# IGNF/StrataNet2-Vegetation-Coverage-Maps

Measured on AMD Instinct MI355X. Metric: plots/s fwd+bwd, 32k-pt synthetic plots, batch 16/GPU, higher is better.
Workload: dtype f32; 1 GPU; C2 ref-arch: 16 plots/GPU x 32768 pts, SA npoint 1024/256 + global, r 1/2 m, train step fwd+P2+loss+bwd+Adam, inputs resident in HBM; plots_per_gpu=16, points_per_plot=32768, batches_per_geometry_pass=8, exchange=none (single GPU), parallelism=single GPU, ranks_seen=1, exchange_in_graph=False

## Files before the change

include/strata_hip.h:

```cpp
#ifndef STRATA_HIP_H
#define STRATA_HIP_H

#include <stddef.h>

#ifdef __cplusplus
extern "C" {
#endif

#define SN2_VERSION 102
#define SN2_EINVAL (-1)
#define SN2_ELIMIT (-2)

#define SN2_MAX_NEIGHBORS 2000
#define SN2_STAT_SLOTS 1024

int sn2_version(void);
int sn2_debug_mfma_chain(const float *a, const float *b, float *d, int mode, void *stream);
int sn2_debug_spin(int blocks, long long clocks, int *out, void *stream);

int sn2_debug_fp1_backward_parts(int mask);
int sn2_debug_fp_rows_form(int form);
int sn2_debug_fp_table_form(int form);
#define SN2_PROBE_SINK_WORDS 4096
int sn2_debug_stream_probe(const float *src, float *dst, size_t n_floats, int mode, float *sink, void *stream);
int sn2_debug_mfma_probe(int mode, int iters, float *sink, double *flops, void *stream);

typedef struct sn2_block {
    int cin, cout;
    const float *W, *b;
    const float *gamma, *beta;
    float *running_mean, *running_var;
    float *a, *c;
    float *mean, *invstd;
    float *stat_slots;
    float *dW, *db, *dgamma, *dbeta;
    int grad_replicas, grad_replica_stride;
    int mma_bf16;
    long long *num_batches_tracked;
    int frozen_stats;
} sn2_block;
#define SN2_BN_FROZEN_KEEP 2
int sn2_grad_reduce(float *flat, int n, int replicas, int stride, void *stream);


int sn2_pack_rows(const float *cloud, const float *xyz, int B, int C, int N, float *rows0, void *stream);

#define SN2_FPS_WS_GRID_WORDS 4104
#define SN2_FPS_WS_XCHG_WORDS 4096
#define SN2_FPS_WS_CTL_WORDS 32
#define SN2_FPS_WS_GRID_OFFSET(B, N) (5L * (B) * (N))
#define SN2_FPS_WS_CTL_OFFSET(B, N) (SN2_FPS_WS_GRID_OFFSET(B, N) + (long)(SN2_FPS_WS_GRID_WORDS + SN2_FPS_WS_XCHG_WORDS) * (B))
#define SN2_FPS_WS_RANK_OFFSET(B, N) (SN2_FPS_WS_CTL_OFFSET(B, N) + SN2_FPS_WS_CTL_WORDS)
#define SN2_FPS_WS_WORDS(B, N) (SN2_FPS_WS_RANK_OFFSET(B, N) + 1L * (B) * (N))
size_t sn2_fps_ws_words(int B, int N);
size_t sn2_fps_ws_grid_offset(int B, int N);
size_t sn2_fps_ws_ctl_offset(int B, int N);
size_t sn2_fps_ws_rank_offset(int B, int N);
int sn2_fps(const float *pos_soa, int B, int N, int M, const int *start, int *idx, float *cpos_soa,
            float *cpos_aos, int *order_ws, void *stream);
int sn2_fps_waves(const float *pos_soa, int B, int N, int M, const int *start, int *idx, float *cpos_soa,
                  float *cpos_aos, int *order_ws, int waves, void *stream);
int sn2_fps_status(const float *pos_soa, int B, int N, int M, const int *start, int *idx, float *cpos_soa,
                   float *cpos_aos, int *order_ws, int waves, unsigned *status, void *stream);
int sn2_fps_live(const float *pos_soa, int B, int N, int M, const int *start, const int *n_live, int *idx, float *cpos_soa,
                 float *cpos_aos, int *order_ws, int waves, int *n_live_out, unsigned *status, void *stream);
int sn2_debug_fps_spin_limit(unsigned sweeps);

int sn2_ball_query(const float *src_soa, int B, int N, const float *cpos_soa, int M, float r2, int cap,
                   int *nbr, int *cnt, unsigned long long *total, const int *fps_ws, void *stream);

int sn2_count_sum(const int *cnt, int n, unsigned long long *total, void *stream);
int sn2_count_sum_group(const int *cnt, int G, int n, unsigned long long *total, size_t total_stride, void *stream);

#define SN2_THREE_NN_WS_WORDS(B, S) ((size_t)(B) * (4 * (size_t)(S) + 1032))
size_t sn2_three_nn_ws_words(int B, int S);
int sn2_three_nn(const float *src_soa, int B, int S, const float *dst_soa, int T, int k, int *idx, float *w,
                 void *ws, const int *dst_fps_ws, void *stream);
#define SN2_THREE_NN_XY_WS_WORDS(B, S, T) ((size_t)(B) * (4 * (size_t)(S) + 5 * (size_t)(T) + 1032))
size_t sn2_three_nn_xy_ws_words(int B, int S, int T);
int sn2_three_nn_xy(const float *src_soa, int B, int S, const float *dst_soa, int T, int k, int *idx, float *w,
                    void *ws, void *stream);

int sn2_prepare_plots(const float *raw, long T, const int *offsets, const float *centers, const float *fake_xy, int n_fake,
                      const int *idx, int B, int N, int train, const double *rot, const int *flips, const float *noise,
                      const long *noise_offsets, long noise_T, float z_max, float *cloud, float *xyz, void *stream);

#define SN2_SUBSAMPLE_LDS 1
#define SN2_SUBSAMPLE_GLOBAL 2
#define SN2_SUBSAMPLE_COARSE 4
#define SN2_SUBSAMPLE_LDS_MAX 16384
int sn2_subsample_form(int n_max, int N);
size_t sn2_subsample_ws_words(int B, int n_max, int N, int form);
int sn2_subsample(const int *offsets, int extra, int n_max, int B, int N, unsigned long long seed, const long long *plot_keys,
                  int form, int *ws, size_t ws_words, int *idx, void *stream);

int sn2_train_batch_ws_words(int B, int n_max, int N, size_t *words);
int sn2_train_batch(const float *raw, long T, const int *offsets, const float *centers, const double *coverages, int P,
                    const int *plot_ids, int B, const float *fake_xy, int n_fake, int n_max, int N, int M1, float z_max,
                    unsigned long long seed, long long epoch, const double *cos_sin, int train, int noise, int *ws,
                    size_t ws_words, float *cloud, float *xyz, double *gt, int *fps_start, void *stream);
int sn2_train_batch_live(const float *raw, long T, const int *offsets, const float *centers, const double *coverages, int P,
                         const int *plot_ids, int B, const float *fake_xy, int n_fake, int n_max, int N, int M1, float z_max,
                         unsigned long long seed, long long epoch, const double *cos_sin, int train, int noise, int *ws,
                         size_t ws_words, float *cloud, float *xyz, double *gt, int *fps_start, int *n_live, void *stream);

int sn2_plots_append(const float *src_raw, long src_T, const int *src_offsets, const float *src_centers, const float *src_cov,
                     const int *sel, int K, float *dst_raw, long cap_T, int *dst_offsets, float *dst_centers, double *dst_cov,
                     int cap_P, int P0, long T0, const int *dst_start, long new_T, void *stream);

#define SN2_ZNORM_WS_WORDS(n, cells) ((size_t)5 * (n) + 3 * (size_t)(cells) + 8)
size_t sn2_znorm_ws_words(int n, long cells);
int sn2_znorm(const float *x, const float *y, const float *z, int n, float radius, float x_min, float y_min, float x_max,
              float y_max, int *ws, float *zmin, float *z_out, void *stream);

size_t sn2_parcel_count_ws_words(int P, int rows);
size_t sn2_parcel_znorm_ws_words(long T, float radius, float x_min, float y_min, float x_max, float y_max);
int sn2_parcel_count(const float *cloud, long T, int L, int rows, const float *centers, int P, const int *cell_start,
                     const int *cell_items, int GX, int GY, double gx0, double gy0, double cell_inv, float radius, int *ws,
                     size_t ws_words, int *prefix, long long *total, void *stream);
int sn2_parcel_fill(const float *cloud, long T, int L, int rows, const float *centers, int P, const int *cell_start,
                    const int *cell_items, int GX, int GY, double gx0, double gy0, double cell_inv, float radius, int *prefix,
                    const int *plot_base, long sum_n, float *raw, int *point_index, void *stream);
int sn2_parcel_znorm(const float *cloud, long T, float x_min, float y_min, float x_max, float y_max, float radius,
                     float disc_radius, const int *offsets, const float *centers, int P, const int *point_index, long sum_n,
                     int *ws, size_t ws_words, float *raw, void *stream);

typedef struct sn2_sa {
    int B, Nsrc, M, cap;
    int cf;
    int nl;
    const float *feat; int feat_stride;
    const float *spos; int spos_stride;
    const float *cpos;
    const int *nbr, *cnt;
    const unsigned long long *total;
    const int *order;
    sn2_block blk[2];
    float *ext; int *arg;
    float *out;
    const float *dout;
    float *dfeat;
    float *bwd_ws;
} sn2_sa;
#define SN2_SA_BWD_WS_REPLICAS 32
#define SN2_SA_BWD_WS_WORDS (SN2_SA_BWD_WS_REPLICAS * 2 * 16 * 12)
#define SN2_SA_SOLO_MIN 64
#define SN2_SA_QUAD_MIN 8
#define SN2_SA_OCT_MIN 4
#define SN2_SA_SOLO_FLAG 0x40000000
#define SN2_SA_OCT_FLAG 0x20000000
#define SN2_SA_PACKED_ITEMS(M) ((M) / 8 + 2)
#define SN2_SA_ORDER_WORDS(B, M) ((size_t)4 * (B) * (M) + (size_t)16 * (B) * SN2_SA_PACKED_ITEMS(M) + 8)
size_t sn2_sa_order_words(int B, int M);
int sn2_sa_order(const int *cnt, int B, int M, int *order, void *stream);
int sn2_sa_order_group(const int *cnt, int G, int B, int M, int *order, size_t stride_words, void *stream);
int sn2_sa_forward(const sn2_sa *p, int training, void *stream);
int sn2_sa_backward(const sn2_sa *p, void *stream);

typedef struct sn2_fp {
    int B, R_per_plot, S_per_plot;
    int ca, cb;
    const float *src; int src_stride; const float *src_a, *src_c;
    const int *knn_idx; const float *knn_w;
    const float *skip; int skip_stride;
    sn2_block blk;
    float *h; int h_stride;
    const float *dy;
    float *dsrc; int dsrc_stride;
    float *dskip; int dskip_stride;
    float *du_scratch;
    float *scatter_ws;
    int scatter_ready;
    const int *bn_sums_done;
    float *src_ws;
    int act_bf16;
    const int *row_perm;
} sn2_fp;
#define SN2_INTERP_CHUNKS(R, S) ((3 * (size_t)(R) + 62) / 63 + (size_t)(S))
#define SN2_FP_SRC_WS_WORDS(B, R, S, cout) ((size_t)(B) * SN2_INTERP_CHUNKS(R, S) * ((((cout) + 3) / 4) * 4))
size_t sn2_interp_chunks(int R_per_plot, int S_per_plot);
size_t sn2_fp_src_ws_words(int B, int R_per_plot, int S_per_plot, int cout);
#define SN2_INTERP_WS_WORDS(B, R, S) \
    ((size_t)(B) * (S) * (((R) + 2047) / 2048 + 6) + 6 * (size_t)(B) * (R) + 64 + 4 * (size_t)(B) * SN2_INTERP_CHUNKS(R, S))
size_t sn2_interp_ws_words(int B, int R_per_plot, int S_per_plot);
int sn2_interp_index(const int *knn_idx, const float *knn_w, const float *src_pos, int B, int R_per_plot,
                     int S_per_plot, float *ws, void *stream);
int sn2_interp_index_perm(const int *knn_idx, const float *knn_w, const float *src_pos, const int *row_perm, int B,
                          int R_per_plot, int S_per_plot, float *ws, void *stream);
int sn2_interp_index_group(const int *knn_idx, const float *knn_w, const float *src_pos, const int *row_perm, int G, int B,
                           int R_per_plot, int S_per_plot, float *ws, size_t ws_stride_words, void *stream);
int sn2_fp_forward(const sn2_fp *p, int training, void *stream);
int sn2_fp_backward(const sn2_fp *p, void *stream);

int sn2_plot_max_forward(const float *h, const float *a, const float *c, int B, int R_per_plot, int C, float *out,
                         int *arg, void *stream);
int sn2_plot_max_backward(const float *dout, const int *arg, int B, int R_per_plot, int C, float *dy, void *stream);

int sn2_global_pool_backward(const float *du, int du_stride, const int *arg, const float *h, const float *mean,
                             const float *invstd, int B, int R_per_plot, int C, float *dx, float *dy, float *dgamma,
                             float *dbeta, void *stream);

#define SN2_GLOBAL_MAX_PLOTS 28
#define SN2_GLOBAL_XCHG_WORDS(B) ((size_t)2 * (size_t)(B) * 4 * 128)
#define SN2_GLOBAL_CTL_WORDS 8
size_t sn2_global_xchg_words(int B);
int sn2_global_level_forward(const sn2_fp *sa3, const sn2_fp *fp3, float *x3, int *arg3, unsigned long long *xchg,
                             unsigned *ctl, void *stream);
#define SN2_GLOBAL_BWD_MAX_ROWS 256
#define SN2_GLOBAL_BWD_XCHG_WORDS ((size_t)2 * SN2_GLOBAL_MAX_PLOTS * 128)
#define SN2_GLOBAL_BWD_CTL_WORDS 64
int sn2_global_level_backward(const sn2_fp *sa3, const sn2_fp *fp3, const int *arg3, unsigned long long *xchg, unsigned *ctl,
                              void *stream);
int sn2_debug_global_spin_limit(unsigned sweeps);

#define SN2_HEAD_LOSS_MAX_PLOTS 128
typedef struct sn2_loss_grad {
    const float *pred;
    const double *gt;
    const float *proba;
    const double *pdf;
    const double *grad_total;
    const int *arg, *nocc, *pix;
    int B, N, D;
    double m, e;
} sn2_loss_grad;

typedef struct sn2_head {
    int R, cin, f_stride;
    const float *f, *fa, *fc;
    const float *W1, *b1, *W2, *b2;
    float *coverages, *proba;
    const float *dcoverages, *dproba;
    float *dy;
    float *dW1, *db1, *dW2, *db2;
    int grad_replicas, grad_replica_stride;
    const int *drop_mask;
    float drop_scale;
    int act_bf16;
    float *zero_fill; long zero_fill_words;
    const sn2_loss_grad *loss;
} sn2_head;
int sn2_head_forward(const sn2_head *p, void *stream);
int sn2_fp_head_eval(const sn2_fp *p, const sn2_head *hd, void *stream);
int sn2_head_backward(const sn2_head *p, void *stream);
int sn2_debug_head_backward_occupancy(int bf16, int with_loss);
int sn2_head_bn_sums(const sn2_head *p, const float *gamma, const float *beta, const float *mean, const float *invstd,
                     float *dgamma, float *dbeta, int *ok, void *stream);
int sn2_fp_bn_sums(const sn2_fp *p, const float *gamma, const float *beta, const float *mean, const float *invstd,
                   float *dgamma, float *dbeta, int *ok, void *stream);


int sn2_plot_project_forward(const float *pred_pointwise, const float *cloud_xy, long plot_stride, int B, int N,
                             int D, unsigned long long *keys, int *pix, int *arg, int *nocc, float *pred,
                             void *stream);
#define SN2_P2_KEY_PARTS(N) (((N) + 4095) / 4096 < 1 ? 1 : (((N) + 4095) / 4096 > 64 ? 64 : ((N) + 4095) / 4096))
size_t sn2_p2_key_parts(int N);
int sn2_plot_pixels(const float *cloud_xy, long plot_stride, int B, int N, int D, float *mm, int *pix, void *stream);
int sn2_plot_project_forward_pix(const float *pred_pointwise, const int *pix, int B, int N, int D,
                                 unsigned long long *keys, int *arg, int *nocc, float *pred, void *stream);
int sn2_plot_project_backward(const float *dpred, const int *arg, const int *nocc, const int *pix, int B, int N,
                              int D, float *dpointwise, void *stream);

int sn2_raster_project(const float *coverages, const float *cloud_xy, long plot_stride, int B, int N, int D,
                       int diam_meters, unsigned long long *keys, int *pix, float *rasters, void *stream);

int sn2_mosaic_merge(const float *rasters, const float *weights, const int *offsets, int B, int D, int H, int W,
                     float *mean, float *wsum, int win_y0, int win_x0, int win_h, int win_w, void *stream);

#define SN2_MOSAIC_HIST_WORDS 10004
int sn2_mosaic_finalize(const float *mean, const float *wsum, int H, int W, int *hist_ws, double *sum_ws, float *thr_out,
                        float *out, void *stream);

#define SN2_MOSAIC_CROP_MAX_BANDS 8
#define SN2_MOSAIC_CROP_MAX_EDGES (1 << 20)
#define SN2_MOSAIC_CROP_MAX_BLOCKS 2048
#define SN2_MOSAIC_CROP_BLOCKS(H, W) \
    ((size_t)(H) * (((size_t)(W) + 255) / 256) < SN2_MOSAIC_CROP_MAX_BLOCKS ? (size_t)(H) * (((size_t)(W) + 255) / 256) \
                                                                           : (size_t)SN2_MOSAIC_CROP_MAX_BLOCKS)
#define SN2_MOSAIC_CROP_WS_WORDS(C, H, W) (4 * (size_t)(C) * SN2_MOSAIC_CROP_BLOCKS(H, W))
extern size_t sn2_mosaic_crop_ws_words(int C, int H, int W);
int sn2_mosaic_crop_stats(float *bands, int C, int H, int W, double x_min, double y_max, double pix, const double *edges, int E,
                          void *ws, double *mean, long long *count, void *stream);

int sn2_kde_lookup(const float *cloud, int B, int C, int N, int z_channel, float z_max, const double *X, const double *Y,
                   int K, double *pdf, void *stream);
#define SN2_KDE_FIT_MAX_K 65536
#define SN2_KDE_FIT_ABS_SLOTS 256
#define SN2_KDE_FIT_SLICES 8
#define SN2_KDE_FIT_WS_WORDS(K) \
    (2 * ((4 + 3 * SN2_KDE_FIT_SLICES) * (size_t)(K) + 3 * (((size_t)(K) + 255) / 256)) + SN2_KDE_FIT_ABS_SLOTS)
size_t sn2_kde_fit_ws_words(int K);
int sn2_kde_fit(const float *z, long n, double bw, int K, void *ws, double *X, double *Y, void *stream);
#define SN2_LOSS_BLOCKS 1024
int sn2_loss_forward(const float *pred, const double *gt, int B, const float *proba, const double *pdf, int R, double m,
                     double e, double *partials, double *out, void *stream);
int sn2_loss_backward(const float *pred, const double *gt, int B, const float *proba, const double *pdf, int R, double m,
                      double e, const double *grad_total, float *dpred, float *dproba, void *stream);

#define SN2_PROJECTED_LOSS_WS (2 * 512 + 2)
int sn2_projected_loss_forward(const float *coverages, const int *pix, const float *proba, const double *pdf, const double *gt,
                               int B, int N, int D, double m, double e, unsigned long long *keys, int *arg, int *nocc,
                               float *pred, double *partials, double *out, void *stream);
int sn2_projected_loss_backward(const float *pred, const double *gt, int B, const float *proba, const double *pdf, int N, int D,
                                double m, double e, const double *grad_total, const int *arg, const int *nocc, const int *pix,
                                float *dcoverages, float *dproba, void *stream);

#define SN2_PLOT_LOSSES_SLICE_ROWS 2048
#define SN2_PLOT_LOSSES_SLICES(N) \
    (((N) + SN2_PLOT_LOSSES_SLICE_ROWS - 1) / SN2_PLOT_LOSSES_SLICE_ROWS < 1 ? 1 : \
     (((N) + SN2_PLOT_LOSSES_SLICE_ROWS - 1) / SN2_PLOT_LOSSES_SLICE_ROWS > 64 ? 64 : ((N) + SN2_PLOT_LOSSES_SLICE_ROWS - 1) / SN2_PLOT_LOSSES_SLICE_ROWS))
size_t sn2_plot_losses_ws_words(int B, int N, int D);
int sn2_plot_losses(const float *coverages, const int *pix, const float *proba, const double *pdf, const double *gt, int B, int N,
                    int D, double m, double e, void *ws, float *pred, double *out, void *stream);

int sn2_adam_step(float *param, const float *grad, float *exp_avg, float *exp_avg_sq, int n, float lr, float beta1,
                  float beta2, float eps, float weight_decay, int *step_dev ,
                  float grad_scale, void *stream);

#define SN2_METER_TERMS 4
int sn2_adam_step_dev(float *param, const float *grad, float *exp_avg, float *exp_avg_sq, int n, const float *lr_dev, float beta1,
                      float beta2, float eps, float weight_decay, int *step_dev, float grad_scale, const double *terms, int n_terms,
                      double *meter, void *stream);


typedef struct sn2_net_layer {
    int cin, cout;
    const float *W, *b, *gamma, *beta;
    float *running_mean, *running_var;
    long long *num_batches_tracked;
    int gW, gb, ggamma, gbeta;
    int mma_bf16;
} sn2_net_layer;

typedef struct sn2_net_model {
    sn2_net_layer sa1[2], sa2, sa3, fp3, fp2, fp1;
    const float *lin1_W, *lin1_b, *lin2_W, *lin2_b;
    int g_lin1_W, g_lin1_b, g_lin2_W, g_lin2_b;
    int n_flat;
    float r1_sq, r2_sq;
    int max_neighbors;
    float drop_p;
    int fuse_global_level;
    int fuse_eval_head;
    int source_side;
    int fps_waves_shared, fps_waves_many;
} sn2_net_model;

typedef struct sn2_net_dims {
    int B, N, M1, M2;
    int cap1, cap2;
    int act_bf16;
    int p2_diam_pix;
} sn2_net_dims;

typedef struct sn2_net_geo {
    const float *xyz;
    int *idx1; float *pos1_soa, *pos1_aos; int *ws1;
    int *nbr1, *cnt1; unsigned long long *tot1; int *ord1;
    int *idx2; float *pos2_soa, *pos2_aos; int *ws2;
    int *nbr2, *cnt2; unsigned long long *tot2; int *ord2;
    const float *pos3;
    int *knn3_idx; float *knn3_w;
    int *knn2_idx; float *knn2_w;
    int *knn1_idx; float *knn1_w;
    float *inv3, *inv2, *inv1;
    int *nn_ws2, *nn_ws1;
    const int *rank1;
    float *rows0;
    int *p2_pix; float *p2_mm;
} sn2_net_geo;

typedef struct sn2_net_act {
    float *aux;
    float *stats;
    float *ext1; int *arg1; float *x1;
    float *ext2; int *arg2; float *x2;
    float *h_sa3, *h3;
    float *x3; int *arg3;
    float *h2;
    void *h1;
    float *src_ws1, *src_ws2;
    float *cov, *proba;
    const int *drop_mask;
    float *bwd_arena; long bwd_arena_words;
} sn2_net_act;

#define SN2_NET_GRAD_IMAGES 32
typedef struct sn2_net_bwd {
    const float *dcov, *dproba;
    float *arena; long arena_words;
    int images, image_stride;
    float *dy2, *dy3, *dx1, *dx2, *dx3, *dy_sa3;
    float *sa1_ws;
    void *dy1, *du1;
    float *du2, *du3;
    int *bn_ok;
    float *src_ws1, *src_ws2;
    int defer_grad_reduce;
    int arena_is_zero;
    int frozen_stats;
    unsigned long long *gl_xchg; unsigned *gl_ctl;
    const sn2_loss_grad *loss;
} sn2_net_bwd;

#define SN2_NET_FORK 1
#define SN2_NET_SHARED 2
#define SN2_NET_INVERTED 4
#define SN2_NET_DEFER_JOIN 8
#define SN2_NET_INPUT_ONLY 16
#define SN2_NET_HAS_ROWS0 32
#define SN2_NET_JOIN_PENDING 64
#define SN2_NET_WITH_GEOMETRY 128
#define SN2_NET_HAS_INVERTED 256

typedef struct sn2_net_io {
    const float *cloud;
    const int *fps_start;
    unsigned *fps_status;
    unsigned long long *gl_xchg; unsigned *gl_ctl;
    void *stream_b, *stream_c, *stream_pack;
    void *ctx;
    int flags;
    int training;
    const int *fps_live;
    int *fps_live1;
} sn2_net_io;

int sn2_net_ctx_create(void **ctx);
int sn2_net_ctx_destroy(void *ctx);
int sn2_net_geo_carve(const sn2_net_model *m, const sn2_net_dims *d, void *base, sn2_net_geo *out, size_t *bytes);
int sn2_net_act_carve(const sn2_net_model *m, const sn2_net_dims *d, int training, void *base, sn2_net_act *out, size_t *bytes);
int sn2_net_bwd_carve(const sn2_net_model *m, const sn2_net_dims *d, void *arena_base, void *scratch_base, sn2_net_bwd *out,
                      size_t *arena_bytes, size_t *scratch_bytes);
int sn2_net_geometry(const sn2_net_model *m, const sn2_net_dims *d, const sn2_net_geo *g, const sn2_net_io *io, void *stream);
int sn2_net_forward(const sn2_net_model *m, const sn2_net_dims *d, const sn2_net_geo *g, const sn2_net_act *a,
                    const sn2_net_io *io, void *stream);
int sn2_net_backward(const sn2_net_model *m, const sn2_net_dims *d, const sn2_net_geo *g, const sn2_net_act *a,
                     const sn2_net_bwd *b, void *stream);

int sn2_adam_step_images(float *param, float *grad_images, int replicas, int stride, float *exp_avg, float *exp_avg_sq, int n,
                         float lr, float beta1, float beta2, float eps, float weight_decay, int *step_dev, float grad_scale,
                         void *stream);
int sn2_adam_step_images_dev(float *param, float *grad_images, int replicas, int stride, float *exp_avg, float *exp_avg_sq, int n,
                             const float *lr_dev, float beta1, float beta2, float eps, float weight_decay, int *step_dev,
                             float grad_scale, const double *terms, int n_terms, double *meter, void *stream);

int sn2_fps_fills_ws(int B, int N, int M);
int sn2_three_nn_uses_grid(int S, int T);
int sn2_fp_rows_small(long R);
int sn2_fp_source_side(long R, int cb, int force);
int sn2_global_level_forward_route(int B, int bf16);
int sn2_global_level_backward_route(int B, int M2, int frozen, int bf16);
int sn2_head_loss_route(int B, int N, int D);

#ifdef __cplusplus
}
#endif
#endif
```

stratanet2_vegetation_coverage_maps_amd/_lib.py:

```python
import ctypes
import functools
import os
from ctypes import POINTER, Structure, c_double, c_float, c_int, c_long, c_longlong, c_void_p

HERE = os.path.dirname(os.path.abspath(__file__))
LIB_PATH = os.path.join(HERE, "csrc", "libstrata_hip.so")

CONSTANTS = {
    "SN2_VERSION": 102, "SN2_EINVAL": -1, "SN2_ELIMIT": -2,
    "SN2_MAX_NEIGHBORS": 2000, "SN2_STAT_SLOTS": 1024, "SN2_BN_FROZEN_KEEP": 2,
    "SN2_FPS_WS_GRID_WORDS": 4104, "SN2_FPS_WS_CTL_WORDS": 32,
    "SN2_SUBSAMPLE_LDS": 1, "SN2_SUBSAMPLE_GLOBAL": 2, "SN2_SUBSAMPLE_COARSE": 4, "SN2_SUBSAMPLE_LDS_MAX": 16384,
    "SN2_SA_BWD_WS_WORDS": 32 * 2 * 16 * 12,
    "SN2_GLOBAL_MAX_PLOTS": 28, "SN2_GLOBAL_CTL_WORDS": 8, "SN2_GLOBAL_BWD_MAX_ROWS": 256,
    "SN2_GLOBAL_BWD_XCHG_WORDS": 2 * 28 * 128, "SN2_GLOBAL_BWD_CTL_WORDS": 64,
    "SN2_MOSAIC_HIST_WORDS": 10004, "SN2_MOSAIC_CROP_MAX_BANDS": 8, "SN2_MOSAIC_CROP_MAX_EDGES": 1 << 20,
    "SN2_MOSAIC_CROP_MAX_BLOCKS": 2048, "SN2_KDE_FIT_MAX_K": 65536, "SN2_LOSS_BLOCKS": 1024, "SN2_PROJECTED_LOSS_WS": 2 * 512 + 2,
    "SN2_NET_GRAD_IMAGES": 32, "SN2_METER_TERMS": 4,
    "SN2_NET_FORK": 1, "SN2_NET_SHARED": 2, "SN2_NET_INVERTED": 4, "SN2_NET_DEFER_JOIN": 8, "SN2_NET_INPUT_ONLY": 16,
    "SN2_NET_HAS_ROWS0": 32, "SN2_NET_JOIN_PENDING": 64, "SN2_NET_WITH_GEOMETRY": 128, "SN2_NET_HAS_INVERTED": 256,
}
globals().update(CONSTANTS)
MAX_NEIGHBORS, STAT_SLOTS, BN_FROZEN_KEEP = CONSTANTS["SN2_MAX_NEIGHBORS"], CONSTANTS["SN2_STAT_SLOTS"], CONSTANTS["SN2_BN_FROZEN_KEEP"]
(NET_FORK, NET_SHARED, NET_INVERTED, NET_DEFER_JOIN, NET_INPUT_ONLY, NET_HAS_ROWS0, NET_JOIN_PENDING, NET_WITH_GEOMETRY,
 NET_HAS_INVERTED) = (CONSTANTS["SN2_NET_" + n] for n in ("FORK", "SHARED", "INVERTED", "DEFER_JOIN", "INPUT_ONLY", "HAS_ROWS0",
                                                          "JOIN_PENDING", "WITH_GEOMETRY", "HAS_INVERTED"))


class Block(Structure):
    _fields_ = [("cin", c_int), ("cout", c_int), ("W", c_void_p), ("b", c_void_p), ("gamma", c_void_p),
                ("beta", c_void_p), ("running_mean", c_void_p), ("running_var", c_void_p), ("a", c_void_p),
                ("c", c_void_p), ("mean", c_void_p), ("invstd", c_void_p), ("stat_slots", c_void_p),
                ("dW", c_void_p), ("db", c_void_p), ("dgamma", c_void_p), ("dbeta", c_void_p),
                ("grad_replicas", c_int), ("grad_replica_stride", c_int), ("mma_bf16", c_int),
                ("num_batches_tracked", c_void_p), ("frozen_stats", c_int)]


class SA(Structure):
    _fields_ = [("B", c_int), ("Nsrc", c_int), ("M", c_int), ("cap", c_int), ("cf", c_int), ("nl", c_int),
                ("feat", c_void_p), ("feat_stride", c_int), ("spos", c_void_p), ("spos_stride", c_int),
                ("cpos", c_void_p), ("nbr", c_void_p), ("cnt", c_void_p), ("total", c_void_p), ("order", c_void_p),
                ("blk", Block * 2),
                ("ext", c_void_p), ("arg", c_void_p), ("out", c_void_p), ("dout", c_void_p), ("dfeat", c_void_p),
                ("bwd_ws", c_void_p)]


class FP(Structure):
    _fields_ = [("B", c_int), ("R_per_plot", c_int), ("S_per_plot", c_int), ("ca", c_int), ("cb", c_int),
                ("src", c_void_p), ("src_stride", c_int), ("src_a", c_void_p), ("src_c", c_void_p),
                ("knn_idx", c_void_p), ("knn_w", c_void_p), ("skip", c_void_p), ("skip_stride", c_int),
                ("blk", Block), ("h", c_void_p), ("h_stride", c_int), ("dy", c_void_p), ("dsrc", c_void_p),
                ("dsrc_stride", c_int), ("dskip", c_void_p), ("dskip_stride", c_int), ("du_scratch", c_void_p),
                ("scatter_ws", c_void_p), ("scatter_ready", c_int), ("bn_sums_done", c_void_p), ("src_ws", c_void_p),
                ("act_bf16", c_int), ("row_perm", c_void_p)]


class LossGrad(Structure):
    _fields_ = [(n, c_void_p) for n in ("pred", "gt", "proba", "pdf", "grad_total", "arg", "nocc", "pix")] + [
        ("B", c_int), ("N", c_int), ("D", c_int), ("m", c_double), ("e", c_double)]


class Head(Structure):
    _fields_ = [("R", c_int), ("cin", c_int), ("f_stride", c_int), ("f", c_void_p), ("fa", c_void_p),
                ("fc", c_void_p), ("W1", c_void_p), ("b1", c_void_p), ("W2", c_void_p), ("b2", c_void_p),
                ("coverages", c_void_p), ("proba", c_void_p), ("dcoverages", c_void_p), ("dproba", c_void_p),
                ("dy", c_void_p), ("dW1", c_void_p), ("db1", c_void_p), ("dW2", c_void_p), ("db2", c_void_p),
                ("grad_replicas", c_int), ("grad_replica_stride", c_int), ("drop_mask", c_void_p), ("drop_scale", c_float),
                ("act_bf16", c_int), ("zero_fill", c_void_p), ("zero_fill_words", c_long), ("loss", POINTER(LossGrad))]


class NetLayer(Structure):
    _fields_ = [("cin", c_int), ("cout", c_int), ("W", c_void_p), ("b", c_void_p), ("gamma", c_void_p), ("beta", c_void_p),
                ("running_mean", c_void_p), ("running_var", c_void_p), ("num_batches_tracked", c_void_p),
                ("gW", c_int), ("gb", c_int), ("ggamma", c_int), ("gbeta", c_int), ("mma_bf16", c_int)]


class NetModel(Structure):
    _fields_ = [("sa1", NetLayer * 2), ("sa2", NetLayer), ("sa3", NetLayer), ("fp3", NetLayer), ("fp2", NetLayer), ("fp1", NetLayer),
                ("lin1_W", c_void_p), ("lin1_b", c_void_p), ("lin2_W", c_void_p), ("lin2_b", c_void_p),
                ("g_lin1_W", c_int), ("g_lin1_b", c_int), ("g_lin2_W", c_int), ("g_lin2_b", c_int), ("n_flat", c_int),
                ("r1_sq", c_float), ("r2_sq", c_float), ("max_neighbors", c_int), ("drop_p", c_float),
                ("fuse_global_level", c_int), ("fuse_eval_head", c_int), ("source_side", c_int),
                ("fps_waves_shared", c_int), ("fps_waves_many", c_int)]


class NetDims(Structure):
    _fields_ = [("B", c_int), ("N", c_int), ("M1", c_int), ("M2", c_int), ("cap1", c_int), ("cap2", c_int), ("act_bf16", c_int),
                ("p2_diam_pix", c_int)]


class NetGeo(Structure):
    _fields_ = [(n, c_void_p) for n in (
        "xyz", "idx1", "pos1_soa", "pos1_aos", "ws1", "nbr1", "cnt1", "tot1", "ord1",
        "idx2", "pos2_soa", "pos2_aos", "ws2", "nbr2", "cnt2", "tot2", "ord2", "pos3",
        "knn3_idx", "knn3_w", "knn2_idx", "knn2_w", "knn1_idx", "knn1_w", "inv3", "inv2", "inv1", "nn_ws2", "nn_ws1",
        "rank1", "rows0", "p2_pix", "p2_mm")]


class NetAct(Structure):
    _fields_ = [(n, c_void_p) for n in (
        "aux", "stats", "ext1", "arg1", "x1", "ext2", "arg2", "x2", "h_sa3", "h3", "x3", "arg3", "h2", "h1", "src_ws1", "src_ws2",
        "cov", "proba", "drop_mask", "bwd_arena")] + [("bwd_arena_words", c_long)]


class NetBwd(Structure):
    _fields_ = [("dcov", c_void_p), ("dproba", c_void_p), ("arena", c_void_p), ("arena_words", c_long), ("images", c_int),
                ("image_stride", c_int)] + [(n, c_void_p) for n in (
                    "dy2", "dy3", "dx1", "dx2", "dx3", "dy_sa3", "sa1_ws", "dy1", "du1", "du2", "du3", "bn_ok", "src_ws1", "src_ws2")] + [
                        ("defer_grad_reduce", c_int), ("arena_is_zero", c_int), ("frozen_stats", c_int), ("gl_xchg", c_void_p),
                        ("gl_ctl", c_void_p), ("loss", POINTER(LossGrad))]


class NetIO(Structure):
    _fields_ = [("cloud", c_void_p), ("fps_start", c_void_p), ("fps_status", c_void_p), ("gl_xchg", c_void_p), ("gl_ctl", c_void_p),
                ("stream_b", c_void_p), ("stream_c", c_void_p), ("stream_pack", c_void_p), ("ctx", c_void_p), ("flags", c_int),
                ("training", c_int), ("fps_live", c_void_p), ("fps_live1", c_void_p)]


SIGNATURES = {
    "sn2_version": [],
    "sn2_debug_mfma_chain": [c_void_p, c_void_p, c_void_p, c_int, c_void_p],
    "sn2_debug_spin": [c_int, c_longlong, c_void_p, c_void_p],
    "sn2_debug_fp1_backward_parts": [c_int],
    "sn2_debug_fp_rows_form": [c_int],
    "sn2_debug_fp_table_form": [c_int],
    "sn2_debug_stream_probe": [c_void_p, c_void_p, ctypes.c_size_t, c_int, c_void_p, c_void_p],
    "sn2_debug_mfma_probe": [c_int, c_int, c_void_p, POINTER(c_double), c_void_p],
    "sn2_pack_rows": [c_void_p, c_void_p, c_int, c_int, c_int, c_void_p, c_void_p],
    "sn2_fps": [c_void_p, c_int, c_int, c_int, c_void_p, c_void_p, c_void_p, c_void_p, c_void_p, c_void_p],
    "sn2_fps_waves": [c_void_p, c_int, c_int, c_int, c_void_p, c_void_p, c_void_p, c_void_p, c_void_p, c_int, c_void_p],
    "sn2_fps_status": [c_void_p, c_int, c_int, c_int, c_void_p, c_void_p, c_void_p, c_void_p, c_void_p, c_int, c_void_p, c_void_p],
    "sn2_fps_live": [c_void_p, c_int, c_int, c_int, c_void_p, c_void_p, c_void_p, c_void_p, c_void_p, c_void_p, c_int, c_void_p, c_void_p,
                     c_void_p],
    "sn2_debug_fps_spin_limit": [ctypes.c_uint],
    "sn2_ball_query": [c_void_p, c_int, c_int, c_void_p, c_int, c_float, c_int, c_void_p, c_void_p, c_void_p, c_void_p,
                       c_void_p],
    "sn2_three_nn": [c_void_p, c_int, c_int, c_void_p, c_int, c_int, c_void_p, c_void_p, c_void_p, c_void_p, c_void_p],
    "sn2_count_sum": [c_void_p, c_int, c_void_p, c_void_p],
    "sn2_count_sum_group": [c_void_p, c_int, c_int, c_void_p, ctypes.c_size_t, c_void_p],
    "sn2_three_nn_xy": [c_void_p, c_int, c_int, c_void_p, c_int, c_int, c_void_p, c_void_p, c_void_p, c_void_p],
    "sn2_prepare_plots": [c_void_p, c_long, c_void_p, c_void_p, c_void_p, c_int, c_void_p, c_int, c_int, c_int, c_void_p,
                          c_void_p, c_void_p, c_void_p, c_long, c_float, c_void_p, c_void_p, c_void_p],
    "sn2_znorm": [c_void_p, c_void_p, c_void_p, c_int, c_float, c_float, c_float, c_float, c_float, c_void_p, c_void_p,
                  c_void_p, c_void_p],
    "sn2_parcel_count": [c_void_p, c_long, c_int, c_int, c_void_p, c_int, c_void_p, c_void_p, c_int, c_int, c_double, c_double,
                         c_double, c_float, c_void_p, ctypes.c_size_t, c_void_p, c_void_p, c_void_p],
    "sn2_parcel_fill": [c_void_p, c_long, c_int, c_int, c_void_p, c_int, c_void_p, c_void_p, c_int, c_int, c_double, c_double,
                        c_double, c_float, c_void_p, c_void_p, c_long, c_void_p, c_void_p, c_void_p],
    "sn2_parcel_znorm": [c_void_p, c_long, c_float, c_float, c_float, c_float, c_float, c_float, c_void_p, c_void_p, c_int,
                         c_void_p, c_long, c_void_p, ctypes.c_size_t, c_void_p, c_void_p],
    "sn2_subsample_form": [c_int, c_int],
    "sn2_subsample": [c_void_p, c_int, c_int, c_int, c_int, ctypes.c_ulonglong, c_void_p, c_int, c_void_p, ctypes.c_size_t,
                      c_void_p, c_void_p],
    "sn2_train_batch_ws_words": [c_int, c_int, c_int, POINTER(ctypes.c_size_t)],
    "sn2_train_batch": [c_void_p, c_long, c_void_p, c_void_p, c_void_p, c_int, c_void_p, c_int, c_void_p, c_int, c_int, c_int, c_int,
                        c_float, ctypes.c_ulonglong, c_longlong, c_void_p, c_int, c_int, c_void_p, ctypes.c_size_t, c_void_p, c_void_p,
                        c_void_p, c_void_p, c_void_p],
    "sn2_train_batch_live": [c_void_p, c_long, c_void_p, c_void_p, c_void_p, c_int, c_void_p, c_int, c_void_p, c_int, c_int, c_int, c_int,
                             c_float, ctypes.c_ulonglong, c_longlong, c_void_p, c_int, c_int, c_void_p, ctypes.c_size_t, c_void_p,
                             c_void_p, c_void_p, c_void_p, c_void_p, c_void_p],
    "sn2_plots_append": [c_void_p, c_long, c_void_p, c_void_p, c_void_p, c_void_p, c_int, c_void_p, c_long, c_void_p, c_void_p,
                         c_void_p, c_int, c_int, c_long, c_void_p, c_long, c_void_p],
    "sn2_sa_order": [c_void_p, c_int, c_int, c_void_p, c_void_p],
    "sn2_sa_order_group": [c_void_p, c_int, c_int, c_int, c_void_p, ctypes.c_size_t, c_void_p],
    "sn2_sa_forward": [POINTER(SA), c_int, c_void_p],
    "sn2_sa_backward": [POINTER(SA), c_void_p],
    "sn2_grad_reduce": [c_void_p, c_int, c_int, c_int, c_void_p],
    "sn2_interp_index": [c_void_p, c_void_p, c_void_p, c_int, c_int, c_int, c_void_p, c_void_p],
    "sn2_interp_index_perm": [c_void_p, c_void_p, c_void_p, c_void_p, c_int, c_int, c_int, c_void_p, c_void_p],
    "sn2_interp_index_group": [c_void_p, c_void_p, c_void_p, c_void_p, c_int, c_int, c_int, c_int, c_void_p, ctypes.c_size_t, c_void_p],
    "sn2_fp_forward": [POINTER(FP), c_int, c_void_p],
    "sn2_fp_backward": [POINTER(FP), c_void_p],
    "sn2_plot_max_forward": [c_void_p, c_void_p, c_void_p, c_int, c_int, c_int, c_void_p, c_void_p, c_void_p],
    "sn2_plot_max_backward": [c_void_p, c_void_p, c_int, c_int, c_int, c_void_p, c_void_p],
    "sn2_global_pool_backward": [c_void_p, c_int, c_void_p, c_void_p, c_void_p, c_void_p, c_int, c_int, c_int, c_void_p, c_void_p,
                                 c_void_p, c_void_p, c_void_p],
    "sn2_global_level_forward": [POINTER(FP), POINTER(FP), c_void_p, c_void_p, c_void_p, c_void_p, c_void_p],
    "sn2_global_level_backward": [POINTER(FP), POINTER(FP), c_void_p, c_void_p, c_void_p, c_void_p],
    "sn2_debug_global_spin_limit": [ctypes.c_uint],
    "sn2_head_forward": [POINTER(Head), c_void_p],
    "sn2_fp_head_eval": [POINTER(FP), POINTER(Head), c_void_p],
    "sn2_fp_bn_sums": [POINTER(FP), c_void_p, c_void_p, c_void_p, c_void_p, c_void_p, c_void_p, c_void_p, c_void_p],
    "sn2_head_bn_sums": [POINTER(Head), c_void_p, c_void_p, c_void_p, c_void_p, c_void_p, c_void_p, c_void_p, c_void_p],
    "sn2_head_backward": [POINTER(Head), c_void_p],
    "sn2_debug_head_backward_occupancy": [c_int, c_int],
    "sn2_plot_project_forward": [c_void_p, c_void_p, c_long, c_int, c_int, c_int, c_void_p, c_void_p, c_void_p,
                                 c_void_p, c_void_p, c_void_p],
    "sn2_plot_pixels": [c_void_p, c_long, c_int, c_int, c_int, c_void_p, c_void_p, c_void_p],
    "sn2_plot_project_forward_pix": [c_void_p, c_void_p, c_int, c_int, c_int, c_void_p, c_void_p, c_void_p, c_void_p, c_void_p],
    "sn2_plot_project_backward": [c_void_p, c_void_p, c_void_p, c_void_p, c_int, c_int, c_int, c_void_p, c_void_p],
    "sn2_raster_project": [c_void_p, c_void_p, c_long, c_int, c_int, c_int, c_int, c_void_p, c_void_p, c_void_p,
                           c_void_p],
    "sn2_mosaic_merge": [c_void_p, c_void_p, c_void_p, c_int, c_int, c_int, c_int, c_void_p, c_void_p,
                         c_int, c_int, c_int, c_int, c_void_p],
    "sn2_mosaic_finalize": [c_void_p, c_void_p, c_int, c_int, c_void_p, c_void_p, c_void_p, c_void_p, c_void_p],
    "sn2_mosaic_crop_stats": [c_void_p, c_int, c_int, c_int, c_double, c_double, c_double, c_void_p, c_int, c_void_p, c_void_p,
                              c_void_p, c_void_p],
    "sn2_kde_lookup": [c_void_p, c_int, c_int, c_int, c_int, c_float, c_void_p, c_void_p, c_int, c_void_p, c_void_p],
    "sn2_kde_fit": [c_void_p, c_long, c_double, c_int, c_void_p, c_void_p, c_void_p, c_void_p],
    "sn2_loss_forward": [c_void_p, c_void_p, c_int, c_void_p, c_void_p, c_int, c_double, c_double, c_void_p, c_void_p,
                         c_void_p],
    "sn2_loss_backward": [c_void_p, c_void_p, c_int, c_void_p, c_void_p, c_int, c_double, c_double, c_void_p, c_void_p,
                          c_void_p, c_void_p],
    "sn2_adam_step": [c_void_p, c_void_p, c_void_p, c_void_p, c_int, c_float, c_float, c_float, c_float, c_float,
                      c_void_p, c_float, c_void_p],
    "sn2_adam_step_dev": [c_void_p, c_void_p, c_void_p, c_void_p, c_int, c_void_p, c_float, c_float, c_float, c_float,
                          c_void_p, c_float, c_void_p, c_int, c_void_p, c_void_p],
    "sn2_projected_loss_forward": [c_void_p, c_void_p, c_void_p, c_void_p, c_void_p, c_int, c_int, c_int, c_double, c_double, c_void_p,
                                   c_void_p, c_void_p, c_void_p, c_void_p, c_void_p, c_void_p],
    "sn2_projected_loss_backward": [c_void_p, c_void_p, c_int, c_void_p, c_void_p, c_int, c_int, c_double, c_double, c_void_p, c_void_p,
                                    c_void_p, c_void_p, c_void_p, c_void_p, c_void_p],
    "sn2_plot_losses": [c_void_p, c_void_p, c_void_p, c_void_p, c_void_p, c_int, c_int, c_int, c_double, c_double, c_void_p, c_void_p,
                        c_void_p, c_void_p],
    "sn2_adam_step_images": [c_void_p, c_void_p, c_int, c_int, c_void_p, c_void_p, c_int, c_float, c_float, c_float, c_float, c_float,
                             c_void_p, c_float, c_void_p],
    "sn2_adam_step_images_dev": [c_void_p, c_void_p, c_int, c_int, c_void_p, c_void_p, c_int, c_void_p, c_float, c_float, c_float,
                                 c_float, c_void_p, c_float, c_void_p, c_int, c_void_p, c_void_p],
    "sn2_net_ctx_create": [POINTER(c_void_p)],
    "sn2_net_ctx_destroy": [c_void_p],
    "sn2_net_geo_carve": [POINTER(NetModel), POINTER(NetDims), c_void_p, POINTER(NetGeo), POINTER(ctypes.c_size_t)],
    "sn2_net_act_carve": [POINTER(NetModel), POINTER(NetDims), c_int, c_void_p, POINTER(NetAct), POINTER(ctypes.c_size_t)],
    "sn2_net_bwd_carve": [POINTER(NetModel), POINTER(NetDims), c_void_p, c_void_p, POINTER(NetBwd), POINTER(ctypes.c_size_t),
                          POINTER(ctypes.c_size_t)],
    "sn2_net_geometry": [POINTER(NetModel), POINTER(NetDims), POINTER(NetGeo), POINTER(NetIO), c_void_p],
    "sn2_net_forward": [POINTER(NetModel), POINTER(NetDims), POINTER(NetGeo), POINTER(NetAct), POINTER(NetIO), c_void_p],
    "sn2_net_backward": [POINTER(NetModel), POINTER(NetDims), POINTER(NetGeo), POINTER(NetAct), POINTER(NetBwd), c_void_p],
    "sn2_fps_fills_ws": [c_int, c_int, c_int],
    "sn2_three_nn_uses_grid": [c_int, c_int],
    "sn2_fp_rows_small": [c_long],
    "sn2_fp_source_side": [c_long, c_int, c_int],
    "sn2_global_level_forward_route": [c_int, c_int],
    "sn2_global_level_backward_route": [c_int, c_int, c_int, c_int],
    "sn2_head_loss_route": [c_int, c_int, c_int],
}

SIZE_HELPERS = {
    "sn2_fps_ws_words": [c_int, c_int],
    "sn2_fps_ws_grid_offset": [c_int, c_int],
    "sn2_fps_ws_ctl_offset": [c_int, c_int],
    "sn2_fps_ws_rank_offset": [c_int, c_int],
    "sn2_three_nn_ws_words": [c_int, c_int],
    "sn2_three_nn_xy_ws_words": [c_int, c_int, c_int],
    "sn2_znorm_ws_words": [c_int, c_long],
    "sn2_sa_order_words": [c_int, c_int],
    "sn2_interp_chunks": [c_int, c_int],
    "sn2_interp_ws_words": [c_int, c_int, c_int],
    "sn2_fp_src_ws_words": [c_int, c_int, c_int, c_int],
    "sn2_global_xchg_words": [c_int],
    "sn2_p2_key_parts": [c_int],
    "sn2_kde_fit_ws_words": [c_int],
    "sn2_parcel_count_ws_words": [c_int, c_int],
    "sn2_parcel_znorm_ws_words": [c_long, c_float, c_float, c_float, c_float, c_float],
    "sn2_subsample_ws_words": [c_int, c_int, c_int, c_int],
    "sn2_plot_losses_ws_words": [c_int, c_int, c_int],
}

EXTERN_SIZE_HELPERS = {
    "sn2_mosaic_crop_ws_words": [c_int, c_int, c_int],
}

_lib = None


class StrataHipError(RuntimeError):
    pass


def load():
    global _lib
    if _lib is not None:
        return _lib
    if not os.path.exists(LIB_PATH):
        raise StrataHipError(
            f"{LIB_PATH} not found: build it with `python -m stratanet2_vegetation_coverage_maps_amd._build` "
            "(or __graft_entry__.build()); the HIP library is mandatory, there is no fallback path")
    lib = ctypes.CDLL(LIB_PATH)
    for name, argtypes in SIGNATURES.items():
        fn = getattr(lib, name)
        fn.argtypes = argtypes
        fn.restype = c_int
    for name, argtypes in list(SIZE_HELPERS.items()) + list(EXTERN_SIZE_HELPERS.items()):
        fn = getattr(lib, name)
        fn.argtypes = argtypes
        fn.restype = ctypes.c_size_t
    if lib.sn2_version() != SN2_VERSION:
        raise StrataHipError(f"libstrata_hip.so version {lib.sn2_version()} != binding {SN2_VERSION}: rebuild")
    _lib = lib
    return lib


@functools.lru_cache(maxsize=4096)
def host_value(name: str, *args) -> int:
    return getattr(load(), name)(*args)


def check(rc: int, what: str):
    if rc != 0:
        kind = "hipError_t" if rc > 0 else {-1: "SN2_EINVAL", -2: "SN2_ELIMIT"}.get(rc, "error")
        raise StrataHipError(f"{what} failed: {kind} {rc}")
```

stratanet2_vegetation_coverage_maps_amd/csrc/global_level.hip:

```cpp
#include "global_level.h"

namespace {

#ifdef SN2_GL_STAMPS
__device__ unsigned long long g_gl_dbg[16];
extern "C" int sn2_debug_gl_stamps(unsigned long long* out) {
    return (int)hipMemcpyFromSymbol(out, HIP_SYMBOL(g_gl_dbg), sizeof(g_gl_dbg));
}
#define GSTAMP(i)                                                                                   \
    if (blockIdx.x == 0 && threadIdx.x == 0) {                                                      \
        unsigned long long t_;                                                                      \
        asm volatile("s_memtime %0\n\ts_waitcnt lgkmcnt(0)" : "=s"(t_)::"memory");                   \
        g_gl_dbg[i] = t_;                                                                           \
    }
#else
#define GSTAMP(i)
#endif
constexpr int GL_QS = OuterAcc<16, 36>::QS;
constexpr int GL_W3 = 64 * 35 + 64, GL_WF = 64 * 96 + 64;
constexpr int GL_FIXED_FLOATS = GL_GROUPS * 64 * GL_QS + GL_GROUPS * 128 + 128 + 64 + 2 * 1024 + 2 * 8 * 128 + GL_W3 + GL_WF;
static_assert((GL_FIXED_FLOATS + GL_MAX_PLOTS * GL_GROUPS * 128) * 4 <= 160 * 1024, "LDS");

template <int KB>
__device__ __forceinline__ void gl_block_tiles(const float* s_q, int QS, int lane, int g, long row0, long R_lim,
                                               const float (&Wb)[KB], float init, float* __restrict__ h, int h_stride,
                                               float& ssum, float& ssq, f32x4 (&V)[4]) {
    const int qq = lane >> 4, cc = lane & 15, o = 16 * g + cc;
#pragma unroll
    for (int t = 0; t < 4; ++t) V[t] = f32x4{init, init, init, init};
#pragma unroll
    for (int kb = 0; kb < KB; ++kb) {
#pragma unroll
        for (int t = 0; t < 4; ++t)
            V[t] = __builtin_amdgcn_mfma_f32_16x16x4f32(s_q[(16 * t + cc) * QS + 4 * kb + qq], Wb[kb], V[t], 0, 0, 0);
    }
#pragma unroll
    for (int t = 0; t < 4; ++t)
#pragma unroll
        for (int j = 0; j < 4; ++j) {
            const long row = row0 + 16 * t + 4 * qq + j;
            const float v = row < R_lim ? fmaxf(V[t][j], 0.f) : 0.f;
            V[t][j] = v;
            ssum += v;
            ssq = fmaf(v, v, ssq);
            if (row < R_lim) h[(size_t)row * h_stride + o] = v;
        }
}

struct GlLayer {
    const float *W, *bias, *gamma, *beta;
    float *running_mean, *running_var, *a, *c, *mean, *invstd;
    long long* nbt;
    float* h;
};
struct GlArgs {
    int B, M2;
    const float* x2;
    const float* pos2;
    const int* knn_idx;
    const float* knn_w;
    float* x3;
    int* arg3;
    GlLayer sa3, fp3;
    gl_u64* xchg;
    unsigned* ctl;
    unsigned spin_limit;
};

template <bool REPAIR>
__device__ __forceinline__ void gl_level_body(const GlArgs& A, float* gl_smem) {
    const int tid = threadIdx.x, lane = tid & 63;
    const int grp = __builtin_amdgcn_readfirstlane(tid >> 8), g = __builtin_amdgcn_readfirstlane((tid >> 6) & 3);
    float* s_q = gl_smem + grp * 64 * GL_QS;

    float* s_red = gl_smem + GL_GROUPS * 64 * GL_QS;
    float* s_ac = s_red + GL_GROUPS * 128;
    float* s_x3 = s_ac + 128;
    float* s_mv = s_x3 + 64;
    int* s_mi = reinterpret_cast<int*>(s_mv + 1024);
    double* s_d = reinterpret_cast<double*>(s_mi + 1024);
    float* s_w3 = reinterpret_cast<float*>(s_d + 8 * 128);
    float* s_wf = s_w3 + GL_W3;
    float* s_x = s_wf + GL_WF;
    __shared__ unsigned s_epoch;
    __shared__ int s_fail;
    const int B = A.B, M2 = A.M2;
    const int b_lo = REPAIR ? 0 : (int)blockIdx.x, b_hi = REPAIR ? B : b_lo + 1;
    const bool lead = REPAIR || blockIdx.x == 0;
    float w3r[3], b3r, bfr;
    f32x4 wfr[2];
#pragma unroll
    for (int j = 0; j < 3; ++j) w3r[j] = A.sa3.W[min(tid + 1024 * j, 64 * 35 - 1)];
#pragma unroll
    for (int j = 0; j < 2; ++j) wfr[j] = reinterpret_cast<const f32x4*>(A.fp3.W)[min(tid + 1024 * j, 64 * 96 / 4 - 1)];
    b3r = A.sa3.bias[tid & 63], bfr = A.fp3.bias[tid & 63];
    unsigned epoch_now = 0;
    if (tid == 0) epoch_now = __hip_atomic_load(&A.ctl[0], __ATOMIC_RELAXED, __HIP_MEMORY_SCOPE_AGENT);
#pragma unroll
    for (int j = 0; j < 3; ++j)
        if (tid + 1024 * j < 64 * 35) s_w3[tid + 1024 * j] = w3r[j];
#pragma unroll
    for (int j = 0; j < 2; ++j)
        if (tid + 1024 * j < 64 * 96 / 4) reinterpret_cast<f32x4*>(s_wf)[tid + 1024 * j] = wfr[j];
    if (tid < 64) s_w3[64 * 35 + tid] = b3r, s_wf[64 * 96 + tid] = bfr;
    if (tid == 0) {
        s_epoch = epoch_now + 1u;
        s_fail = 0;
    }
    const int nblk = (M2 + 63) >> 6, trips = (nblk + GL_GROUPS - 1) / GL_GROUPS;
    const int qq = lane >> 4, cc = lane & 15, o = 16 * g + cc;
    const int n_gran = B * GL_GROUPS * 128;
    const double n_rows = (double)B * (double)M2;
    __syncthreads();
    const unsigned epoch = s_epoch;
    unsigned applied = 0;
    if constexpr (REPAIR) applied = __hip_atomic_load(&A.ctl[3], __ATOMIC_RELAXED, __HIP_MEMORY_SCOPE_AGENT);
    f32x4 V3[4];
#pragma unroll
    for (int t = 0; t < 4; ++t) V3[t] = f32x4{0.f, 0.f, 0.f, 0.f};
    GSTAMP(0)
    for (int b = b_lo; b < b_hi; ++b) {
        constexpr int CA = 32, CB = 3, CI = CA + CB, CK = CI + 1, KB = (CK + 3) / 4, QS = OuterAcc<16, CK>::QS;
        const long row_lo = (long)b * M2, R_lim = row_lo + M2;
        float Wb[KB];
        float ssum = 0.f, ssq = 0.f;
        for (int it = 0; it < trips; ++it) {
            const int blk = it * GL_GROUPS + grp;
            const long r0 = row_lo + (long)blk * 64;
            if (blk < nblk) {
                stage_inputs<CA, CB, false>(s_q, QS, g, lane, r0, (int)R_lim, M2, M2, A.x2, 32, nullptr, nullptr, nullptr, nullptr,
                                            A.pos2, 4);
                if (g == 2) {
#pragma unroll
                    for (int k = CK; k < 4 * KB; ++k) s_q[lane * QS + k] = 0.f;
                }
            }
            __syncthreads();
            if (it == 0) {
#pragma unroll
                for (int kb = 0; kb < KB; ++kb) {
                    const int k = 4 * kb + qq;
                    Wb[kb] = k < CI ? s_w3[o * CI + k] : (k == CI ? s_w3[64 * CI + o] : 0.f);
                }
            }
            if (blk < nblk) gl_block_tiles<KB>(s_q, QS, lane, g, r0, R_lim, Wb, 0.f, A.sa3.h, 64, ssum, ssq, V3);
            __syncthreads();
        }
        ssum += __shfl_xor(ssum, 16);
        ssq += __shfl_xor(ssq, 16);
        ssum += __shfl_xor(ssum, 32);
        ssq += __shfl_xor(ssq, 32);
        if (qq == 0) {
            s_red[grp * 128 + o] = ssum;
            s_red[grp * 128 + 64 + o] = ssq;
        }
        __syncthreads();
        if (b == b_lo) { GSTAMP(1) }
        if (tid < GL_GROUPS * 128)
            __hip_atomic_store(A.xchg + (size_t)b * GL_GROUPS * 128 + tid,
                               ((gl_u64)(epoch * 2u + 0u) << 32) | (gl_u64)__float_as_uint(s_red[tid]), __ATOMIC_RELAXED,
                               __HIP_MEMORY_SCOPE_AGENT);
        if constexpr (REPAIR) __syncthreads();
    }
    {
        const unsigned tag = epoch * 2u + 0u;
        if (!gl_collect(A.xchg, n_gran, tag, s_x, A.spin_limit)) s_fail = 1;
        __syncthreads();
        GSTAMP(2)
        if (s_fail) {
            if constexpr (!REPAIR) {
                if (tid < GL_GROUPS * 128)
                    __hip_atomic_store(A.xchg + n_gran + (size_t)b_lo * GL_GROUPS * 128 + tid, (gl_u64)((epoch * 2u + 1u) ^ GL_POISON) << 32,
                                       __ATOMIC_RELAXED, __HIP_MEMORY_SCOPE_AGENT);
                if (tid == 0) {
                    atomicAdd(&A.ctl[1], 1u);
                    if (lead) {
                        __hip_atomic_store(&A.ctl[3], 0u, __ATOMIC_RELAXED, __HIP_MEMORY_SCOPE_AGENT);
                        __hip_atomic_store(&A.ctl[0], epoch, __ATOMIC_RELAXED, __HIP_MEMORY_SCOPE_AGENT);
                    }
                }
                return;
            }
        }
        {
            const int col = tid & 127, part = tid >> 7;
            double acc = 0.0;
            for (int w = part; w < B * GL_GROUPS; w += 8) acc += (double)s_x[w * 128 + col];
            s_d[part * 128 + col] = acc;
        }
        __syncthreads();
        if (tid < 64) {
            double s1 = 0.0, s2 = 0.0;
#pragma unroll
            for (int part = 0; part < 8; ++part) s1 += s_d[part * 128 + tid], s2 += s_d[part * 128 + 64 + tid];
            float aa, cc2, mean, invstd;
            const bool upd = lead && !(applied & 1u);
            sn2_bn_from_sums(s1, s2, n_rows, A.sa3.gamma[tid], A.sa3.beta[tid], upd ? &A.sa3.running_mean[tid] : nullptr,
                             upd ? &A.sa3.running_var[tid] : nullptr, aa, cc2, mean, invstd);
            s_ac[tid] = aa;
            s_ac[64 + tid] = cc2;
            if (lead) {
                A.sa3.a[tid] = aa, A.sa3.c[tid] = cc2, A.sa3.mean[tid] = mean, A.sa3.invstd[tid] = invstd;
                if (tid == 0 && upd && A.sa3.nbt) *A.sa3.nbt += 1;
            }
        }
        __syncthreads();
    }
    GSTAMP(3)
    for (int b = b_lo; b < b_hi; ++b) {
    const long row_lo = (long)b * M2, R_lim = row_lo + M2;
    if (!REPAIR && trips == 1) {
        const float aa = s_ac[o], cc2 = s_ac[64 + o];
        float best = -INFINITY;
        int bi = 0x7FFFFFFF;
#pragma unroll
        for (int t = 0; t < 4; ++t)
#pragma unroll
            for (int j = 0; j < 4; ++j) {
                const int r = grp * 64 + 16 * t + 4 * qq + j;
                const float y = fmaf(aa, V3[t][j], cc2);
                if (r < M2 && y > best) best = y, bi = r;
            }
#pragma unroll
        for (int m = 16; m <= 32; m <<= 1) {
            const float v = __shfl_xor(best, m);
            const int i = __shfl_xor(bi, m);
            if (v > best || (v == best && i < bi)) best = v, bi = i;
        }
        if (qq == 0) s_mv[grp * 64 + o] = best, s_mi[grp * 64 + o] = bi;
        __syncthreads();
        if (tid < 64) {
            best = s_mv[tid], bi = s_mi[tid];
            for (int k2 = 1; k2 < GL_GROUPS; ++k2) {
                const float v = s_mv[k2 * 64 + tid];
                const int i = s_mi[k2 * 64 + tid];
                if (v > best || (v == best && i < bi)) best = v, bi = i;
            }
            A.x3[(size_t)b * 64 + tid] = best;
            A.arg3[(size_t)b * 64 + tid] = bi;
            s_x3[tid] = best;
        }
        __syncthreads();
    } else {
        const int ch = tid & 63, rg = tid >> 6;
        const float aa = s_ac[ch], cc2 = s_ac[64 + ch];
        float best = -INFINITY;
        int bi = 0x7FFFFFFF;
        const float* hb = A.sa3.h + (size_t)row_lo * 64 + ch;
        int r = rg;
        for (; r + 7 * 16 < M2; r += 8 * 16) {
            float v[8];
#pragma unroll
            for (int u = 0; u < 8; ++u) v[u] = hb[(size_t)(r + u * 16) * 64];
#pragma unroll
            for (int u = 0; u < 8; ++u) {
                const float y = fmaf(aa, v[u], cc2);
                if (y > best) best = y, bi = r + u * 16;
            }
        }
        for (; r < M2; r += 16) {
            const float y = fmaf(aa, hb[(size_t)r * 64], cc2);
            if (y > best) best = y, bi = r;
        }
        s_mv[tid] = best;
        s_mi[tid] = bi;
        __syncthreads();
        if (tid < 64) {
            for (int k2 = 1; k2 < 16; ++k2) {
                const float v = s_mv[k2 * 64 + ch];
                const int i = s_mi[k2 * 64 + ch];
                if (v > best || (v == best && i < bi)) best = v, bi = i;
            }
            A.x3[(size_t)b * 64 + ch] = best;
            A.arg3[(size_t)b * 64 + ch] = bi;
            s_x3[ch] = best;
        }
        __syncthreads();
    }
    if (b == b_lo) { GSTAMP(4) }
    {
        constexpr int CA = 64, CB = 32, CI = CA + CB, KB = CB / 4, QS = OuterAcc<16, 36>::QS;
        float* s_pv = s_mv;
        {
            const int oo = tid >> 4, part = tid & 15;
            const float4 w4 = *reinterpret_cast<const float4*>(s_wf + oo * CI + 4 * part);
            const float4 u4 = *reinterpret_cast<const float4*>(s_x3 + 4 * part);
            float acc = ((w4.x * u4.x + w4.y * u4.y) + w4.z * u4.z) + w4.w * u4.w;
#pragma unroll
            for (int m = 8; m > 0; m >>= 1) acc += __shfl_xor(acc, m);
            if (part == 0) s_pv[oo] = acc + s_wf[64 * CI + oo];
        }
        float Wb[KB];
#pragma unroll
        for (int kb = 0; kb < KB; ++kb) Wb[kb] = s_wf[o * CI + CA + 4 * kb + qq];
        float ssum = 0.f, ssq = 0.f;
        f32x4 Vf[4];
        for (int it = 0; it < trips; ++it) {
            const int blk = it * GL_GROUPS + grp;
            const long r0 = row_lo + (long)blk * 64;
            if (blk < nblk && (REPAIR || trips > 1)) {
                const int t256 = tid & 255;
#pragma unroll
                for (int pass = 0; pass < 2; ++pass) {
                    const int row = pass * 32 + (t256 >> 3), q8 = t256 & 7;
                    const long r = r0 + row;
                    const size_t rr = r < R_lim ? (size_t)r : (size_t)(R_lim - 1);
                    *reinterpret_cast<float4*>(&s_q[row * QS + 4 * q8]) = reinterpret_cast<const float4*>(A.x2 + rr * 32)[q8];
                }
            }
            __syncthreads();
            if (blk < nblk) gl_block_tiles<KB>(s_q, QS, lane, g, r0, R_lim, Wb, s_pv[o], A.fp3.h, 64, ssum, ssq, Vf);
            __syncthreads();
        }
        ssum += __shfl_xor(ssum, 16);
        ssq += __shfl_xor(ssq, 16);
        ssum += __shfl_xor(ssum, 32);
        ssq += __shfl_xor(ssq, 32);
        if (qq == 0) {
            s_red[grp * 128 + o] = ssum;
            s_red[grp * 128 + 64 + o] = ssq;
        }
    }
    __syncthreads();
    if (b == b_lo) { GSTAMP(5) }
    if (tid < GL_GROUPS * 128)
        __hip_atomic_store(A.xchg + n_gran + (size_t)b * GL_GROUPS * 128 + tid,
                           ((gl_u64)(epoch * 2u + 1u) << 32) | (gl_u64)__float_as_uint(s_red[tid]), __ATOMIC_RELAXED,
                           __HIP_MEMORY_SCOPE_AGENT);
    if constexpr (REPAIR) __syncthreads();
    }
    {
        gl_u64* gx = A.xchg + n_gran;
        const unsigned tag = epoch * 2u + 1u;
        if (!lead) return;
        if (!gl_collect(gx, n_gran, tag, s_x, A.spin_limit)) s_fail = 1;
        __syncthreads();
        GSTAMP(6)
        if (s_fail) {
            if (tid == 0) {
                atomicAdd(&A.ctl[1], 1u);
                __hip_atomic_store(&A.ctl[3], 1u, __ATOMIC_RELAXED, __HIP_MEMORY_SCOPE_AGENT);
                __hip_atomic_store(&A.ctl[0], epoch, __ATOMIC_RELAXED, __HIP_MEMORY_SCOPE_AGENT);
            }
            return;
        }
        {
            const int col = tid & 127, part = tid >> 7;
            double acc = 0.0;
            for (int w = part; w < B * GL_GROUPS; w += 8) acc += (double)s_x[w * 128 + col];
            s_d[part * 128 + col] = acc;
        }
        __syncthreads();
        if (tid < 64) {
            double s1 = 0.0, s2 = 0.0;
#pragma unroll
            for (int part = 0; part < 8; ++part) s1 += s_d[part * 128 + tid], s2 += s_d[part * 128 + 64 + tid];
            float aa, cc2, mean, invstd;
            const bool upd = !(applied & 2u);
            sn2_bn_from_sums(s1, s2, n_rows, A.fp3.gamma[tid], A.fp3.beta[tid], upd ? &A.fp3.running_mean[tid] : nullptr,
                             upd ? &A.fp3.running_var[tid] : nullptr, aa, cc2, mean, invstd);
            A.fp3.a[tid] = aa, A.fp3.c[tid] = cc2, A.fp3.mean[tid] = mean, A.fp3.invstd[tid] = invstd;
            if (tid == 0 && upd && A.fp3.nbt) *A.fp3.nbt += 1;
        }
        __syncthreads();
        GSTAMP(7)
        if (tid == 0) {
            if constexpr (REPAIR) {
                __hip_atomic_store(&A.ctl[2], __hip_atomic_load(&A.ctl[1], __ATOMIC_RELAXED, __HIP_MEMORY_SCOPE_AGENT), __ATOMIC_RELAXED,
                                   __HIP_MEMORY_SCOPE_AGENT);
                __hip_atomic_store(&A.ctl[0], epoch + 2u, __ATOMIC_RELAXED, __HIP_MEMORY_SCOPE_AGENT);
            } else {
                __hip_atomic_store(&A.ctl[3], 3u, __ATOMIC_RELAXED, __HIP_MEMORY_SCOPE_AGENT);
                __hip_atomic_store(&A.ctl[0], epoch, __ATOMIC_RELAXED, __HIP_MEMORY_SCOPE_AGENT);
            }
        }
    }
}

__global__ __launch_bounds__(1024) void global_level_fwd_kernel(GlArgs A) {
    extern __shared__ __attribute__((aligned(16))) float gl_smem[];
    __shared__ int s_repair;
    gl_level_body<false>(A, gl_smem);
    __syncthreads();
    if (threadIdx.x == 0) {
        const unsigned t = atomicAdd(&A.ctl[4], 1u);
        int repair = 0;
        if (t == gridDim.x - 1) {
            __hip_atomic_store(&A.ctl[4], 0u, __ATOMIC_RELAXED, __HIP_MEMORY_SCOPE_AGENT);
            repair = __hip_atomic_load(&A.ctl[1], __ATOMIC_RELAXED, __HIP_MEMORY_SCOPE_AGENT) !=
                     __hip_atomic_load(&A.ctl[2], __ATOMIC_RELAXED, __HIP_MEMORY_SCOPE_AGENT);
        }
        s_repair = repair;
    }
    __syncthreads();
    if (!s_repair) return;
    gl_level_body<true>(A, gl_smem);
}

}

unsigned g_gl_spin_limit = 1u << 18;
extern "C" int sn2_debug_global_spin_limit(unsigned sweeps) {
    g_gl_spin_limit = sweeps ? sweeps : (1u << 18);
    return 0;
}

extern "C" int sn2_global_level_forward_route(int B, int bf16) { return B <= GL_MAX_PLOTS && !bf16; }
extern "C" size_t sn2_global_xchg_words(int B) { return SN2_GLOBAL_XCHG_WORDS(B); }

extern "C" int sn2_global_level_forward(const sn2_fp* sa3, const sn2_fp* fp3, float* x3, int* arg3, unsigned long long* xchg,
                                        unsigned* ctl, void* stream) {
    if (!sa3 || !fp3 || !x3 || !arg3 || !xchg || !ctl) return SN2_EINVAL;
    const int B = sa3->B, M2 = sa3->R_per_plot;
    if (!(B > 0 && M2 > 0 && fp3->B == B && fp3->R_per_plot == M2 && sa3->S_per_plot == M2 && fp3->S_per_plot == 1)) return SN2_EINVAL;
    if (!(sa3->ca == 32 && sa3->cb == 3 && sa3->blk.cin == 35 && sa3->blk.cout == 64 && fp3->ca == 64 && fp3->cb == 32 &&
          fp3->blk.cin == 96 && fp3->blk.cout == 64))
        return SN2_ELIMIT;
    if (!sn2_global_level_forward_route(B, sa3->blk.mma_bf16 || fp3->blk.mma_bf16) || sa3->act_bf16 || fp3->act_bf16) return SN2_ELIMIT;
    if (sa3->knn_idx || sa3->src_a || !fp3->knn_idx || !fp3->knn_w || fp3->src_a) return SN2_EINVAL;
    if (!sa3->src || sa3->src_stride != 32 || !sa3->skip || sa3->skip_stride != 4 || !sa3->h || sa3->h_stride != 64) return SN2_EINVAL;
    if (fp3->src != x3 || fp3->src_stride != 64 || fp3->skip != sa3->src || fp3->skip_stride != 32 || !fp3->h || fp3->h_stride != 64)
        return SN2_EINVAL;
    if ((long)B * M2 >= (1L << 31) / 64) return SN2_ELIMIT;
    for (const sn2_block* k : {&sa3->blk, &fp3->blk})
        if (!k->W || !k->b || !k->gamma || !k->beta || !k->running_mean || !k->running_var || !k->a || !k->c || !k->mean || !k->invstd)
            return SN2_EINVAL;
    GlArgs A;
    A.B = B, A.M2 = M2;
    A.x2 = sa3->src, A.pos2 = sa3->skip, A.knn_idx = fp3->knn_idx, A.knn_w = fp3->knn_w, A.x3 = x3, A.arg3 = arg3;
    auto layer = [](const sn2_fp* p) {
        GlLayer l;
        l.W = p->blk.W, l.bias = p->blk.b, l.gamma = p->blk.gamma, l.beta = p->blk.beta;
        l.running_mean = p->blk.running_mean, l.running_var = p->blk.running_var;
        l.a = p->blk.a, l.c = p->blk.c, l.mean = p->blk.mean, l.invstd = p->blk.invstd;
        l.nbt = p->blk.num_batches_tracked, l.h = p->h;
        return l;
    };
    A.sa3 = layer(sa3), A.fp3 = layer(fp3);
    A.xchg = xchg, A.ctl = ctl;
    A.spin_limit = g_gl_spin_limit;
    const size_t lds = ((size_t)GL_FIXED_FLOATS + (size_t)B * GL_GROUPS * 128) * 4;
    (void)hipFuncSetAttribute(reinterpret_cast<const void*>(&global_level_fwd_kernel), hipFuncAttributeMaxDynamicSharedMemorySize, (int)lds);
    hipLaunchKernelGGL(global_level_fwd_kernel, dim3(B), dim3(1024), lds, (hipStream_t)stream, A);
    SN2_RETURN_LAUNCH();
}
```

stratanet2_vegetation_coverage_maps_amd/csrc/net.hip:

```cpp
#include "common.h"

#include <cstring>
#include <new>

namespace {

constexpr int WIDTHS[7] = {16, 16, 32, 64, 64, 34, 34};
constexpr int WIDTH_SUM = 260;
constexpr int GRAD_IMAGES = SN2_NET_GRAD_IMAGES;

struct NetCtx {
    hipEvent_t fork, b_tables, b_nn, b_done, c_nn, c_done, pack_fork, packed;
};

inline bool fp_src_ws_wanted(const sn2_net_model* m, long R, int cb, bool force) {
    return m->source_side && sn2_fp_source_side(R, cb, force);
}
inline bool fused_eval_head(const sn2_net_model* m, const sn2_net_dims* d, int training) {
    return !training && m->fuse_eval_head && !d->act_bf16 && m->source_side;
}
inline int gl_bf16(const sn2_net_model* m) { return m->sa3.mma_bf16 || m->fp3.mma_bf16; }

struct Carver {
    uintptr_t base;
// ... 298 lines not shown
    if (!g || !bytes) return SN2_EINVAL;
    const size_t B = d->B, N = d->N, M1 = d->M1, M2 = d->M2;
    memset(g, 0, sizeof(*g));
    Carver c(base);
    g->idx1 = c.take<int>(B * M1), g->pos1_soa = c.take<float>(B * 3 * M1), g->pos1_aos = c.take<float>(B * M1 * 4);
    g->ws1 = sn2_fps_fills_ws(d->B, d->N, d->M1) ? c.take<int>((size_t)SN2_FPS_WS_WORDS(B, N)) : nullptr;
    g->nbr1 = c.take<int>(B * M1 * (size_t)d->cap1), g->cnt1 = c.take<int>(B * M1);
    g->tot1 = c.take<unsigned long long>(1), g->ord1 = c.take<int>(SN2_SA_ORDER_WORDS(B, M1));
    g->idx2 = c.take<int>(B * M2), g->pos2_soa = c.take<float>(B * 3 * M2), g->pos2_aos = c.take<float>(B * M2 * 4);
    g->ws2 = sn2_fps_fills_ws(d->B, d->M1, d->M2) ? c.take<int>((size_t)SN2_FPS_WS_WORDS(B, M1)) : nullptr;
    g->nbr2 = c.take<int>(B * M2 * (size_t)d->cap2), g->cnt2 = c.take<int>(B * M2);
    g->tot2 = c.take<unsigned long long>(1), g->ord2 = c.take<int>(SN2_SA_ORDER_WORDS(B, M2));
    g->knn3_idx = c.take<int>(B * M2 * 3), g->knn3_w = c.take<float>(B * M2 * 3);
    g->knn2_idx = c.take<int>(B * M1 * 3), g->knn2_w = c.take<float>(B * M1 * 3);
    g->knn1_idx = c.take<int>(B * N * 3), g->knn1_w = c.take<float>(B * N * 3);
    g->inv3 = c.take<float>(SN2_INTERP_WS_WORDS(B, M2, 1));
    g->inv2 = c.take<float>(SN2_INTERP_WS_WORDS(B, M1, M2));
    g->inv1 = c.take<float>(SN2_INTERP_WS_WORDS(B, N, M1));
    g->nn_ws2 = sn2_three_nn_uses_grid(d->M2, d->M1) ? c.take<int>(SN2_THREE_NN_XY_WS_WORDS(B, M2, M1)) : nullptr;
    g->nn_ws1 = sn2_three_nn_uses_grid(d->M1, d->N) ? c.take<int>(SN2_THREE_NN_XY_WS_WORDS(B, M1, N)) : nullptr;
    g->rows0 = c.take<float>(B * N * 12);
    if (d->p2_diam_pix > 0) g->p2_pix = c.take<int>(B * N), g->p2_mm = c.take<float>(B * 4);
    *bytes = c.bytes();
    return 0;
}

extern "C" int sn2_net_act_carve(const sn2_net_model* m, const sn2_net_dims* d, int training, void* base, sn2_net_act* a,
                                 size_t* bytes) {
    SN2_TRY(check_dims(m, d));
    if (!a || !bytes) return SN2_EINVAL;
    const size_t B = d->B, N = d->N, M1 = d->M1, M2 = d->M2;
    memset(a, 0, sizeof(*a));
    Carver c(base);
    a->aux = c.take<float>(4 * WIDTH_SUM), a->stats = c.take<float>((size_t)SN2_STAT_SLOTS * 2 * WIDTH_SUM);
    a->ext1 = c.take<float>(B * M1 * 16), a->arg1 = c.take<int>(B * M1 * 16), a->x1 = c.take<float>(B * M1 * 16);
    a->ext2 = c.take<float>(B * M2 * 32), a->arg2 = c.take<int>(B * M2 * 32), a->x2 = c.take<float>(B * M2 * 32);
    a->h_sa3 = c.take<float>(B * M2 * 64), a->h3 = c.take<float>(B * M2 * 64);
    a->x3 = c.take<float>(B * 64), a->arg3 = c.take<int>(B * 64);
    a->h2 = c.take<float>(B * M1 * 36);
    const bool fused_eval = fused_eval_head(m, d, training);
    if (!fused_eval) a->h1 = d->act_bf16 ? (void*)c.take<unsigned short>(B * N * 36) : (void*)c.take<float>(B * N * 36);
    if (fp_src_ws_wanted(m, (long)B * N, 8, fused_eval)) a->src_ws1 = c.take<float>(SN2_FP_SRC_WS_WORDS(B, N, M1, 34));
    if (fp_src_ws_wanted(m, (long)B * M1, 16, false)) a->src_ws2 = c.take<float>(SN2_FP_SRC_WS_WORDS(B, M1, M2, 34));
    *bytes = c.bytes();
    return 0;
}

extern "C" int sn2_net_bwd_carve(const sn2_net_model* m, const sn2_net_dims* d, void* arena_base, void* scratch_base,
                                 sn2_net_bwd* b, size_t* arena_bytes, size_t* scratch_bytes) {
    SN2_TRY(check_dims(m, d));
    if (!b || !arena_bytes || !scratch_bytes || m->n_flat <= 0) return SN2_EINVAL;
    const size_t B = d->B, N = d->N, M1 = d->M1, M2 = d->M2;
    memset(b, 0, sizeof(*b));
    const size_t stride = ((size_t)m->n_flat + 63) / 64 * 64;
    float* ar = static_cast<float*>(arena_base);
    size_t o = GRAD_IMAGES * stride;
    auto take = [&](size_t n) {
        float* p = ar + o;
        o += (n + 3) / 4 * 4;
        return p;
    };
    b->arena = ar, b->images = GRAD_IMAGES, b->image_stride = (int)stride;
    b->dy2 = take(B * M1 * 36), b->dy3 = take(B * M2 * 64), b->dx1 = take(B * M1 * 16), b->dx2 = take(B * M2 * 32);
    b->dx3 = take(B * 64), b->dy_sa3 = take(B * M2 * 64);
    b->sa1_ws = take(SN2_SA_BWD_WS_WORDS);
    b->arena_words = (long)o;
    *arena_bytes = o * sizeof(float);
    Carver c(scratch_base);
    if (d->act_bf16) {
        b->dy1 = c.take<unsigned short>(B * N * 36), b->du1 = c.take<unsigned short>(B * N * 36);
    } else {
        b->dy1 = c.take<float>(B * N * 36), b->du1 = c.take<float>(B * N * 36);
    }
    b->du2 = c.take<float>(B * M1 * 64), b->du3 = c.take<float>(B * M2 * 64);
    b->bn_ok = c.take<int>(4);
    if (fp_src_ws_wanted(m, (long)B * N, 8, false)) b->src_ws1 = c.take<float>(SN2_FP_SRC_WS_WORDS(B, N, M1, 34));
    if (fp_src_ws_wanted(m, (long)B * M1, 16, false)) b->src_ws2 = c.take<float>(SN2_FP_SRC_WS_WORDS(B, M1, M2, 34));
    *scratch_bytes = c.bytes();
    return 0;
}

extern "C" int sn2_net_geometry(const sn2_net_model* m, const sn2_net_dims* d, const sn2_net_geo* g, const sn2_net_io* io,
                                void* stream) {
    SN2_TRY(check_dims(m, d));
    if (!io) return SN2_EINVAL;
    SN2_TRY(check_geo(d, g));
    SN2_TRY(check_geo_workspaces(d, g));
    if ((io->flags & SN2_NET_INVERTED) && (!g->inv1 || !g->inv2 || !g->inv3)) return SN2_EINVAL;
    return geometry_impl(m, d, g, io, io->flags, (hipStream_t)stream);
}

extern "C" int sn2_net_forward(const sn2_net_model* m, const sn2_net_dims* d, const sn2_net_geo* g, const sn2_net_act* a,
                               const sn2_net_io* io, void* stream) {
    SN2_TRY(check_dims(m, d));
    SN2_TRY(check_model_ptrs(m));
    if (!io || !a) return SN2_EINVAL;
    SN2_TRY(check_geo(d, g));
    if (!a->aux || !a->stats || !a->ext1 || !a->arg1 || !a->x1 || !a->ext2 || !a->arg2 || !a->x2 || !a->h_sa3 || !a->h3 || !a->x3 ||
        !a->arg3 || !a->h2 || !a->cov || !a->proba)
        return SN2_EINVAL;
    if (io->training < 0 || io->training > SN2_BN_FROZEN_KEEP) return SN2_EINVAL;
    const int mode = io->training, training = mode != 0 ? 1 : 0, batch_stats = mode == 1 ? 1 : 0, flags = io->flags;
    const int B = d->B, N = d->N, M2 = d->M2;
    hipStream_t cur = (hipStream_t)stream;
    NetCtx* ctx = static_cast<NetCtx*>(io->ctx);
    const bool fused_eval = fused_eval_head(m, d, training);
    if (!fused_eval && !a->h1) return SN2_EINVAL;
    if (training && !(g->inv1 && g->inv2 && g->inv3)) return SN2_EINVAL;
    const GradDst nograd{nullptr, 0, 0};
    bool join_b = false, join_c = false, wait_pack = false;
    bool have_rows0 = flags & SN2_NET_HAS_ROWS0;
    if (flags & SN2_NET_WITH_GEOMETRY) {
        if (!io->cloud) return SN2_EINVAL;
        SN2_TRY(check_geo_workspaces(d, g));
        int gflags = (flags & (SN2_NET_FORK | SN2_NET_SHARED)) | (training ? SN2_NET_INVERTED : 0);
        const bool fork = (flags & SN2_NET_FORK) && ctx && io->stream_b && io->stream_c;
        if (fork) {
            gflags |= SN2_NET_DEFER_JOIN;
            if (io->stream_pack && !have_rows0) {
                hipStream_t sp = (hipStream_t)io->stream_pack;
                NET_HIP(hipEventRecord(ctx->pack_fork, cur));
                NET_HIP(hipStreamWaitEvent(sp, ctx->pack_fork, 0));
                SN2_TRY(sn2_pack_rows(io->cloud, g->xyz, B, 10, N, g->rows0, sp));
                NET_HIP(hipEventRecord(ctx->packed, sp));
                wait_pack = have_rows0 = true;
            }
        } else {
            gflags &= ~SN2_NET_FORK;
        }
        SN2_TRY(geometry_impl(m, d, g, io, gflags, cur));
        join_b = join_c = fork;
    } else {
        if (flags & SN2_NET_JOIN_PENDING) {
            if (!ctx) return SN2_EINVAL;
            join_b = join_c = true;
        }
        if (training && !(flags & SN2_NET_HAS_INVERTED)) {
            if (join_b) NET_HIP(hipStreamWaitEvent(cur, ctx->b_done, 0));
            if (join_c) NET_HIP(hipStreamWaitEvent(cur, ctx->c_done, 0));
            join_b = join_c = false;
            SN2_TRY(inverted_tables(d, g, 3, cur));
        }
    }
    if (wait_pack) NET_HIP(hipStreamWaitEvent(cur, ctx->packed, 0));
    if (!have_rows0) {
        if (!io->cloud) return SN2_EINVAL;
        SN2_TRY(sn2_pack_rows(io->cloud, g->xyz, B, 10, N, g->rows0, cur));
    }
    sn2_sa sa;
    sa1_desc(&sa, m, d, g, a, nograd, nullptr);
    SN2_TRY(sn2_sa_forward(&sa, mode, cur));
    if (join_b) NET_HIP(hipStreamWaitEvent(cur, ctx->b_tables, 0));
    sa2_desc(&sa, m, d, g, a, nograd, nullptr, nullptr);
    SN2_TRY(sn2_sa_forward(&sa, mode, cur));
    if (join_b) NET_HIP(hipStreamWaitEvent(cur, ctx->b_nn, 0));
    sn2_fp p3, pf3;
    fp_desc(&p3, d, a, sa3_in(m, d, g, a), nograd);
    fp_desc(&pf3, d, a, fp3_in(m, d, g, a), nograd);
    if (batch_stats && m->fuse_global_level && io->gl_xchg && io->gl_ctl && sn2_global_level_forward_route(B, gl_bf16(m))) {
        SN2_TRY(sn2_global_level_forward(&p3, &pf3, a->x3, a->arg3, io->gl_xchg, io->gl_ctl, cur));
    } else {
        SN2_TRY(sn2_fp_forward(&p3, mode, cur));
        SN2_TRY(sn2_plot_max_forward(a->h_sa3, p3.blk.a, p3.blk.c, B, M2, 64, a->x3, a->arg3, cur));
        SN2_TRY(sn2_fp_forward(&pf3, mode, cur));
    }
    sn2_fp p2;
    fp_desc(&p2, d, a, fp2_in(m, d, g, a, a->src_ws2), nograd);
    SN2_TRY(sn2_fp_forward(&p2, mode, cur));
    if (join_c) NET_HIP(hipStreamWaitEvent(cur, ctx->c_nn, 0));
    sn2_fp p1;
    sn2_head hd;
    if (fused_eval) {
        if (!a->src_ws1) return SN2_EINVAL;
        sn2_net_act a2 = *a;
        a2.h1 = nullptr;
        fp_desc(&p1, d, &a2, fp1_in(m, d, g, &a2, a->src_ws1), nograd);
        head_desc(&hd, m, d, &a2, 0);
        SN2_TRY(sn2_fp_head_eval(&p1, &hd, cur));
    } else {
        fp_desc(&p1, d, a, fp1_in(m, d, g, a, a->src_ws1), nograd);
        SN2_TRY(sn2_fp_forward(&p1, mode, cur));
        head_desc(&hd, m, d, a, batch_stats);
        if (training && a->bwd_arena && a->bwd_arena_words > 0) hd.zero_fill = a->bwd_arena, hd.zero_fill_words = a->bwd_arena_words;
        SN2_TRY(sn2_head_forward(&hd, cur));
    }
    if (join_b) NET_HIP(hipStreamWaitEvent(cur, ctx->b_done, 0));
    if (join_c) NET_HIP(hipStreamWaitEvent(cur, ctx->c_done, 0));
    return 0;
}

extern "C" int sn2_net_backward(const sn2_net_model* m, const sn2_net_dims* d, const sn2_net_geo* g, const sn2_net_act* a,
                                const sn2_net_bwd* b, void* stream) {
    SN2_TRY(check_dims(m, d));
    SN2_TRY(check_model_ptrs(m));
    if (!a || !b) return SN2_EINVAL;
    SN2_TRY(check_geo(d, g));
    if (!g->inv1 || !g->inv2 || !g->inv3) return SN2_EINVAL;
    if (!a->aux || !a->stats || !a->h1 || !a->h2 || !a->h3 || !a->h_sa3 || !a->x3 || !a->arg3) return SN2_EINVAL;
    if (!b->arena || b->images != GRAD_IMAGES || b->image_stride < m->n_flat || !b->dy1 || !b->du1 || !b->du2 || !b->du3 || !b->bn_ok ||
        !b->dy2 || !b->dy3 || !b->dx1 || !b->dx2 || !b->dx3 || !b->dy_sa3 || b->arena_words <= 0)
        return SN2_EINVAL;
    const int B = d->B, M2 = d->M2;
    if (b->loss && (b->dcov || b->dproba || b->loss->B != d->B || b->loss->N != d->N ||
                    !sn2_head_loss_route(b->loss->B, b->loss->N, b->loss->D)))
        return SN2_EINVAL;
    hipStream_t cur = (hipStream_t)stream;
    if (!b->arena_is_zero) {
        sn2_fill_words(b->arena, 0u, (size_t)b->arena_words, cur);
        NET_HIP(hipGetLastError());
    }
    const GradDst gd{b->arena, b->image_stride, b->frozen_stats ? 1 : 0};
    sn2_head hd;
    head_desc(&hd, m, d, a, b->frozen_stats ? 0 : 1);
    hd.coverages = hd.proba = nullptr;
    hd.dcoverages = b->dcov, hd.dproba = b->dproba, hd.dy = static_cast<float*>(b->dy1);
    hd.loss = b->loss;
    hd.dW1 = b->arena + m->g_lin1_W, hd.db1 = b->arena + m->g_lin1_b, hd.dW2 = b->arena + m->g_lin2_W, hd.db2 = b->arena + m->g_lin2_b;
    hd.grad_replicas = GRAD_IMAGES, hd.grad_replica_stride = b->image_stride;
    SN2_TRY(sn2_head_backward(&hd, cur));
    SN2_TRY(sn2_head_bn_sums(&hd, m->fp1.gamma, m->fp1.beta, aux_row(a, 6, 2), aux_row(a, 6, 3), b->arena + m->fp1.ggamma,
                             b->arena + m->fp1.gbeta, b->bn_ok + 0, cur));
    sn2_fp p1;
    fp_desc(&p1, d, a, fp1_in(m, d, g, a, b->src_ws1), gd);
    p1.dy = static_cast<const float*>(b->dy1), p1.dsrc = b->dy2, p1.dsrc_stride = 36, p1.dskip = nullptr, p1.dskip_stride = 0;
    p1.du_scratch = static_cast<float*>(b->du1), p1.scatter_ws = g->inv1, p1.scatter_ready = 1, p1.bn_sums_done = b->bn_ok + 0;
    p1.row_perm = (g->rank1 && p1.src_ws) ? g->rank1 : nullptr;
    SN2_TRY(sn2_fp_backward(&p1, cur));
    SN2_TRY(sn2_fp_bn_sums(&p1, m->fp2.gamma, m->fp2.beta, aux_row(a, 5, 2), aux_row(a, 5, 3), b->arena + m->fp2.ggamma,
                           b->arena + m->fp2.gbeta, b->bn_ok + 1, cur));
    sn2_fp p2;
    fp_desc(&p2, d, a, fp2_in(m, d, g, a, b->src_ws2), gd);
    p2.dy = b->dy2, p2.dsrc = b->dy3, p2.dsrc_stride = 64, p2.dskip = b->dx1, p2.dskip_stride = 16;
    p2.du_scratch = b->du2, p2.scatter_ws = g->inv2, p2.scatter_ready = 1, p2.bn_sums_done = b->bn_ok + 1;
    SN2_TRY(sn2_fp_backward(&p2, cur));
    sn2_fp pf3, p3;
    fp_desc(&pf3, d, a, fp3_in(m, d, g, a), gd);
    pf3.dy = b->dy3, pf3.dsrc = b->dx3, pf3.dsrc_stride = 64, pf3.dskip = b->dx2, pf3.dskip_stride = 32;
    fp_desc(&p3, d, a, sa3_in(m, d, g, a), gd);
    p3.dsrc = b->dx2, p3.dsrc_stride = 32;
    if (m->fuse_global_level && b->gl_xchg && b->gl_ctl && sn2_global_level_backward_route(B, M2, b->frozen_stats, gl_bf16(m))) {
        SN2_TRY(sn2_global_level_backward(&p3, &pf3, a->arg3, b->gl_xchg, b->gl_ctl, cur));
    } else {
        SN2_TRY(sn2_fp_bn_sums(&p2, m->fp3.gamma, m->fp3.beta, aux_row(a, 4, 2), aux_row(a, 4, 3), b->arena + m->fp3.ggamma,
                               b->arena + m->fp3.gbeta, b->bn_ok + 2, cur));
        pf3.du_scratch = b->du3, pf3.scatter_ws = g->inv3, pf3.scatter_ready = -1, pf3.bn_sums_done = b->bn_ok + 2;
        SN2_TRY(sn2_fp_backward(&pf3, cur));
        SN2_TRY(sn2_global_pool_backward(b->du3, 64, a->arg3, a->h_sa3, aux_row(a, 3, 2), aux_row(a, 3, 3), B, M2, 64, b->dx3,
                                         b->dy_sa3, b->arena + m->sa3.ggamma, b->arena + m->sa3.gbeta, cur));
        p3.dy = b->dy_sa3, p3.bn_sums_done = b->bn_ok + 3;
        SN2_TRY(sn2_fp_backward(&p3, cur));
    }
    sn2_sa sa;
    sa2_desc(&sa, m, d, g, a, gd, b->dx2, b->dx1);
    SN2_TRY(sn2_sa_backward(&sa, cur));
    sa1_desc(&sa, m, d, g, a, gd, b->dx1, b->sa1_ws);
    SN2_TRY(sn2_sa_backward(&sa, cur));
    if (b->defer_grad_reduce) return 0;
    return sn2_grad_reduce(b->arena, m->n_flat, GRAD_IMAGES, b->image_stride, cur);
}
```

stratanet2_vegetation_coverage_maps_amd/csrc/sa.hip:

```cpp
#include "mlp.h"

template <int CF, int NL, int C1, int C2, int PASS>
int sa_mfma_launch_fwd(const sn2_sa* p, int training, hipStream_t st, int* nblocks_out);
template <int CF, int NL, int C1, int C2, int PASS>
int sa_mfma_launch_bwd(const sn2_sa* p, float* ws, hipStream_t st);

namespace {


__global__ __launch_bounds__(256) void sa_bwd_prep_kernel(const float* __restrict__ dout, const float* __restrict__ ext,
                                                          const int* __restrict__ arg, const float* __restrict__ mean,
                                                          const float* __restrict__ invstd, int rows, int C,
                                                          float* __restrict__ dgamma, float* __restrict__ dbeta) {
    const int o = threadIdx.x % C, g = threadIdx.x / C, G = 256 / C;
    float sb = 0.f, sg = 0.f;
    const float mu = mean[o], is = invstd[o];
    const int step = gridDim.x * G;
    for (int r0 = blockIdx.x * G + g; g < G && r0 < rows; r0 += 8 * step) {
        int ar[8];
        float dv[8], ev[8];
#pragma unroll
        for (int u = 0; u < 8; ++u) {
            const int r = r0 + u * step;
            const size_t i = (size_t)(r < rows ? r : r0) * C + o;
            ar[u] = r < rows ? arg[i] : -1;
            dv[u] = dout[i];
            ev[u] = ext[i];
        }
#pragma unroll
        for (int u = 0; u < 8; ++u)
            if (ar[u] >= 0) {
                sb += dv[u];
                sg = fmaf(dv[u], (ev[u] - mu) * is, sg);
            }
    }
    __shared__ float s_red[128];
    for (int i = threadIdx.x; i < 2 * C; i += 256) s_red[i] = 0.f;
    __syncthreads();
    if (g < G) {
        atomicAdd(&s_red[o], sb);
        atomicAdd(&s_red[C + o], sg);
    }
    __syncthreads();
    if (threadIdx.x < 2 * C) {
        const float v = s_red[threadIdx.x];
        if (v != 0.f) atomicAdd(threadIdx.x < C ? &dbeta[threadIdx.x] : &dgamma[threadIdx.x - C], v);
    }
}

__global__ __launch_bounds__(256) void sa_bwd_combine_kernel(const float* __restrict__ ws, const float* __restrict__ dgamma,
                                                             const float* __restrict__ dbeta,
                                                             const unsigned long long* __restrict__ total, int C, int CIN,
                                                             float* __restrict__ dW, float* __restrict__ db) {
    const int n = C * (CIN + 1), i = threadIdx.x;
    if (i >= n) return;
    float part[2][SN2_SA_BWD_WS_REPLICAS];
#pragma unroll
    for (int r = 0; r < SN2_SA_BWD_WS_REPLICAS; ++r) {
        part[0][r] = ws[(size_t)r * 2 * n + i];
        part[1][r] = ws[(size_t)r * 2 * n + n + i];
    }
    const unsigned long long etot = *total;
    const float invE = etot > 0 ? (float)(1.0 / (double)etot) : 0.f;
    const int o = i / (CIN + 1), k = i - o * (CIN + 1);
    const float dg = dgamma[o] * invE, de = dbeta[o] * invE;
    float sx = 0.f, sm = 0.f;
#pragma unroll
    for (int r = 0; r < SN2_SA_BWD_WS_REPLICAS; ++r) sx += part[0][r], sm += part[1][r];
    const float v = -fmaf(dg, sx, de * sm);
    float* dst = k < CIN ? &dW[o * CIN + k] : &db[o];
    *dst += v;
}

int check(const sn2_sa* p) {
    if (!p || p->B <= 0 || p->Nsrc <= 0 || p->M <= 0 || p->cap <= 0) return SN2_EINVAL;
    if (!p->feat || !p->spos || !p->cpos || !p->nbr || !p->cnt || !p->total || !p->ext || !p->arg || !p->out)
        return SN2_EINVAL;
    if (p->feat_stride < p->cf || (p->feat_stride & 3) || p->spos_stride < 4 || (p->spos_stride & 3)) return SN2_EINVAL;
    const bool sa1 = p->cf == 8 && p->nl == 2 && p->blk[0].cin == 11 && p->blk[0].cout == 16 && p->blk[1].cin == 16 &&
                     p->blk[1].cout == 16;
    const bool sa2 = p->cf == 16 && p->nl == 1 && p->blk[0].cin == 19 && p->blk[0].cout == 32;
    const bool sa3 = p->cf == 32 && p->nl == 1 && p->blk[0].cin == 35 && p->blk[0].cout == 64;
    return (sa1 || sa2 || sa3) ? 0 : SN2_ELIMIT;
}

template <int CF, int NL, int C1, int C2>
int forward_t(const sn2_sa* p, int training, hipStream_t st) {
    const sn2_block* last = &p->blk[NL - 1];
    int nb = 0;
    const int batch_stats = training == 1;
    if constexpr (NL == 2) {
        if (batch_stats) SN2_TRY((sa_mfma_launch_fwd<CF, NL, C1, C2, 0>(p, training, st, &nb)));
        SN2_TRY(sn2_bn_finalize(&p->blk[0], nb, p->total, 0, batch_stats, st));
    }
    if (!training) {
        SN2_TRY(sn2_bn_finalize(last, 0, p->total, 0, 0, st));
        return sa_mfma_launch_fwd<CF, NL, C1, C2, 1>(p, 0, st, &nb);
    }
    SN2_TRY((sa_mfma_launch_fwd<CF, NL, C1, C2, 1>(p, training, st, &nb)));
    return sn2_bn_finalize_apply(last, batch_stats ? nb : 0, p->total, 0, batch_stats, p->ext, p->arg, p->out, (long)p->B * p->M, st);
}

template <int CF, int NL, int C1, int C2>
int backward_t(const sn2_sa* p, hipStream_t st) {
    const sn2_block* last = &p->blk[NL - 1];
    const int rows = p->B * p->M, C = last->cout;
    int pb = sn2_cdiv(rows, 256 / C);
    if (pb > 256) pb = 256;
    hipLaunchKernelGGL(sa_bwd_prep_kernel, dim3(pb), dim3(256), 0, st, p->dout, p->ext, p->arg, last->mean, last->invstd,
                       rows, C, last->dgamma, last->dbeta);
    if constexpr (NL == 2) {
        const sn2_block* k0 = &p->blk[0];
        if (!p->dfeat && p->bwd_ws && !k0->mma_bf16) {
            SN2_TRY((sa_mfma_launch_bwd<CF, NL, C1, C2, 2>(p, p->bwd_ws, st)));
            if (k0->frozen_stats || last->frozen_stats) return 0;
            static_assert(C1 * (CF + 4) <= 256, "one thread per element of [dW0 | db0]");
            hipLaunchKernelGGL(sa_bwd_combine_kernel, dim3(1), dim3((C1 * (CF + 4) + 63) / 64 * 64), 0, st, p->bwd_ws, k0->dgamma,
                               k0->dbeta, p->total, C1, CF + 3, k0->dW, k0->db);
            SN2_RETURN_LAUNCH();
        }
        SN2_TRY((sa_mfma_launch_bwd<CF, NL, C1, C2, 2>(p, nullptr, st)));
    }
    SN2_TRY((sa_mfma_launch_bwd<CF, NL, C1, C2, 3>(p, nullptr, st)));
    return 0;
}

}

namespace {
__global__ __launch_bounds__(1024) void sa_order_sort_kernel(const int* __restrict__ cnt, int B, int M, int P2,
                                                             int* __restrict__ order_all, size_t stride) {
    extern __shared__ __attribute__((aligned(16))) unsigned s_key[];
    __shared__ int s_n[3];
    const int bg = blockIdx.x, tid = threadIdx.x, NT = (int)blockDim.x;
    const int hb = bg / B, b = bg - hb * B;
    int* __restrict__ order = order_all + (size_t)hb * stride;
    const int* cb = cnt + (size_t)bg * M;
    if (tid < 3) s_n[tid] = 0;
    __syncthreads();
    int n_here[3] = {0, 0, 0};
    for (int i = tid; i < P2; i += NT) {
        unsigned key = 0xFFFFFFFFu;
        if (i < M) {
            const int c = cb[i];
            key = ((unsigned)(0x3FFFF - c) << 14) | (unsigned)i;
            n_here[0] += c > SN2_SA_SOLO_MIN ? 1 : 0;
            n_here[1] += (c > SN2_SA_QUAD_MIN && c <= SN2_SA_SOLO_MIN) ? 1 : 0;
            n_here[2] += (c > SN2_SA_OCT_MIN && c <= SN2_SA_QUAD_MIN) ? 1 : 0;
        }
        s_key[i] = key;
    }
#pragma unroll
    for (int k = 0; k < 3; ++k)
        if (n_here[k]) atomicAdd(&s_n[k], n_here[k]);
    __syncthreads();
    for (int k = 2; k <= P2; k <<= 1) {
        for (int j = k >> 1; j > 0; j >>= 1) {
            for (int t = tid; t < (P2 >> 1); t += NT) {
                const int lo = ((t & ~(j - 1)) << 1) | (t & (j - 1)), hi = lo | j;
                const unsigned a = s_key[lo], c = s_key[hi];
                const bool up = (lo & k) == 0;
                if ((a > c) == up) {
                    s_key[lo] = c;
                    s_key[hi] = a;
                }
            }
            __syncthreads();
        }
    }
    const int nsolo = s_n[0], r_oct = nsolo + s_n[1], r_hex = r_oct + s_n[2];
    const int items_a = nsolo + ((s_n[1] + 3) >> 2), n_oct_items = (s_n[2] + 7) >> 3, n_hex_items = (M - r_hex + 15) >> 4;
    int* packed = order + (size_t)4 * B * M;
    for (int r = tid; r < M; r += NT) {
        const int id = b * M + (int)(s_key[r] & 0x3FFFu);
        if (r < nsolo) {
            int* dst = order + 4 * ((size_t)r * B + b);
            dst[0] = dst[1] = dst[2] = dst[3] = id | SN2_SA_SOLO_FLAG;
        } else if (r < r_oct) {
            const int rl = r - nsolo;
            order[4 * ((size_t)(nsolo + (rl >> 2)) * B + b) + (rl & 3)] = id;
        } else if (r < r_hex) {
            const int rl = r - r_oct;
            int* dst = packed + 16 * ((size_t)(rl >> 3) * B + b) + 2 * (rl & 7);
            dst[0] = dst[1] = id | SN2_SA_OCT_FLAG;
        } else {
            const int rl = r - r_hex;
            packed[16 * ((size_t)(n_oct_items + (rl >> 4)) * B + b) + (rl & 15)] = id;
        }
    }
    if (tid == 0) {
        int* trailer = packed + (size_t)16 * B * SN2_SA_PACKED_ITEMS(M);
        atomicMax(&trailer[0], items_a);
        atomicMax(&trailer[1], n_oct_items + n_hex_items);
    }
}
}

static int sa_order_impl(const int* cnt, int G, int B, int M, int* order, size_t stride, hipStream_t st);
extern "C" size_t sn2_sa_order_words(int B, int M) { return SN2_SA_ORDER_WORDS(B, M); }

extern "C" int sn2_sa_order(const int* cnt, int B, int M, int* order, void* stream) {
    if (!cnt || !order || B <= 0 || M <= 0) return SN2_EINVAL;
    return sa_order_impl(cnt, 1, B, M, order, SN2_SA_ORDER_WORDS(B, M), (hipStream_t)stream);
}
extern "C" int sn2_sa_order_group(const int* cnt, int G, int B, int M, int* order, size_t stride_words, void* stream) {
    if (!cnt || !order || G <= 0 || B <= 0 || M <= 0 || stride_words < SN2_SA_ORDER_WORDS(B, M)) return SN2_EINVAL;
    return sa_order_impl(cnt, G, B, M, order, stride_words, (hipStream_t)stream);
}
static int sa_order_impl(const int* cnt, int G, int B, int M, int* order, size_t stride, hipStream_t st) {
    if (M > 16384) return SN2_ELIMIT;
    sn2_fill_words(order, 0xFFFFFFFFu, (size_t)(G - 1) * stride + (size_t)SN2_SA_ORDER_WORDS(B, M), st);
    int P2 = 2;
    while (P2 < M) P2 <<= 1;
    if ((size_t)P2 * 4 > 48 * 1024)
        (void)hipFuncSetAttribute(reinterpret_cast<const void*>(&sa_order_sort_kernel),
                                  hipFuncAttributeMaxDynamicSharedMemorySize, P2 * 4);
    hipLaunchKernelGGL(sa_order_sort_kernel, dim3(G * B), dim3(sn2_small_sort_wg(B) ? 256 : 1024), (size_t)P2 * 4, st, cnt, B, M, P2,
                       order, stride);
    SN2_RETURN_LAUNCH();
}

extern "C" int sn2_sa_forward(const sn2_sa* p, int training, void* stream) {
    SN2_TRY(check(p));
    if (training < 0 || training > SN2_BN_FROZEN_KEEP) return SN2_EINVAL;
    if (p->nl == 2) return forward_t<8, 2, 16, 16>(p, training, (hipStream_t)stream);
    if (p->cf == 32) return forward_t<32, 1, 64, 64>(p, training, (hipStream_t)stream);
    return forward_t<16, 1, 32, 32>(p, training, (hipStream_t)stream);
}

extern "C" int sn2_sa_backward(const sn2_sa* p, void* stream) {
    SN2_TRY(check(p));
    if (!p->dout) return SN2_EINVAL;
    if (p->nl == 2) return backward_t<8, 2, 16, 16>(p, (hipStream_t)stream);
    if (p->cf == 32) return backward_t<32, 1, 64, 64>(p, (hipStream_t)stream);
    return backward_t<16, 1, 32, 32>(p, (hipStream_t)stream);
}
```

stratanet2_vegetation_coverage_maps_amd/executor.py:

```python
import ctypes
import weakref
from ctypes import byref

import torch

from . import _lib
from . import hip_ops as ops
from ._lib import NetAct, NetBwd, NetDims, NetGeo, NetIO, NetModel, StrataHipError

F32, I32, I64, BF16, U8 = torch.float32, torch.int32, torch.int64, torch.bfloat16, torch.uint8
_FAKE_BASE = 1 << 40
_ITEM = {F32: 4, I32: 4, I64: 8, BF16: 2, U8: 1}


def _geo_shapes(B, N, M1, M2, cap1, cap2):
    return {
        "idx1": (I32, (B, M1)), "pos1_soa": (F32, (B, 3, M1)), "pos1_aos": (F32, (B * M1, 4)), "ws1": (I32, (ops.fps_ws_words(B, N),)),
        "nbr1": (I32, (B * M1, cap1)), "cnt1": (I32, (B * M1,)), "tot1": (I64, (1,)), "ord1": (I32, (ops.sa_order_len(B, M1),)),
        "idx2": (I32, (B, M2)), "pos2_soa": (F32, (B, 3, M2)), "pos2_aos": (F32, (B * M2, 4)), "ws2": (I32, (ops.fps_ws_words(B, M1),)),
        "nbr2": (I32, (B * M2, cap2)), "cnt2": (I32, (B * M2,)), "tot2": (I64, (1,)), "ord2": (I32, (ops.sa_order_len(B, M2),)),
        "knn3_idx": (I32, (B * M2, 3)), "knn3_w": (F32, (B * M2, 3)), "knn2_idx": (I32, (B * M1, 3)), "knn2_w": (F32, (B * M1, 3)),
        "knn1_idx": (I32, (B * N, 3)), "knn1_w": (F32, (B * N, 3)),
        "inv3": (F32, (ops.interp_ws_words(B, M2, 1),)), "inv2": (F32, (ops.interp_ws_words(B, M1, M2),)),
        "inv1": (F32, (ops.interp_ws_words(B, N, M1),)),
# ... 70 lines not shown
        if len(_ZEROS) > 16:
            _ZEROS.clear()
        z = _ZEROS[key] = torch.zeros(B, 3, 1, dtype=F32, device=dev)
    return z


class ArenaGeometry:

    def __init__(self, plan, dev, model):
        self.plan = plan
        self.B, self.N, self.M1, self.M2 = plan.B, plan.N, plan.M1, plan.M2
        self.arena = torch.empty(plan.geo_bytes, dtype=U8, device=dev)
        self.pos3 = _pos3(dev, plan.B)
        self.fps_live1 = torch.empty(plan.B, dtype=I32, device=dev)
        self.xyz = None
        self.has_rows0, self.has_inverted = False, False
        self.ready, self._join = None, None
        self.p2_diam_pix = None
        g = NetGeo()
        base = self.arena.data_ptr()
        for name, (off, _, _) in plan.geo_offsets.items():
            setattr(g, name, base + off)
        g.pos3 = self.pos3.data_ptr()
        self._want_rank1 = bool(model.fp1_morton_rows and "ws1" in plan.geo_offsets and model._fp1_source_side(plan.B * plan.N))
        if self._want_rank1:
            g.rank1 = self.rank1.data_ptr()
        self.cgeo = g

    _PAIRS = {"knn3": ("knn3_idx", "knn3_w"), "knn2": ("knn2_idx", "knn2_w"), "knn1": ("knn1_idx", "knn1_w")}

    def __getattr__(self, name):
        d = self.__dict__
        plan = d.get("plan")
        if plan is None:
            raise AttributeError(name)
        spec = plan.geo_offsets.get(name)
        if spec is not None:
            v = _view(d["arena"], *spec)
        elif name in self._PAIRS:
            v = tuple(getattr(self, n) for n in self._PAIRS[name])
        elif name == "nn_ws":
            v = tuple(getattr(self, n) if n in plan.geo_offsets else None for n in ("nn_ws2", "nn_ws1"))
        elif name == "rank1":
            v = ops.fps_ws_rank(self.ws1, self.B, self.N) if d.get("_want_rank1") else None
        elif name in ("ws1", "ws2", "nn_ws1", "nn_ws2", "p2_pix", "p2_mm"):
            v = None
        else:
            raise AttributeError(name)
        d[name] = v
        return v


def geo_struct(g):
    cg = getattr(g, "cgeo", None)
    if cg is not None:
        return cg
    cg = NetGeo()
    p = lambda t: None if t is None else t.data_ptr()
    for n in ("idx1", "pos1_soa", "pos1_aos", "nbr1", "cnt1", "tot1", "ord1", "idx2", "pos2_soa", "pos2_aos", "nbr2", "cnt2", "tot2",
              "ord2", "inv3", "inv2", "inv1", "rows0"):
        setattr(cg, n, p(getattr(g, n)))
    for n in ("ws1", "ws2", "rank1", "p2_pix", "p2_mm"):
        setattr(cg, n, p(getattr(g, n, None)))
    nn_ws = getattr(g, "nn_ws", None) or (None, None)
    cg.nn_ws2, cg.nn_ws1 = p(nn_ws[0]), p(nn_ws[1])
    for k in ("knn3", "knn2", "knn1"):
        idx, w = getattr(g, k)
        setattr(cg, k + "_idx", idx.data_ptr())
        setattr(cg, k + "_w", w.data_ptr())
    pos3 = getattr(g, "pos3", None)
    if pos3 is None:
        pos3 = g.pos3 = _pos3(g.idx1.device, g.B)
    cg.pos3 = pos3.data_ptr()
    g.cgeo = cg
    return cg


def _check_handle(g, plan, what):
    d = plan.dims
    ok = (g.B, g.N, g.M1, g.M2) == (d.B, d.N, d.M1, d.M2)
    if ok:
        gp = getattr(g, "plan", None)
        if gp is not None:
            ok = gp is plan or (gp.dims.cap1, gp.dims.cap2, gp.geo_bytes) == (d.cap1, d.cap2, plan.geo_bytes) or \
                (gp.dims.cap1, gp.dims.cap2) == (d.cap1, d.cap2) and gp.dims.p2_diam_pix >= d.p2_diam_pix
        else:
            ok = g.nbr1.shape[1] == d.cap1 and g.nbr2.shape[1] == d.cap2
    if not ok:
        raise ValueError(f"{what} do not match this batch")


class NetSaved:

    def __init__(self, plan, geo, arena, cact, training):
        self.plan, self.geo, self.arena, self.cact, self.training = plan, geo, arena, cact, training
        self.B, self.N, self.M1, self.M2 = plan.B, plan.N, plan.M1, plan.M2

    def __getattr__(self, name):
        d = self.__dict__
        plan = d.get("plan")
        if plan is None:
            raise AttributeError(name)
        spec = plan.act_offsets[1 if d["training"] else 0].get(name)
        if spec is not None:
            v = d[name] = _view(d["arena"], *spec)
            return v
        return getattr(d["geo"], name)


_BLOCKS = ("sa1_module.conv.local_nn.0", "sa1_module.conv.local_nn.1", "sa2_module.conv.local_nn.0", "sa3_module.nn.0",
           "fp3_module.nn.0", "fp2_module.nn.0", "fp1_module.nn.0")


class ModelStruct:

    def __init__(self, model, params, max_neighbors):
        offs, n_flat = ops.flat_layout(params)
        off_of = {id(p): o for p, o in zip(params, offs)}
        self.param_offsets, self.n_flat = offs, n_flat
        self.param_shapes = [tuple(p.shape) for p in params]
        self.param_numels = [p.numel() for p in params]
        m = NetModel()
        mods = dict(model.named_modules())
        layers = [m.sa1[0], m.sa1[1], m.sa2, m.sa3, m.fp3, m.fp2, m.fp1]
        self.tensors = []
        for L, name in zip(layers, _BLOCKS):
            blk = mods[name]
            lin, bn = blk[0], blk[2]
            prefix = name.rsplit(".", 1)[0]
            for t in (lin.weight, lin.bias, bn.weight, bn.bias, bn.running_mean, bn.running_var):
                ops._chk(t, F32, None, name)
            L.cin, L.cout = lin.in_features, lin.out_features
            L.W, L.b, L.gamma, L.beta = lin.weight.data_ptr(), lin.bias.data_ptr(), bn.weight.data_ptr(), bn.bias.data_ptr()
            L.running_mean, L.running_var = bn.running_mean.data_ptr(), bn.running_var.data_ptr()
            nbt = bn.num_batches_tracked
            if nbt is not None:
                ops._chk(nbt, I64, None, "num_batches_tracked")
            L.num_batches_tracked = None if nbt is None else nbt.data_ptr()
            L.gW, L.gb, L.ggamma, L.gbeta = (off_of[id(t)] for t in (lin.weight, lin.bias, bn.weight, bn.bias))
            L.mma_bf16 = int(model.mma_dtype == "bf16" and prefix in model.BF16_BLOCKS)
            self.tensors += [lin.weight, lin.bias, bn.weight, bn.bias, bn.running_mean, bn.running_var] + ([nbt] if nbt is not None else [])
        for t, shape in ((model.lin1.weight, (16, 34)), (model.lin1.bias, (16,)), (model.lin2.weight, (5, 16)), (model.lin2.bias, (5,))):
            ops._chk(t, F32, shape, "head parameter")
        m.lin1_W, m.lin1_b, m.lin2_W, m.lin2_b = (t.data_ptr() for t in (model.lin1.weight, model.lin1.bias, model.lin2.weight, model.lin2.bias))
        m.g_lin1_W, m.g_lin1_b, m.g_lin2_W, m.g_lin2_b = (off_of[id(t)] for t in (model.lin1.weight, model.lin1.bias, model.lin2.weight,
                                                                                model.lin2.bias))
        self.tensors += [model.lin1.weight, model.lin1.bias, model.lin2.weight, model.lin2.bias]
        m.n_flat = n_flat
        m.r1_sq, m.r2_sq = ops.r2_threshold(model.sa1_module.r), ops.r2_threshold(model.sa2_module.r)
        m.max_neighbors = int(max_neighbors)
        m.drop_p = float(model.drop)
        m.fuse_global_level, m.fuse_eval_head, m.source_side = int(bool(model.fuse_global_level)), int(bool(model.fuse_eval_head)), int(bool(ops.SOURCE_SIDE))
        m.fps_waves_shared, m.fps_waves_many = int(model.fps_waves_shared), int(model.fps_waves_many)
        self.c = m
        self.settings = settings_of(model, max_neighbors)
        self.key = tuple(t.data_ptr() for t in self.tensors)
        self.plans = {}
        dev = model.lin1.weight.device
        if any(t.device != dev for t in self.tensors):
            raise StrataHipError("PointNet2: parameters and buffers must live on one HIP device")

    def current(self, model, max_neighbors):
        return self.settings == settings_of(model, max_neighbors) and self.key == tuple(t.data_ptr() for t in self.tensors)

    def plan(self, model, B, N):
        k = (B, N)
        p = self.plans.get(k)
        if p is None:
            if len(self.plans) > 32:
                self.plans.clear()
            p = self.plans[k] = Plan(model, self.c, B, N, self.c.max_neighbors)
        return p


def settings_of(model, max_neighbors):
    return (model.mma_dtype, float(model.drop), bool(model.fuse_global_level), bool(model.fuse_eval_head), bool(ops.SOURCE_SIDE),
            int(model.fps_waves_shared), int(model.fps_waves_many), float(model.sa1_module.r), float(model.sa2_module.r),
            float(model.sa1_module.ratio), float(model.sa2_module.ratio), int(max_neighbors), model.p2_diam_pix,
            bool(model.fp1_morton_rows))


class NetCtx:

    def __init__(self):
        h = ctypes.c_void_p()
        _lib.check(_lib.load().sn2_net_ctx_create(byref(h)), "sn2_net_ctx_create")
        self.handle = h.value
        self._fin = weakref.finalize(self, _destroy_ctx, self.handle)


def _destroy_ctx(handle):
    try:
        _lib.load().sn2_net_ctx_destroy(handle)
    except Exception:
        pass


def _io(model, dev, training, flags, cloud=None, fps_start=None, fork=False, n_live=None, geo=None):
    io = NetIO()
    if n_live is not None:
        io.fps_live, io.fps_live1 = n_live.data_ptr(), geo.fps_live1.data_ptr()
    io.cloud = None if cloud is None else cloud.data_ptr()
    io.fps_start = None if fps_start is None else fps_start.data_ptr()
    io.fps_status = ops.fps_status_word(dev).data_ptr()
    io.training = int(training) if training in (0, 1, 2) else int(bool(training))
    if fork:
        io.stream_b = ops.shared_stream(dev, "fork_b").cuda_stream
        io.stream_c = ops.shared_stream(dev, "fork_c").cuda_stream
        io.stream_pack = ops.shared_stream(dev, "pack").cuda_stream
        io.ctx = model._net_ctx().handle
    io.flags = flags
    return io


def geometry(model, ms, xyz, fps_start, out=None, fork=None, shared=False, defer_join=False, inverted=True, cloud=None, n_live=None):
    dev = xyz.device
    B, _, N = xyz.shape
    ops._chk(xyz, F32, (B, 3, N), "xyz")
    ops._chk(fps_start, I32, (2, B), "fps_start")
    if n_live is not None:
        ops._chk(n_live, I32, (B,), "n_live")
    plan = ms.plan(model, B, N)
    g = out if out is not None else ArenaGeometry(plan, dev, model)
    _check_handle(g, plan, "geometry buffers")
    cg = geo_struct(g)
    g.xyz = xyz
    cg.xyz = xyz.data_ptr()
    fork = model.geometry_fork if fork is None else fork
    flags = (_lib.NET_FORK if fork else 0) | (_lib.NET_SHARED if shared else 0) | (_lib.NET_INVERTED if inverted else 0)
    if fork and defer_join:
        flags |= _lib.NET_DEFER_JOIN
    if cloud is not None:
        ops._chk(cloud, F32, (B, 10, N), "cloud")
        flags |= _lib.NET_INPUT_ONLY
    io = _io(model, dev, model.training, flags, cloud=cloud, fps_start=fps_start, fork=fork, n_live=n_live, geo=g)
    _lib.check(_lib.load().sn2_net_geometry(byref(ms.c), byref(plan.dims), byref(cg), byref(io), ops._stream()), "sn2_net_geometry")
    g.has_inverted = bool(inverted)
    g.has_rows0 = cloud is not None
    if cloud is not None and plan.dims.p2_diam_pix > 0 and getattr(g, "p2_pix", None) is not None:
        g.p2_diam_pix = int(plan.dims.p2_diam_pix)
    g._join = "ctx" if (fork and defer_join) else None
    return g


def forward(model, ms, xyz, cloud, fps_start, training, geo=None, drop_keep=None, need_grad=True, n_live=None):
    dev = xyz.device
    B, _, N = xyz.shape
    ops._chk(xyz, F32, (B, 3, N), "xyz")
    ops._chk(cloud, F32, (B, 10, N), "cloud")
    plan = ms.plan(model, B, N)
    lib = _lib.load()
    fork = False
    frozen = (not training) and bool(need_grad)
    keep = bool(training) or frozen
    mode = 1 if training else (_lib.BN_FROZEN_KEEP if frozen else 0)
    if geo is None:
        ops._chk(fps_start, I32, (2, B), "fps_start")
        geo = ArenaGeometry(plan, dev, model)
        fork = bool(model.geometry_fork)
        flags = _lib.NET_WITH_GEOMETRY | (_lib.NET_FORK if fork else 0)
        geo.has_inverted = keep
        fs = fps_start
        if n_live is not None:
            ops._chk(n_live, I32, (B,), "n_live")
    else:
        _check_handle(geo, plan, "prefetched geometry tables")
        flags, fs, n_live = 0, None, None
        if getattr(geo, "has_rows0", False):
            flags |= _lib.NET_HAS_ROWS0
        if getattr(geo, "_join", None) is not None:
            flags |= _lib.NET_JOIN_PENDING
            geo._join = None
            fork = True
        if getattr(geo, "has_inverted", True):
            flags |= _lib.NET_HAS_INVERTED
    cg = geo_struct(geo)
    geo.xyz = xyz
    cg.xyz = xyz.data_ptr()
    t = 1 if keep else 0
    arena = torch.empty(plan.act_bytes[t], dtype=U8, device=dev)
    ca = NetAct()
    base = arena.data_ptr()
    for name, (off, _, _) in plan.act_offsets[t].items():
        setattr(ca, name, base + off)
    cov = torch.empty(B * N, 4, dtype=F32, device=dev)
    proba = torch.empty(B * N, 4, dtype=F32, device=dev)
    ca.cov, ca.proba = cov.data_ptr(), proba.data_ptr()
    if drop_keep is not None:
        ops._chk(drop_keep, I32, (B * N,), "drop_mask")
        ca.drop_mask = drop_keep.data_ptr()
    bwd_arena = None
    if keep and need_grad:
        bwd_arena = torch.empty(plan.bwd_arena_words, dtype=F32, device=dev)
        ca.bwd_arena, ca.bwd_arena_words = bwd_arena.data_ptr(), plan.bwd_arena_words
    io = _io(model, dev, mode, flags, cloud=cloud, fps_start=fs, fork=fork, n_live=n_live, geo=geo)
    if training and model.fuse_global_level and plan.gl_forward:
        ws = ops.global_level_ws(dev, owner=model)
        io.gl_xchg, io.gl_ctl = ws[0].data_ptr(), ws[1].data_ptr()
    _lib.check(lib.sn2_net_forward(byref(ms.c), byref(plan.dims), byref(cg), byref(ca), byref(io), ops._stream()), "sn2_net_forward")
    geo.has_rows0 = True
    if keep:
        geo.has_inverted = True
    s = NetSaved(plan, geo, arena, ca, keep)
    s.frozen = frozen
    s.drop_keep = drop_keep
    s.xyz = xyz
    s.ms = ms
    s.bwd_arena = bwd_arena
    return cov, proba, s


def backward(model, s, dcov, dproba, loss=None):
    plan, ms = s.plan, s.ms
    dev = s.xyz.device
    R = plan.B * plan.N
    arena = s.__dict__.get("bwd_arena")
    s.bwd_arena = None
    pre_zeroed = arena is not None
    if arena is None:
        arena = torch.empty(plan.bwd_arena_words, dtype=F32, device=dev)
    scratch = torch.empty(plan.bwd_scratch_bytes, dtype=U8, device=dev)
    cb = NetBwd()
    sz, sz2 = ctypes.c_size_t(), ctypes.c_size_t()
    lib = _lib.load()
    _lib.check(lib.sn2_net_bwd_carve(byref(ms.c), byref(plan.dims), arena.data_ptr(), scratch.data_ptr(), byref(cb), byref(sz), byref(sz2)),
               "sn2_net_bwd_carve")
    if dcov is not None:
        dcov = ops._chk(dcov.contiguous(), F32, (R, 4), "dcoverages")
        cb.dcov = dcov.data_ptr()
    if dproba is not None:
        dproba = ops._chk(dproba.contiguous(), F32, (R, 4), "dproba")
        cb.dproba = dproba.data_ptr()
# ... 19 lines not shown
```

stratanet2_vegetation_coverage_maps_amd/hip_ops.py:

```python
import ctypes
import math
from typing import Optional

import numpy as np
import torch

from . import _lib
from ._lib import FP, SA, Block, Head, LossGrad, StrataHipError, check

I32, F32, F64, I64, BF16 = torch.int32, torch.float32, torch.float64, torch.int64, torch.bfloat16


_timing = None


class timing:

    def __init__(self, names=None):
        self.names = None if names is None else set(names)
        self.events = []

    def __enter__(self):
        global _timing
        self._prev, _timing = _timing, self
# ... 575 lines not shown
    _call("sn2_plots_append", _ptr(src_raw), src_T, _ptr(src_offsets), _ptr(src_centers), _ptr(src_cov), _ptr(sel), K, _ptr(dst_raw),
          cap_T, _ptr(dst_offsets), _ptr(dst_centers), _ptr(dst_cov), cap_P, P0, T0, _ptr(dst_start), new_T, _stream())


def znorm(xyz: torch.Tensor, radius: float):
    _, n = xyz.shape
    _chk(xyz, F32, (3, n), "xyz")
    if not radius > 0:
        raise ValueError("znorm: radius must be positive")
    lo = xyz[:2].min(1).values.tolist()
    hi = xyz[:2].max(1).values.tolist()
    cells = (int((hi[0] - lo[0]) / radius) + 2) * (int((hi[1] - lo[1]) / radius) + 2)
    ws = torch.empty(_host("sn2_znorm_ws_words", n, cells), dtype=I32, device=xyz.device)
    zmin = torch.empty(n, dtype=F32, device=xyz.device)
    zout = torch.empty(n, dtype=F32, device=xyz.device)
    _call("sn2_znorm", _ptr(xyz[0]), _ptr(xyz[1]), _ptr(xyz[2]), n, float(radius), lo[0], lo[1], hi[0], hi[1], _ptr(ws),
          _ptr(zmin), _ptr(zout), _stream())
    return zmin, zout


def parcel_count_ws_words(P: int, rows: int) -> int:
    return int(_lib.load().sn2_parcel_count_ws_words(int(P), int(rows)))


def parcel_znorm_ws_words(T: int, radius: float, x_min: float, y_min: float, x_max: float, y_max: float) -> int:
    return int(_lib.load().sn2_parcel_znorm_ws_words(int(T), float(radius), float(x_min), float(y_min), float(x_max),
                                                     float(y_max)))


def _chk_center_grid(grid, P: int):
    start, items, GX, GY, gx0, gy0, inv = grid
    _chk(start, I32, (GX * GY + 1,), "cell_start")
    _chk(items, I32, None, "cell_items")
    if items.dim() != 1 or items.numel() < 1 or items.numel() > P:
        raise ValueError("cell_items: expected 1..P centre ids")
    return start, items, int(GX), int(GY), float(gx0), float(gy0), float(inv)


def parcel_count(cloud: torch.Tensor, centers: torch.Tensor, grid, radius: float, L: int, rows: int):
    _, T = cloud.shape
    _chk(cloud, F32, (10, T), "cloud")
    P = centers.shape[0]
    _chk(centers, F32, (P, 2), "centers")
    start, items, GX, GY, gx0, gy0, inv = _chk_center_grid(grid, P)
    dev = cloud.device
    nw = parcel_count_ws_words(P, rows)
    ws = torch.empty(nw + 4, dtype=I32, device=dev)
    prefix = torch.empty(P * rows + 1, dtype=I32, device=dev)
    total = torch.empty(1, dtype=I64, device=dev)
    _call("sn2_parcel_count", _ptr(cloud), T, int(L), int(rows), _ptr(centers), P, _ptr(start), _ptr(items), GX, GY, gx0, gy0,
          inv, float(radius), _ptr(ws), nw, _ptr(prefix), _ptr(total), _stream())
    return prefix, total


def parcel_fill(cloud: torch.Tensor, centers: torch.Tensor, grid, radius: float, L: int, rows: int, prefix: torch.Tensor,
                plot_base: torch.Tensor, sum_n: int):
    _, T = cloud.shape
    _chk(cloud, F32, (10, T), "cloud")
    P = centers.shape[0]
    _chk(centers, F32, (P, 2), "centers")
    start, items, GX, GY, gx0, gy0, inv = _chk_center_grid(grid, P)
    _chk(prefix, I32, (P * rows + 1,), "prefix")
    _chk(plot_base, I32, (P,), "plot_base")
    dev = cloud.device
    raw = torch.empty(10, sum_n, dtype=F32, device=dev)
    pidx = torch.empty(sum_n, dtype=I32, device=dev)
    _call("sn2_parcel_fill", _ptr(cloud), T, int(L), int(rows), _ptr(centers), P, _ptr(start), _ptr(items), GX, GY, gx0, gy0,
          inv, float(radius), _ptr(prefix), _ptr(plot_base), int(sum_n), _ptr(raw), _ptr(pidx), _stream())
    return raw, pidx


def parcel_znorm(cloud: torch.Tensor, bbox, radius: float, disc_radius: float, offsets: torch.Tensor, centers: torch.Tensor,
                 point_index: torch.Tensor, raw: torch.Tensor):
    _, T = cloud.shape
    _chk(cloud, F32, (10, T), "cloud")
    P = centers.shape[0]
    _chk(centers, F32, (P, 2), "centers")
    _chk(offsets, I32, (P + 1,), "offsets")
    sum_n = point_index.shape[0]
    _chk(point_index, I32, (sum_n,), "point_index")
    _chk(raw, F32, (10, sum_n), "raw")
    nw = parcel_znorm_ws_words(T, radius, *bbox)
    if nw == 0:
        raise ValueError("parcel_znorm: the parcel's extent needs more than 2^26 cells of the z-norm radius")
    ws = torch.empty(nw + 4, dtype=I32, device=cloud.device)
    _call("sn2_parcel_znorm", _ptr(cloud), T, *[float(v) for v in bbox], float(radius), float(disc_radius), _ptr(offsets),
          _ptr(centers), P, _ptr(point_index), sum_n, _ptr(ws), nw, _ptr(raw), _stream())
    return raw


def sa_order_len(B: int, M: int) -> int:
    return _host("sn2_sa_order_words", int(B), int(M))


def sa_order(cnt: torch.Tensor, B: int, M: int, out: Optional[torch.Tensor] = None) -> torch.Tensor:
    _chk(cnt, I32, (B * M,), "cnt")
    n = sa_order_len(B, M)
    if out is None:
        out = torch.empty(n, dtype=I32, device=cnt.device)
    else:
        _chk(out, I32, (n,), "out order")
    _call("sn2_sa_order", _ptr(cnt), B, M, _ptr(out), _stream())
    return out


def sa_order_group(cnt: torch.Tensor, G: int, B: int, M: int, out_all: torch.Tensor, stride: int):
    _chk(cnt, I32, (G * B * M,), "cnt")
    if stride < sa_order_len(B, M):
        raise ValueError("sa_order_group: stride smaller than a table")
    _chk(out_all, I32, (G * stride,), "out order tables")
    _call("sn2_sa_order_group", _ptr(cnt), G, B, M, _ptr(out_all), stride, _stream(), key="sn2_sa_order")


SA_BWD_WS_WORDS = _lib.SN2_SA_BWD_WS_WORDS


def sa_desc(blocks, feat, cf, spos, cpos_aos, nbr, cnt, total, B, Nsrc, M, ext, arg, out, dout=None, dfeat=None,
            with_grads=False, order=None, bwd_ws=None) -> SA:
    cap = nbr.shape[1]
    cl = blocks[-1].cout
    feat_stride = _chk_rows(feat, F32, B * Nsrc, cf, "feat")
    spos_stride = _chk_rows(spos, F32, B * Nsrc, 4, "spos")
    _chk(cpos_aos, F32, (B * M, 4), "cpos_aos")
    _chk(nbr, I32, (B * M, cap), "nbr")
    _chk(cnt, I32, (B * M,), "cnt")
    _chk(total, I64, (1,), "total")
    _chk(ext, F32, (B * M, cl), "ext")
    _chk(arg, I32, (B * M, cl), "arg")
    _chk(out, F32, (B * M, cl), "out")
    d = SA()
    d.B, d.Nsrc, d.M, d.cap, d.cf, d.nl = B, Nsrc, M, cap, cf, len(blocks)
    d.feat, d.feat_stride, d.spos, d.spos_stride = _ptr(feat), feat_stride, _ptr(spos), spos_stride
    d.cpos, d.nbr, d.cnt, d.total = _ptr(cpos_aos), _ptr(nbr), _ptr(cnt), _ptr(total)
    if order is not None:
        _chk(order, I32, (sa_order_len(B, M),), "order")
    d.order = _ptr(order)
    for i, bb in enumerate(blocks):
        bb.fill(d.blk[i], with_grads)
    d.ext, d.arg, d.out = _ptr(ext), _ptr(arg), _ptr(out)
    if dout is not None:
        _chk(dout, F32, (B * M, cl), "dout")
    if dfeat is not None:
        _chk(dfeat, F32, (B * Nsrc, cf), "dfeat")
    if bwd_ws is not None:
        _chk(bwd_ws, F32, (SA_BWD_WS_WORDS,), "bwd_ws")
    d.dout, d.dfeat, d.bwd_ws = _ptr(dout), _ptr(dfeat), _ptr(bwd_ws)
    return d


def sa_forward(d: SA, training: bool):
    _call("sn2_sa_forward", d, int(training), _stream(), tag=f"cf={d.cf}")


def sa_backward(d: SA):
    _call("sn2_sa_backward", d, _stream(), tag=f"cf={d.cf}")


def interp_ws_words(B: int, R_per_plot: int, S_per_plot: int) -> int:
    return _host("sn2_interp_ws_words", int(B), int(R_per_plot), int(S_per_plot))


def interp_chunks(R_per_plot: int, S_per_plot: int) -> int:
    return _host("sn2_interp_chunks", int(R_per_plot), int(S_per_plot))


def fp_src_ws_words(B: int, R_per_plot: int, S_per_plot: int, cout: int) -> int:
    return _host("sn2_fp_src_ws_words", int(B), int(R_per_plot), int(S_per_plot), int(cout))


def fp_rows_small(R: int) -> bool:
    return bool(_host("sn2_fp_rows_small", int(R)))


def fp_source_side(R: int, cb: int, force: bool = False) -> bool:
    return bool(_host("sn2_fp_source_side", int(R), int(cb), int(bool(force))))


def interp_index(knn, B: int, R_per_plot: int, S_per_plot: int, out: Optional[torch.Tensor] = None,
                 src_pos: Optional[torch.Tensor] = None, row_perm: Optional[torch.Tensor] = None) -> torch.Tensor:
    if src_pos is not None:
        _chk(src_pos, F32, (B * S_per_plot, 4), "src_pos")
    if row_perm is not None:
        _chk(row_perm, I32, (B * R_per_plot,), "row_perm")
    R = B * R_per_plot
    _chk(knn[0], I32, (R, 3), "knn_idx")
    _chk(knn[1], F32, (R, 3), "knn_w")
    n = interp_ws_words(B, R_per_plot, S_per_plot)
    if out is None:
        out = torch.empty(n, dtype=F32, device=knn[0].device)
    else:
        _chk(out, F32, (n,), "out index")
    _call("sn2_interp_index_perm", _ptr(knn[0]), _ptr(knn[1]), _ptr(src_pos), _ptr(row_perm), B, R_per_plot, S_per_plot, _ptr(out),
          _stream(), key="sn2_interp_index")
    return out


def interp_index_group(knn, G: int, B: int, R_per_plot: int, S_per_plot: int, out_all: torch.Tensor, stride: int,
                       src_pos: Optional[torch.Tensor] = None, row_perm: Optional[torch.Tensor] = None):
    R = G * B * R_per_plot
    _chk(knn[0], I32, (R, 3), "knn_idx")
    _chk(knn[1], F32, (R, 3), "knn_w")
    if src_pos is not None:
        _chk(src_pos, F32, (G * B * S_per_plot, 4), "src_pos")
    if row_perm is not None:
        _chk(row_perm, I32, (R,), "row_perm")
    if stride % 4 or stride < interp_ws_words(B, R_per_plot, S_per_plot):
        raise ValueError("interp_index_group: stride must be a multiple of 4 words and hold one index")
    _chk(out_all, F32, (G * stride,), "out indices")
    _call("sn2_interp_index_group", _ptr(knn[0]), _ptr(knn[1]), _ptr(src_pos), _ptr(row_perm), G, B, R_per_plot, S_per_plot, _ptr(out_all),
          stride, _stream(), key="sn2_interp_index")


SOURCE_SIDE = True


def fp_desc(block: BlockBuffers, B, R_per_plot, S_per_plot, ca, cb, src, h, src_affine=None, knn=None, skip=None,
            dy=None, dsrc=None, dskip=None, du_scratch=None, with_grads=False, interp_index=None,
            bn_sums_done=None, row_perm=None, force_src_ws=False, gather=True) -> FP:
    R = B * R_per_plot
    hs = (block.cout + 3) // 4 * 4
    AT = BF16 if (h is not None and h.dtype == BF16) else F32
    n_src_rows = R if knn is None else B * S_per_plot
    src_stride = _chk_rows(src, F32, n_src_rows, ca, "src")
    if src.shape[1] < (ca + 3) // 4 * 4 and src_stride < (ca + 3) // 4 * 4:
        raise ValueError("fp: src rows must be padded to a multiple of 4 floats")
    if h is not None or not force_src_ws:
        _chk(h, AT, (R, hs), "h")
    d = FP()
    d.B, d.R_per_plot, d.S_per_plot, d.ca, d.cb = B, R_per_plot, S_per_plot, ca, cb
    d.src, d.src_stride = _ptr(src), src_stride
    if src_affine is not None:
        _chk(src_affine[0], F32, (ca,), "src_a")
        _chk(src_affine[1], F32, (ca,), "src_c")
        d.src_a, d.src_c = _ptr(src_affine[0]), _ptr(src_affine[1])
    else:
        d.src_a = d.src_c = None
    if knn is not None:
        _chk(knn[0], I32, (R, 3), "knn_idx")
        _chk(knn[1], F32, (R, 3), "knn_w")
        d.knn_idx, d.knn_w = _ptr(knn[0]), _ptr(knn[1])
    else:
        d.knn_idx = d.knn_w = None
    if cb > 0:
        d.skip_stride = _chk_rows(skip, F32, R, cb, "skip", align=4 if cb % 4 == 0 else 1)
        d.skip = _ptr(skip)
    else:
        d.skip, d.skip_stride = None, 0
    block.fill(d.blk, with_grads)
    if not fp_rows_small(R):
        d.blk.mma_bf16 = 0
    d.h, d.h_stride = _ptr(h), hs
    if dy is not None:
        _chk(dy, AT, (R, hs), "dy")
    d.dsrc_stride = d.dskip_stride = 0
    if dsrc is not None:
        d.dsrc_stride = _chk_rows(dsrc, F32, n_src_rows, ca, "dsrc", align=1)
    if dskip is not None:
        d.dskip_stride = _chk_rows(dskip, F32, R, cb, "dskip", align=1)
    d.scatter_ws, d.scatter_ready = None, 0
    if bn_sums_done is not None:
        _chk(bn_sums_done, I32, (1,), "bn_sums_done")
    d.bn_sums_done = _ptr(bn_sums_done)
    d._src_ws = None
    if SOURCE_SIDE and knn is not None and fp_source_side(R, cb, force_src_ws):
        d._src_ws = torch.empty(fp_src_ws_words(B, R_per_plot, S_per_plot, block.cout), dtype=F32, device=src.device)
    d.src_ws = _ptr(d._src_ws)
    d.row_perm = None
    if row_perm is not None and d._src_ws is not None and du_scratch is not None:
        _chk(row_perm, I32, (R,), "row_perm")
        d.row_perm = _ptr(row_perm)
    d.act_bf16 = int(AT == BF16)
    if d.act_bf16 and d._src_ws is None:
        raise ValueError("fp: bfloat16 activation rows need the source-side form (hip_ops.fp_source_side)")
    if du_scratch is not None:
        _chk(du_scratch, AT, (R, max(ca, hs)), "du_scratch")
        if knn is not None and dsrc is not None:
            words = interp_ws_words(B, R_per_plot, S_per_plot)
            if interp_index is not None:
                _chk(interp_index, F32, (words,), "interp_index")
                d._scatter_ws, d.scatter_ready = interp_index, 1
            else:
                d._scatter_ws = torch.empty(words, dtype=F32, device=src.device)
            d.scatter_ws = _ptr(d._scatter_ws)
            if not gather:
                d.scatter_ready = -1
    d.dy, d.dsrc, d.dskip, d.du_scratch = _ptr(dy), _ptr(dsrc), _ptr(dskip), _ptr(du_scratch)
    return d


def fp_bn_sums(d: FP, gamma, beta, mean, invstd, dgamma, dbeta, ok):
    for t, n in ((gamma, "gamma"), (beta, "beta"), (mean, "mean"), (invstd, "invstd"), (dgamma, "dgamma"), (dbeta, "dbeta")):
        _chk(t, F32, (d.ca,), n)
    _chk(ok, I32, (1,), "ok")
    _call("sn2_fp_bn_sums", d, _ptr(gamma), _ptr(beta), _ptr(mean), _ptr(invstd), _ptr(dgamma), _ptr(dbeta), _ptr(ok), _stream())


def fp_forward(d: FP, training: bool):
    _call("sn2_fp_forward", d, int(training), _stream(), tag=f"{d.ca}+{d.cb}->{d.blk.cout}")


def fp_backward(d: FP):
    _call("sn2_fp_backward", d, _stream(), tag=f"{d.ca}+{d.cb}->{d.blk.cout}")


def plot_max_forward(h, a, c, B, R_per_plot, C):
    hs = (C + 3) // 4 * 4
    _chk(h, F32, (B * R_per_plot, hs), "h")
    _chk(a, F32, (C,), "a")
    _chk(c, F32, (C,), "c")
    out = torch.empty(B, C, dtype=F32, device=h.device)
    arg = torch.empty(B, C, dtype=I32, device=h.device)
    _call("sn2_plot_max_forward", _ptr(h), _ptr(a), _ptr(c), B, R_per_plot, C, _ptr(out), _ptr(arg), _stream())
    return out, arg


GL_MAX_PLOTS = _lib.SN2_GLOBAL_MAX_PLOTS
_GLOBAL_WS = {}
_GLOBAL_WS_ALL = []


class _GlobalWs(list):
    __slots__ = ("__weakref__",)


def global_level_ws(dev, B: int = GL_MAX_PLOTS, owner=None):
    dev = torch.device(dev)
    if B > GL_MAX_PLOTS:
        raise ValueError(f"global_level_forward takes at most {GL_MAX_PLOTS} plots")
    key = dev.index if dev.index is not None else torch.cuda.current_device()
    store = _GLOBAL_WS if owner is None else owner.__dict__.setdefault("_gl_ws", {})
    ws = store.get(key)
    if ws is None:
        if torch.cuda.is_current_stream_capturing():
            raise StrataHipError("global_level_forward: its exchange area must exist before a stream capture starts -- run one "
                                 "eager training forward first (TrainPipeline.capture does) or call hip_ops.global_level_ws(dev, owner=model)")
        ws = _GlobalWs([torch.zeros(_host("sn2_global_xchg_words", GL_MAX_PLOTS), dtype=I64, device=dev),
                        torch.zeros(_lib.SN2_GLOBAL_CTL_WORDS, dtype=I32, device=dev), 0,
                        torch.zeros(_lib.SN2_GLOBAL_BWD_XCHG_WORDS, dtype=I64, device=dev),
                        torch.zeros(_lib.SN2_GLOBAL_BWD_CTL_WORDS, dtype=I32, device=dev)])
        store[key] = ws
        import weakref
        _GLOBAL_WS_ALL[:] = [r for r in _GLOBAL_WS_ALL if r() is not None]
        _GLOBAL_WS_ALL.append(weakref.ref(ws))
    return ws


def global_level_forward_fused(B: int, *blocks) -> bool:
    return bool(_host("sn2_global_level_forward_route", int(B), int(any(b.mma_bf16 for b in blocks))))


def global_level_forward(d_sa3: FP, d_fp3: FP, x3: torch.Tensor, arg3: torch.Tensor, owner=None):
    B = d_sa3.B
    _chk(x3, F32, (B, 64), "x3")
    _chk(arg3, I32, (B, 64), "arg3")
    ws = global_level_ws(x3.device, B, owner=owner)
    _call("sn2_global_level_forward", d_sa3, d_fp3, _ptr(x3), _ptr(arg3), _ptr(ws[0]), _ptr(ws[1]), _stream())


GL_BWD_MAX_ROWS = _lib.SN2_GLOBAL_BWD_MAX_ROWS


def global_level_backward_fused(B: int, M2: int, frozen: bool, *blocks) -> bool:
    return bool(_host("sn2_global_level_backward_route", int(B), int(M2), int(bool(frozen)), int(any(b.mma_bf16 for b in blocks))))


def global_level_backward(d_sa3: FP, d_fp3: FP, arg3: torch.Tensor, owner=None):
    B = d_sa3.B
    _chk(arg3, I32, (B, 64), "arg3")
    ws = global_level_ws(arg3.device, B, owner=owner)
    _call("sn2_global_level_backward", d_sa3, d_fp3, _ptr(arg3), _ptr(ws[3]), _ptr(ws[4]), _stream())


def global_level_gave_up(dev, warn: bool = True) -> int:
    dev = torch.device(dev)
    key = dev.index if dev.index is not None else torch.cuda.current_device()
    total = 0
    for r in list(_GLOBAL_WS_ALL):
        ws = r()
        if ws is None or ws[1].device.index != key:
            continue
        n = int(ws[1][1].item()) + int(ws[4][1].item())
        total += n
        if n > ws[2]:
            seen, ws[2] = ws[2], n
            if warn:
                import warnings
                warnings.warn(f"global_level_forward / backward: {n - seen} exchange wait(s) gave up on {dev}; those launches were finished "
                              "by their last workgroup alone (results unaffected, the passes took longer); set "
                              "PointNet2.fuse_global_level = False where other kernels or processes share the device",
                              StrataHipWarning, stacklevel=2)
    return total


def plot_max_backward(dout, arg, B, R_per_plot, C, dy):
    hs = (C + 3) // 4 * 4
    _chk(dout, F32, (B, C), "dout")
    _chk(arg, I32, (B, C), "arg")
    _chk(dy, F32, (B * R_per_plot, hs), "dy")
    _call("sn2_plot_max_backward", _ptr(dout), _ptr(arg), B, R_per_plot, C, _ptr(dy), _stream())


def global_pool_backward(du, arg, h, mean, invstd, B, R_per_plot, dx, dy, dgamma, dbeta):
    _chk(du, F32, (B * R_per_plot, 64), "du")
    _chk(arg, I32, (B, 64), "arg")
    _chk(h, F32, (B * R_per_plot, 64), "h")
    for t, n in ((mean, "mean"), (invstd, "invstd"), (dgamma, "dgamma"), (dbeta, "dbeta")):
        _chk(t, F32, (64,), n)
    _chk(dx, F32, (B, 64), "dx")
    _chk(dy, F32, (B * R_per_plot, 64), "dy")
    _call("sn2_global_pool_backward", _ptr(du), 64, _ptr(arg), _ptr(h), _ptr(mean), _ptr(invstd), B, R_per_plot, 64, _ptr(dx), _ptr(dy),
          _ptr(dgamma), _ptr(dbeta), _stream())


def dropout_mask_words(keep: torch.Tensor) -> torch.Tensor:
    if keep.dim() != 2 or keep.shape[1] != 16:
        raise ValueError("dropout mask must be (rows, 16)")
    pow2 = (2 ** torch.arange(16, device=keep.device, dtype=torch.int32))
    return ((keep != 0).to(torch.int32) * pow2).sum(1, dtype=torch.int32).contiguous()


def head_loss_route(B: int, N: int, diam_pix: int) -> bool:
    return bool(_host("sn2_head_loss_route", int(B), int(N), int(diam_pix)))


def loss_grad_desc(pred, gt, proba, pdf, grad_total, arg, nocc, pix, B: int, N: int, diam_pix: int, m: float, e: float) -> LossGrad:
    R, D = B * N, int(diam_pix)
    _chk(pred, F32, (B, 4), "pred")
    _chk(gt, F64, (B, 4), "gt")
    _chk(proba, F32, (R, 4), "proba")
    if pdf is not None:
        _chk(pdf, F64, (R, 3), "pdf")
    _chk(grad_total, F64, None, "grad_total")
    _chk(arg, I32, (B * D * D * 3,), "arg")
    _chk(nocc, I32, (B,), "nocc")
    _chk(pix, I32, (R,), "pix")
    if grad_total.numel() != 1:
        raise ValueError("loss_grad_desc: grad_total is ONE fp64 scalar on the device")
    g = LossGrad()
    g.pred, g.gt, g.proba, g.pdf, g.grad_total = _ptr(pred), _ptr(gt), _ptr(proba), _ptr(pdf), _ptr(grad_total)
    g.arg, g.nocc, g.pix = _ptr(arg), _ptr(nocc), _ptr(pix)
    g.B, g.N, g.D, g.m, g.e = int(B), int(N), D, float(m), float(e)
    g.tensors = (pred, gt, proba, pdf, grad_total, arg, nocc, pix)
    return g


def head_desc(f, fa, fc, lin1, lin2, coverages=None, proba=None, dcov=None, dproba=None, dy=None, grads=None,
              grad_images=(1, 0), drop_mask=None, drop_p: float = 0.0, rows: Optional[int] = None, loss: Optional[LossGrad] = None) -> Head:
    if f is None:
        if rows is None or coverages is None:
            raise ValueError("head_desc: without f the row count and the outputs must be given")
        R, AT = int(rows), F32
    else:
        R = f.shape[0]
        AT = BF16 if f.dtype == BF16 else F32
        _chk(f, AT, (R, 36), "f")
    _chk(fa, F32, (34,), "fa")
    _chk(fc, F32, (34,), "fc")
    _chk(lin1.weight, F32, (16, 34), "lin1.weight")
    _chk(lin1.bias, F32, (16,), "lin1.bias")
    _chk(lin2.weight, F32, (5, 16), "lin2.weight")
    _chk(lin2.bias, F32, (5,), "lin2.bias")
    d = Head()
    d.R, d.cin, d.f_stride = R, 34, 36
    d.f, d.fa, d.fc = _ptr(f), _ptr(fa), _ptr(fc)
    d.W1, d.b1, d.W2, d.b2 = _ptr(lin1.weight), _ptr(lin1.bias), _ptr(lin2.weight), _ptr(lin2.bias)
    for t, n in ((coverages, "coverages"), (proba, "proba"), (dcov, "dcoverages"), (dproba, "dproba")):
        if t is not None:
            _chk(t, F32, (R, 4), n)
    d.coverages, d.proba, d.dcoverages, d.dproba = _ptr(coverages), _ptr(proba), _ptr(dcov), _ptr(dproba)
    if dy is not None:
        _chk(dy, AT, (R, 36), "dy")
    d.dy = _ptr(dy)
    d.act_bf16 = int(AT == BF16)
    if grads is not None:
        for t, ref in zip(grads, (lin1.weight, lin1.bias, lin2.weight, lin2.bias)):
            _chk(t, F32, ref.shape, "head grad view")
        d.dW1, d.db1, d.dW2, d.db2 = (_ptr(t) for t in grads)
        d.grad_replicas, d.grad_replica_stride = grad_images
    else:
        d.dW1 = d.db1 = d.dW2 = d.db2 = None
        d.grad_replicas, d.grad_replica_stride = 1, 0
    if drop_mask is not None:
        _chk(drop_mask, I32, (R,), "drop_mask")
        d.drop_mask, d.drop_scale = _ptr(drop_mask), (1.0 / (1.0 - drop_p) if drop_p < 1.0 else 0.0)
    else:
        d.drop_mask, d.drop_scale = None, 1.0
    if loss is not None:
        if dcov is not None or dproba is not None:
            raise ValueError("head_desc: a loss-gradient descriptor takes the place of dcov and dproba")
        d.loss = ctypes.pointer(loss)
        d._loss = loss
    return d


GRAD_IMAGES = _lib.SN2_NET_GRAD_IMAGES


def flat_layout(params):
    offs, o = [], 0
    for p in params:
        offs.append(o)
        o += p.numel()
    return offs, o


def grad_images_alloc(n_flat: int, device, extra_words: int = 0):
    stride = (n_flat + 63) // 64 * 64
    arena = torch.zeros(GRAD_IMAGES * stride + extra_words, dtype=F32, device=device)
# ... 388 lines not shown
```

stratanet2_vegetation_coverage_maps_amd/point_net2.py:

```python
import os
from collections import OrderedDict

import torch
import torch.nn as nn
from torch.nn import BatchNorm1d as BN
from torch.nn import Linear as Lin
from torch.nn import ReLU
from torch.nn import Sequential as Seq

from . import executor as X
from . import hip_ops as ops
from ._lib import BN_FROZEN_KEEP, MAX_NEIGHBORS as _MAXN, STAT_SLOTS, StrataHipError

MAX_NEIGHBORS = _MAXN

F32, I32, I64, F64 = torch.float32, torch.int32, torch.int64, torch.float64


def MLP(channels):
    return Seq(*[Seq(Lin(channels[i - 1], channels[i]), ReLU(), BN(channels[i])) for i in range(1, len(channels))])


class PointConv(nn.Module):

    def __init__(self, local_nn):
        super().__init__()
        self.local_nn = local_nn


class SAModule(nn.Module):
    def __init__(self, ratio, r, nn_):
        super().__init__()
        self.ratio, self.r = ratio, r
        self.conv = PointConv(nn_)


class GlobalSAModule(nn.Module):
    def __init__(self, nn_):
        super().__init__()
        self.nn = nn_


class FPModule(nn.Module):
    def __init__(self, k, nn_):
        super().__init__()
        self.k = k
        self.nn = nn_


def _at(o, stem, l, tail=""):
    return getattr(o, f"{stem}{l}{tail}")


def _put(o, stem, l, value, tail=""):
    setattr(o, f"{stem}{l}{tail}", value)


def _pad4(c):
    return (c + 3) // 4 * 4


class _Saved:
    pass


def _blocks_of(seq, aux_arena, stats_arena, cursor, mma_bf16=False):
    out = []
    for blk in seq:
        lin, bn = blk[0], blk[2]
        c = lin.out_features
        aux = aux_arena[cursor[0]:cursor[0] + 4 * c].view(4, c)
        ns = STAT_SLOTS * 2 * c
        st = stats_arena[cursor[1]:cursor[1] + ns]
        cursor[0] += 4 * c
        cursor[1] += ns
        out.append(ops.BlockBuffers(lin, bn, aux, st))
        out[-1].mma_bf16 = mma_bf16
    return out


class _PointNet2Fn(torch.autograd.Function):

    @staticmethod
    def forward(ctx, model, xyz, cloud, fps_start, geo, drop_keep, *params):
        training = model.training
        need_grad = bool(getattr(model, "_grad_mode_at_call", True)) and any(ctx.needs_input_grad[6:])
        n_live = model.__dict__.pop("_n_live_at_call", None)
        cov, proba, saved = model._forward_impl(xyz, cloud, fps_start, training, geo, drop_keep, need_grad=need_grad,
                                                **({} if n_live is None else {"n_live": n_live}))
        ctx.model = model
        if not isinstance(saved, X.NetSaved):
            saved.training = training
        ctx.saved = saved if need_grad else None
        ctx.n_params = len(params)
        return cov, proba

    @staticmethod
    def backward(ctx, dcov, dproba):
        if ctx.saved is None:
            raise RuntimeError("PointNet2: backward through a forward that recorded no graph")
        pending = ctx.__dict__.pop("loss_grad", None)
        loss = None
        if pending is not None:
            if pending.is_placeholder(dcov) and pending.is_placeholder(dproba):
                loss, dcov, dproba = pending.desc(), None, None
            else:
                gc, gp = pending.materialize()
                dcov = gc if (dcov is None or pending.is_placeholder(dcov)) else dcov + gc
                dproba = gp if (dproba is None or pending.is_placeholder(dproba)) else dproba + gp
        grads = ctx.model._backward_impl(ctx.saved, dcov, dproba) if loss is None else ctx.model._backward_impl(ctx.saved, None, None, loss=loss)
        ctx.saved = None
        return (None, None, None, None, None, None) + tuple(grads)


class PointNet2(nn.Module):
    def __init__(self, args):
        super().__init__()
        self._init_fields(args)
        ndim = 3
        mlp1 = [self.n_input_feats + ndim, 16, 16]
        mlp2 = [mlp1[-1] + ndim, 32]
        mlp3 = [mlp2[-1] + ndim, 64]
        self.sa1_module = SAModule(args.ratio1, args.r1, MLP(mlp1))
        self.sa2_module = SAModule(args.ratio2, args.r2, MLP(mlp2))
        self.sa3_module = GlobalSAModule(MLP(mlp3))
        mlp3_fp = [mlp3[-1] + mlp2[-1], 64]
        mlp2_fp = [mlp3_fp[-1] + mlp1[-1], 34]
        mlp1_fp = [mlp2_fp[-1] + self.n_input_feats, 34]
        self.fp3_module = FPModule(1, MLP(mlp3_fp))
        self.fp2_module = FPModule(3, MLP(mlp2_fp))
        self.fp1_module = FPModule(3, MLP(mlp1_fp))
        self.lin1 = nn.Linear(mlp1_fp[-1], 16)
        self.lin2 = nn.Linear(16, self.n_class + 1)
        self.lin2.bias = nn.Parameter(torch.tensor([0.733, 0.266, 0.235, 0.358, 0.500]))
        self.softmax = nn.Softmax(dim=1)
        self.sigmoid = nn.Sigmoid()
        if self.cuda_device is not None:
            self.cuda(self.cuda_device)

    def _init_fields(self, args):
        self.cuda_device = args.cuda
        self.subsample_size = args.subsample_size
        self.n_class = args.n_class
        self.drop = args.drop
        self.n_input_feats = args.n_input_feats - 2
        self.set_patience_attributes(args)
        self.log_embeddings = args.log_embeddings
        self.last_G_tensor = None
        self._last_flat_grad = None
        self._last_cloud_dev = None
        self.set_mma_dtype(getattr(args, "mma_dtype", "fp32"))
        if self.n_class != 4 or self.n_input_feats != 8:
            raise ValueError("the HIP kernels cover the reference architecture: n_class=4, 10 input features")

    BF16_BLOCKS = ("sa1_module.conv.local_nn", "sa2_module.conv.local_nn", "sa3_module.nn", "fp3_module.nn", "fp2_module.nn")
    mma_dtype = "fp32"
    fps_waves_shared = int(os.environ.get("SN2_FPS_WAVES_SHARED", "8"))
    fps_waves_many = int(os.environ.get("SN2_FPS_WAVES_MANY", "4"))
    geometry_fork = True
    executor = os.environ.get("SN2_EXECUTOR", "1") == "1"
    defer_grad_reduce = False
    _grad_images_pending = None
    geometry_pair_takes_group_cloud = True
    fuse_eval_head = os.environ.get("SN2_FUSE_EVAL_HEAD", "1") == "1"
    fuse_global_level = os.environ.get("SN2_FUSE_GLOBAL_LEVEL", "1") == "1"
    fuse_loss_backward = os.environ.get("SN2_FUSE_LOSS_BACKWARD", "1") == "1"
    p2_diam_pix = None

    def set_mma_dtype(self, dtype: str):
        if dtype not in ("fp32", "bf16"):
            raise ValueError("mma_dtype must be 'fp32' or 'bf16'")
        self.mma_dtype = dtype
        return self

    def forward(self, cloud_data):
        cloud, xyz = cloud_data["cloud"], cloud_data["xyz"]
        dev = self.lin1.weight.device
        if dev.type != "cuda":
            raise StrataHipError("PointNet2.forward needs a HIP device (args.cuda): the product path has no CPU "
                                 "fallback; the CPU restatement lives in oracle/ and is test infrastructure")
        if cloud.dim() != 3 or cloud.shape[1] != self.n_input_feats + 2 or xyz.shape != (cloud.shape[0], 3, cloud.shape[2]):
            raise ValueError(f"expected cloud (B,{self.n_input_feats + 2},N) and xyz (B,3,N), got "
                             f"{tuple(cloud.shape)} and {tuple(xyz.shape)}")
        with torch.cuda.device(dev):
            geo = cloud_data.get("geometry", None) if isinstance(cloud_data, dict) else None
            if geo is None and not cloud.is_cuda and not xyz.is_cuda and self.host_upload_overlap:
                return self._forward_from_host(cloud_data, cloud, dev)
            cloud_d = cloud.to(device=dev, dtype=F32, non_blocking=True).contiguous()
            if geo is not None:
                if getattr(geo, "ready", None) is not None:
                    cs = torch.cuda.current_stream()
                    cs.wait_event(geo.ready)
                    for v in geo.__dict__.values():
                        for t in (v if isinstance(v, tuple) else (v,)):
                            if isinstance(t, torch.Tensor):
                                t.record_stream(cs)
                xyz_d, fs = geo.xyz, None
            else:
                xyz_d, fs = self._stage_positions(cloud_data, dev)
                self._n_live_at_call = self._stage_live(cloud_data, dev, xyz_d.shape[0])
            self._last_cloud_dev = (cloud, cloud_d)
            params = self._params()
            self._grad_mode_at_call = torch.is_grad_enabled()
            cov, proba = _PointNet2Fn.apply(self, xyz_d, cloud_d, fs, geo, self._dropout_keep(cloud_data, cloud_d), *params)
        return cov, proba

    host_upload_overlap = os.environ.get("SN2_HOST_UPLOAD_OVERLAP", "1") == "1"

    def _forward_from_host(self, cloud_data, cloud, dev):
        ring = ops.pinned_ring(dev)
        cur = torch.cuda.current_stream(dev)
        cloud_d = torch.empty(cloud.shape, dtype=F32, device=dev)
        start = torch.cuda.Event()
        start.record(cur)
        xyz_d, fs = self._stage_positions(cloud_data, dev, ring=ring)
        g = self._geometry(xyz_d, fs, defer_join=True, inverted=self.training or torch.is_grad_enabled(),
                           **self._live_kw(self._stage_live(cloud_data, dev, xyz_d.shape[0])))
        up = ops.shared_stream(dev, "upload")
        up.wait_event(start)
        ring.upload(cloud, stream=up, dtype=F32, out=cloud_d, consumer=cur)
        self._last_cloud_dev = (cloud, cloud_d)
        from .project_to_2d import remember_upload
        remember_upload(cloud, cloud_d)
        params = self._params()
        self._grad_mode_at_call = torch.is_grad_enabled()
        return _PointNet2Fn.apply(self, xyz_d, cloud_d, None, g, self._dropout_keep(cloud_data, cloud_d), *params)

    def _params(self):
        c = self.__dict__.get("_leafs")
        if c is not None:
            mods = self._modules
            ok = all(mods.get(k) is v for k, v in c[0]) and all(m._parameters.get(n) is p for m, n, p in c[1]) and \
                all(m._buffers.get(n) is b for m, n, b in c[2])
            if ok:
                return self.__dict__["_param_list"]
        self.invalidate_caches()
        ps = list(self.parameters())
        leaf_p, leaf_b = [], []
        for mod in self.modules():
            leaf_p += [(mod, n, p) for n, p in mod._parameters.items() if p is not None]
            leaf_b += [(mod, n, b) for n, b in mod._buffers.items() if b is not None]
        self.__dict__["_param_list"] = ps
        self.__dict__["_leafs"] = (tuple(self._modules.items()), leaf_p, leaf_b)
        return ps

    def invalidate_caches(self):
        for k in ("_param_list", "_leafs", "_net_ms"):
            self.__dict__.pop(k, None)

    def _apply(self, fn, *a, **kw):
        self.invalidate_caches()
        return super()._apply(fn, *a, **kw)

    def load_state_dict(self, *a, **kw):
        self.invalidate_caches()
        return super().load_state_dict(*a, **kw)

    def _use_executor(self):
        return bool(self.executor) and ops._timing is None

    def _net_model(self):
        params = self._params()
        ms = self.__dict__.get("_net_ms")
        if ms is None or not ms.current(self, MAX_NEIGHBORS):
            ms = self.__dict__["_net_ms"] = X.ModelStruct(self, params, MAX_NEIGHBORS)
        return ms

    def _net_ctx(self):
        c = self.__dict__.get("_net_ctx_obj")
        if c is None:
            c = self.__dict__["_net_ctx_obj"] = X.NetCtx()
        return c

    def _dropout_keep(self, cloud_data, cloud_d):
        if not (self.training and self.drop > 0):
            return None
        R = cloud_d.shape[0] * cloud_d.shape[2]
        keep = cloud_data.get("dropout_mask", None) if isinstance(cloud_data, dict) else None
        if keep is None:
            keep = torch.empty(R, 16, dtype=F32, device=cloud_d.device).bernoulli_(max(0.0, 1.0 - float(self.drop)))
        else:
            keep = torch.as_tensor(keep).to(device=cloud_d.device)
            if tuple(keep.shape) != (R, 16):
                raise ValueError(f"dropout_mask must have shape ({R},16)")
        return ops.dropout_mask_words(keep)

    fp1_morton_rows = os.environ.get("SN2_FP1_MORTON_ROWS", "0") == "1"

    @staticmethod
    def _fp1_source_side(rows):
        return bool(ops.SOURCE_SIDE) and ops.fp_source_side(rows, 8)

    def _act_dtype(self, rows):
        return torch.bfloat16 if (self.mma_dtype == "bf16" and self._fp1_source_side(rows)) else F32

    @property
    def sa_levels(self):
        return tuple(m for m in self._modules.values() if isinstance(m, SAModule))

    @property
    def global_sa(self):
        return next(m for m in self._modules.values() if isinstance(m, GlobalSAModule))

    @property
    def fp_levels(self):
        return tuple(m for m in self._modules.values() if isinstance(m, FPModule))

    def _fp_by_level(self):
        fps = self.fp_levels
        return dict(zip(range(len(fps), 0, -1), fps))

    def _block_seqs(self):
        sa = [(f"sa{l}_module.conv.local_nn", m.conv.local_nn) for l, m in enumerate(self.sa_levels, 1)]
        fp = self._fp_by_level()
        return sa + [(f"sa{len(sa) + 1}_module.nn", self.global_sa.nn)] + [(f"fp{j}_module.nn", m.nn) for j, m in fp.items()]

    def _sizes(self, N):
        out = []
        for m in self.sa_levels:
# ... 196 lines not shown
        pos, sa, fp = self._positions(gp, xyz2, L), self.sa_levels, self._fp_by_level()
        live = n_live2
        for l in range(1, L + 1):
            live = self._fps_level(gp, pos, l, Ms[l], fps_start2[l - 1], live, waves=self.fps_waves_shared if l == 1 else 0)
            self._ball_level(gp, pos, l, sa[l - 1].r, False)
        for j in range(L + 1, 0, -1):
            self._nn_table(gp, pos, j, fp[j].k)
        grp = gp._grp
        tot_flat = grp.totals.view(-1)
        for l in range(1, L + 1):
            ops.count_sum_group(_at(gp, "cnt", l), G, B * Ms[l], tot_flat[l - 1:], L)
        for l in range(1, L + 1):
            ops.sa_order_group(_at(gp, "cnt", l), G, B, Ms[l], grp.ord[l], grp.so[l])
        rank = gp.rank1 if halves[0].rank1 is not None else None
        for j in range(L + 1, 0, -1):
            kw = {"src_pos": gp.pos1_aos, "row_perm": rank} if j == 1 else {}
            ops.interp_index_group(_at(gp, "knn", j), G, B, Ms[j - 1], Ms[j] if j <= L else 1, grp.inv[j], grp.si[j], **kw)
        if cloud2 is not None:
            self._input_only(gp, cloud2, xyz2)
        for h, g in enumerate(halves):
            g.xyz = xyz2[h * B:(h + 1) * B]
            g.has_rows0 = cloud2 is not None
            g.p2_diam_pix = gp.p2_diam_pix if cloud2 is not None else None
            g.has_inverted = True
            if clouds is not None and cloud2 is None:
                self._input_only(g, clouds[h], g.xyz)
        return halves

    def prefetch_geometry(self, cloud_data, lane: int = 0):
        dev = self.lin1.weight.device
        if dev.type != "cuda":
            raise StrataHipError("prefetch_geometry needs a HIP device")
        with torch.cuda.device(dev):
            xyz_d, fs = self._stage_positions(cloud_data, dev)
            side = ops.shared_stream(dev, f"side{lane}")
            side.wait_stream(torch.cuda.current_stream())
            xyz_d.record_stream(side)
            fs.record_stream(side)
            nl = self._stage_live(cloud_data, dev, xyz_d.shape[0])
            if nl is not None:
                nl.record_stream(side)
            with torch.cuda.stream(side):
                cl = cloud_data.get("cloud", None) if isinstance(cloud_data, dict) else None
                cl = cl if (isinstance(cl, torch.Tensor) and cl.is_cuda and cl.dtype == F32 and cl.is_contiguous()) else None
                g = self._geometry(xyz_d, fs, shared=True, fork=False, inverted=self.training, cloud=cl, **self._live_kw(nl))
                g.fps_start = fs
                g.ready = torch.cuda.Event()
                g.ready.record(side)
            g.stream = side
        return g

    def _stage_positions(self, cloud_data, dev, ring=None):
        xyz = cloud_data["xyz"]
        if ring is not None and not xyz.is_cuda:
            xyz_d = ring.upload(xyz, dtype=F32)
        else:
            xyz_d = xyz.to(device=dev, dtype=F32, non_blocking=True).contiguous()
        B, _, N = xyz_d.shape
        Ms = self._level_sizes(N)
        L = len(Ms) - 1
        fs = cloud_data.get("fps_start", None) if isinstance(cloud_data, dict) else None
        if fs is None:
            fs = torch.stack([torch.randint(0, S, (B,)) for S in Ms[:L]])
        fs = torch.as_tensor(fs).to(device=dev, dtype=I32, non_blocking=True).contiguous()
        if fs.shape != (L, B):
            raise ValueError(f"fps_start must have shape ({L},{B})")
        return xyz_d, fs

    def _stage_live(self, cloud_data, dev, B):
        nl = cloud_data.get("n_live", None) if isinstance(cloud_data, dict) else None
        if nl is None or not self.geometry_takes_n_live:
            return None
        nl = torch.as_tensor(nl).to(device=dev, dtype=I32, non_blocking=True).contiguous()
        if nl.shape != (B,):
            raise ValueError(f"n_live must have shape ({B},)")
        return nl

    @staticmethod
    def _live_kw(n_live):
        return {} if n_live is None else {"n_live": n_live}

    def _forward_impl(self, xyz, cloud, fps_start, training, geo=None, drop_keep=None, need_grad=True, n_live=None):
        if self._use_executor():
            cov, proba, s = X.forward(self, self._net_model(), xyz, cloud, fps_start, training, geo, drop_keep, need_grad=need_grad,
                                      n_live=n_live)
            if self.log_embeddings:
                self.last_G_tensor = s.x3
            return cov, proba, s
        dev = xyz.device
        B, _, N = xyz.shape
        Ms = self._level_sizes(N)
        L = len(Ms) - 1
        G = L + 1
        cur_stream = torch.cuda.current_stream(dev)
        frozen = (not training) and bool(need_grad)
        keep = bool(training) or frozen
        mode = 1 if training else (BN_FROZEN_KEEP if frozen else 0)
        rows0, packed = None, None
        if geo is not None and getattr(geo, "has_rows0", False) and geo.rows0.shape[0] == B * N:
            rows0 = geo.rows0
        if geo is None:
            if self.geometry_fork:
                rows0 = torch.empty(B * N, 12, dtype=F32, device=dev)
                pack_stream = ops.shared_stream(dev, "pack")
                pack_stream.wait_stream(cur_stream)
                with torch.cuda.stream(pack_stream):
                    ops.pack_rows(cloud, xyz, out=rows0)
                    packed = torch.cuda.Event()
                    packed.record(pack_stream)
            geo = self._geometry(xyz, fps_start, defer_join=True, inverted=keep, n_live=n_live)
        elif self._dims(geo, L) != (B, *Ms):
            raise ValueError("prefetched geometry does not match this batch")
        join = getattr(geo, "_join", None)
        geo._join = None
        if join == "ctx":
            raise StrataHipError("a geometry pass launched by the executor with a deferred join must be consumed by the executor")
        if keep and not getattr(geo, "has_inverted", True):
            if join is not None:
                cur_stream.wait_stream(join[0])
                cur_stream.wait_stream(join[1])
                join = None
            for l in range(1, L + 1):
                ops.count_sum(_at(geo, "cnt", l), _at(geo, "tot", l))
            for j in range(G, 0, -1):
                self._inverted_table(geo, Ms, j)
            geo.has_inverted = True
        s = _Saved()
        s.__dict__.update({k: v for k, v in geo.__dict__.items()
                           if k not in ("ready", "stream", "totals", "nn_ws", "fps_start", "_join", "has_rows0")
                           and not k.startswith(("ws", "fps_live"))})
        s.xyz = xyz
        seqs = self._block_seqs()
        width = sum(blk[0].out_features for _, seq in seqs for blk in seq)
        aux = torch.empty(4 * width, dtype=F32, device=dev)
        stats = torch.empty(STAT_SLOTS * 2 * width, dtype=F32, device=dev)
        cur = [0, 0]
        blocks = [_blocks_of(seq, aux, stats, cur, self.mma_dtype == "bf16" and prefix in self.BF16_BLOCKS) for prefix, seq in seqs]
        s.b_sa = dict(enumerate(blocks[:L], 1))
        s.b_glob = blocks[L][0]
        s.b_fp = dict(zip(range(G, 0, -1), (b[0] for b in blocks[G:])))
        s.blocks = [bb for b in blocks for bb in b]
        s.aux, s.stats = aux, stats
        for bb in s.blocks:
            bb.frozen = frozen
        e = lambda *shape, dt=F32: torch.empty(*shape, dtype=dt, device=dev)

        if packed is not None:
            cur_stream.wait_event(packed)
            s.rows0 = rows0
        elif rows0 is not None:
            s.rows0 = rows0
        else:
            s.rows0 = ops.pack_rows(cloud, xyz)
        for l in range(1, L + 1):
            R, C = B * Ms[l], s.b_sa[l][-1].cout
            _put(s, "ext", l, e(R, C))
            _put(s, "arg", l, e(R, C, dt=I32))
            _put(s, "x", l, e(R, C))
            ops.sa_forward(self._sa_desc(s, l), mode)
            if l == 1 and join is not None:
                cur_stream.wait_stream(join[0])
        R, C = B * Ms[L], s.b_glob.cout
        _put(s, "h_sa", G, e(R, _pad4(C)))
        _put(s, "h", G, e(R, _pad4(s.b_fp[G].cout)))
        if training and self.fuse_global_level and ops.global_level_forward_fused(B, s.b_glob, s.b_fp[G]):
            _put(s, "x", G, e(B, C))
            _put(s, "arg", G, e(B, C, dt=I32))
            ops.global_level_forward(self._global_sa_desc(s), self._fp_desc(s, G), _at(s, "x", G), _at(s, "arg", G), owner=self)
        else:
            ops.fp_forward(self._global_sa_desc(s), mode)
            x, arg = ops.plot_max_forward(_at(s, "h_sa", G), s.b_glob.a, s.b_glob.c, B, Ms[L], C)
            _put(s, "x", G, x)
            _put(s, "arg", G, arg)
            ops.fp_forward(self._fp_desc(s, G), mode)
        if self.log_embeddings:
            self.last_G_tensor = _at(s, "x", G)
        for j in range(L, 1, -1):
            _put(s, "h", j, e(B * Ms[j - 1], _pad4(s.b_fp[j].cout)))
            ops.fp_forward(self._fp_desc(s, j), mode)
        if join is not None:
            cur_stream.wait_stream(join[1])
        cov, proba = e(B * N, 4), e(B * N, 4)
        s.drop_keep = drop_keep
        b1 = s.b_fp[1]
        if not keep and self.fuse_eval_head and self._act_dtype(B * N) == F32 and ops.SOURCE_SIDE:
            s.h1 = None
            ops.fp_head_eval(self._fp_desc(s, 1, force_src_ws=True),
                             ops.head_desc(None, b1.a, b1.c, self.lin1, self.lin2, cov, proba, rows=B * N))
            return cov, proba, s
        s.h1 = torch.empty(B * N, _pad4(b1.cout), dtype=self._act_dtype(B * N), device=dev)
        ops.fp_forward(self._fp_desc(s, 1), mode)
        ops.head_forward(ops.head_desc(s.h1, b1.a, b1.c, self.lin1, self.lin2, cov, proba, drop_mask=drop_keep, drop_p=self.drop))
        return cov, proba, s

    def _sa_desc(self, s, l, dout=None, dfeat=None, g=False, bwd_ws=None):
        blocks = s.b_sa[l]
        cf = blocks[0].cin - 3
        if l == 1:
            feat, spos, S = s.rows0[:, 0:cf], s.rows0[:, cf:cf + 4], s.N
        else:
            feat, spos, S = _at(s, "x", l - 1), _at(s, "pos", l - 1, "_aos"), _at(s, "M", l - 1)
        return ops.sa_desc(blocks, feat, cf, spos, _at(s, "pos", l, "_aos"), _at(s, "nbr", l), _at(s, "cnt", l), _at(s, "tot", l), s.B, S,
                           _at(s, "M", l), _at(s, "ext", l), _at(s, "arg", l), _at(s, "x", l), dout=dout, dfeat=dfeat, with_grads=g,
                           order=getattr(s, f"ord{l}", None), bwd_ws=bwd_ws)

    def _global_sa_desc(self, s, **kw):
        L = len(s.b_sa)
        M = _at(s, "M", L)
        return ops.fp_desc(s.b_glob, s.B, M, M, s.b_glob.cin - 3, 3, _at(s, "x", L), _at(s, "h_sa", L + 1), skip=_at(s, "pos", L, "_aos"), **kw)

    def _fp_desc(self, s, j, **kw):
        L, blk = len(s.b_sa), s.b_fp[j]
        if j == L + 1:
            src, S, ca, affine = _at(s, "x", j), 1, s.b_glob.cout, None
        else:
            up = s.b_fp[j + 1]
            src, S, ca, affine = _at(s, "h", j + 1), _at(s, "M", j), up.cout, (up.a, up.c)
        if j == 1:
            R, skip = s.N, s.rows0[:, 0:blk.cin - ca]
            kw["row_perm"] = getattr(s, "rank1", None)
        else:
            R, skip = _at(s, "M", j - 1), _at(s, "x", j - 1)
        return ops.fp_desc(blk, s.B, R, S, ca, blk.cin - ca, src, _at(s, "h", j), src_affine=affine, knn=_at(s, "knn", j), skip=skip, **kw)

    def _backward_impl(self, s, dcov, dproba, loss=None):
        if isinstance(s, X.NetSaved):
            return X.backward(self, s, dcov, dproba, loss=loss)
        dev = s.xyz.device
        B, N, L = s.B, s.N, len(s.b_sa)
        G = L + 1
        Ms = [N] + [_at(s, "M", l) for l in range(1, G)]
        params = self._params()
        shapes = OrderedDict((f"dy{j}", (B * Ms[j - 1], _pad4(s.b_fp[j].cout))) for j in range(2, G + 1))
        shapes.update((f"dx{l}", (B * Ms[l], s.b_sa[l][-1].cout)) for l in range(1, G))
        shapes[f"dx{G}"] = (B, s.b_glob.cout)
        shapes[f"dy_sa{G}"] = (B * Ms[L], _pad4(s.b_glob.cout))
        sizes = OrderedDict((k, r * c) for k, (r, c) in shapes.items())
        sizes["sa1_ws"] = ops.SA_BWD_WS_WORDS
        flat, buf, views, images, arena = self._grad_arena(params, sizes, dev)
        dy = {j: buf[f"dy{j}"].view(shapes[f"dy{j}"]) for j in range(2, G + 1)}
        dx = {l: buf[f"dx{l}"].view(shapes[f"dx{l}"]) for l in range(1, G + 1)}
        for bb in s.blocks:
            bb.grads = (views[id(bb.lin.weight)], views[id(bb.lin.bias)], views[id(bb.bn.weight)], views[id(bb.bn.bias)])
            bb.grad_images = images
        dcov = None if dcov is None else dcov.contiguous()
        dproba = None if dproba is None else dproba.contiguous()
        e = lambda *shape, dt=F32: torch.empty(*shape, dtype=dt, device=dev)
        bn_ok = e(L + 2, dt=I32)

        def bn_sums(fn, d, blk, k):
            fn(d, blk.bn.weight.detach(), blk.bn.bias.detach(), blk.aux[2], blk.aux[3], views[id(blk.bn.weight)], views[id(blk.bn.bias)],
               bn_ok[k:k + 1])

        b1 = s.b_fp[1]
        dy[1] = e(B * N, _pad4(b1.cout), dt=s.h1.dtype)
        hg = (views[id(self.lin1.weight)], views[id(self.lin1.bias)], views[id(self.lin2.weight)], views[id(self.lin2.bias)])
        hd = ops.head_desc(s.h1, b1.a, b1.c, self.lin1, self.lin2, dcov=dcov, dproba=dproba, dy=dy[1], grads=hg,
                           grad_images=images, drop_mask=getattr(s, "drop_keep", None), drop_p=self.drop, loss=loss)
        ops.head_backward(hd)
        bn_sums(ops.head_bn_sums, hd, b1, 0)
        for j in range(1, G):
            blk, ca = s.b_fp[j], s.b_fp[j + 1].cout
            du = e(B * Ms[j - 1], max(ca, _pad4(blk.cout)), dt=dy[j].dtype)
            d = self._fp_desc(s, j, dy=dy[j], dsrc=dy[j + 1], du_scratch=du, with_grads=True, interp_index=_at(s, "inv", j),
                              bn_sums_done=bn_ok[j - 1:j], **({"dskip": dx[j - 1]} if j > 1 else {}))
            ops.fp_backward(d)
            if j < L:
                bn_sums(ops.fp_bn_sums, d, s.b_fp[j + 1], j)
        top, gb = s.b_fp[G], s.b_glob
        if self.fuse_global_level and ops.global_level_backward_fused(B, Ms[L], getattr(top, "frozen", False), gb, top):
            ops.global_level_backward(self._global_sa_desc(s, dsrc=dx[L], with_grads=True),
                                      self._fp_desc(s, G, dy=dy[G], dsrc=dx[G], dskip=dx[L], with_grads=True), _at(s, "arg", G), owner=self)
        else:
            bn_sums(ops.fp_bn_sums, d, top, L)
            du = e(B * Ms[L], max(gb.cout, _pad4(top.cout)))
            ops.fp_backward(self._fp_desc(s, G, dy=dy[G], dsrc=dx[G], dskip=dx[L], du_scratch=du, with_grads=True,
                                          interp_index=_at(s, "inv", G), bn_sums_done=bn_ok[L:L + 1], gather=False))
            dy_sa = buf[f"dy_sa{G}"].view(shapes[f"dy_sa{G}"])
            ops.global_pool_backward(du, _at(s, "arg", G), _at(s, "h_sa", G), gb.aux[2], gb.aux[3], B, Ms[L], dx[G], dy_sa,
                                     views[id(gb.bn.weight)], views[id(gb.bn.bias)])
            ops.fp_backward(self._global_sa_desc(s, dy=dy_sa, dsrc=dx[L], with_grads=True, bn_sums_done=bn_ok[L + 1:L + 2]))
        for l in range(L, 1, -1):
            ops.sa_backward(self._sa_desc(s, l, dout=dx[l], dfeat=dx[l - 1], g=True))
        ops.sa_backward(self._sa_desc(s, 1, dout=dx[1], g=True, bwd_ws=buf["sa1_ws"]))
        if getattr(self, "defer_grad_reduce", False):
            self._grad_images_pending = (arena,) + tuple(images)
        else:
            ops.grad_reduce(arena, flat.numel(), images)
            self._grad_images_pending = None
        s.flat_grad = flat
        self._last_flat_grad = flat
        return [views[id(p)] for p in params]

    @staticmethod
    def _grad_arena(params, sizes, dev):
        poffs, n_flat = ops.flat_layout(params)
        offs, tot = {}, 0
        for k, n in sizes.items():
            offs[k] = tot
            tot += (n + 3) // 4 * 4
        arena, flat, images, extra = ops.grad_images_alloc(n_flat, dev, tot)
        buf = {k: extra[offs[k]:offs[k] + n] for k, n in sizes.items()}
        views = {id(p): flat[o:o + p.numel()].view(p.shape) for p, o in zip(params, poffs)}
        return flat, buf, views, images, arena

    @staticmethod
    def get_long_form(data):
        B, f, N = data.shape
        return data.permute(1, 0, 2).reshape(f, B * N).transpose(1, 0)

    def get_batch_format(self, data):
        n = self.subsample_size
        return data.view(-1, n, data.shape[1]).transpose(1, 2)

    def set_patience_attributes(self, args):
        self.stopped_early = False
        self.best_metric_value = 10 ** 6
        self.best_metric_epoch = 1
        self.patience_in_epochs = args.patience_in_epochs

    def stop_early(self, val_metric, epoch, args):
# ... 30 lines not shown
```

Measured before the change: 24200 plots/s.

## Fold SA2 batch-norm finalize/apply into the fused global-level forward kernel

The SA2 forward now skips its separate BN finalize+apply launch and returns the pending stat-slot count. The fused global-level forward kernel then reduces the SA2 stat slots, computes the BN affine, applies it to the SA2 output and, when M2 fits, stages the result straight into LDS instead of reloading x2 from global memory. This removes one kernel launch and one read/write pass over the SA2 activation. In exchange, every block of the global kernel redundantly reduces all stat slots, and the kernel gains registers and shared-memory use.

```diff
diff --git a/include/strata_hip.h b/include/strata_hip.h
--- a/include/strata_hip.h
+++ b/include/strata_hip.h
@@ -156,6 +156,7 @@
 int sn2_sa_order_group(const int *cnt, int G, int B, int M, int *order, size_t stride_words, void *stream);
 int sn2_sa_forward(const sn2_sa *p, int training, void *stream);
 int sn2_sa_backward(const sn2_sa *p, void *stream);
+int sn2_sa_forward_pending(const sn2_sa *p, int *nslots, void *stream);
 
 typedef struct sn2_fp {
     int B, R_per_plot, S_per_plot;
@@ -206,6 +207,8 @@
 size_t sn2_global_xchg_words(int B);
 int sn2_global_level_forward(const sn2_fp *sa3, const sn2_fp *fp3, float *x3, int *arg3, unsigned long long *xchg,
                              unsigned *ctl, void *stream);
+int sn2_global_level_forward_sa2(const sn2_fp *sa3, const sn2_fp *fp3, float *x3, int *arg3, unsigned long long *xchg,
+                                 unsigned *ctl, const sn2_sa *sa2, int sa2_slots, void *stream);
 #define SN2_GLOBAL_BWD_MAX_ROWS 256
 #define SN2_GLOBAL_BWD_XCHG_WORDS ((size_t)2 * SN2_GLOBAL_MAX_PLOTS * 128)
 #define SN2_GLOBAL_BWD_CTL_WORDS 64
@@ -344,7 +347,9 @@
     int fuse_eval_head;
     int source_side;
     int fps_waves_shared, fps_waves_many;
+    int fold_bn_edges;
 } sn2_net_model;
+#define SN2_FOLD_SA2_FINALIZE 1
 
 typedef struct sn2_net_dims {
     int B, N, M1, M2;
@@ -451,6 +456,7 @@
 int sn2_fp_source_side(long R, int cb, int force);
 int sn2_global_level_forward_route(int B, int bf16);
 int sn2_global_level_backward_route(int B, int M2, int frozen, int bf16);
+int sn2_fold_sa2_finalize_route(int B, int bf16);
 int sn2_head_loss_route(int B, int N, int D);
 
 #ifdef __cplusplus
diff --git a/stratanet2_vegetation_coverage_maps_amd/_lib.py b/stratanet2_vegetation_coverage_maps_amd/_lib.py
--- a/stratanet2_vegetation_coverage_maps_amd/_lib.py
+++ b/stratanet2_vegetation_coverage_maps_amd/_lib.py
@@ -16,7 +16,7 @@
     "SN2_GLOBAL_BWD_XCHG_WORDS": 2 * 28 * 128, "SN2_GLOBAL_BWD_CTL_WORDS": 64,
     "SN2_MOSAIC_HIST_WORDS": 10004, "SN2_MOSAIC_CROP_MAX_BANDS": 8, "SN2_MOSAIC_CROP_MAX_EDGES": 1 << 20,
     "SN2_MOSAIC_CROP_MAX_BLOCKS": 2048, "SN2_KDE_FIT_MAX_K": 65536, "SN2_LOSS_BLOCKS": 1024, "SN2_PROJECTED_LOSS_WS": 2 * 512 + 2,
-    "SN2_NET_GRAD_IMAGES": 32, "SN2_METER_TERMS": 4,
+    "SN2_NET_GRAD_IMAGES": 32, "SN2_METER_TERMS": 4, "SN2_FOLD_SA2_FINALIZE": 1,
     "SN2_NET_FORK": 1, "SN2_NET_SHARED": 2, "SN2_NET_INVERTED": 4, "SN2_NET_DEFER_JOIN": 8, "SN2_NET_INPUT_ONLY": 16,
     "SN2_NET_HAS_ROWS0": 32, "SN2_NET_JOIN_PENDING": 64, "SN2_NET_WITH_GEOMETRY": 128, "SN2_NET_HAS_INVERTED": 256,
 }
@@ -81,7 +81,7 @@
                 ("g_lin1_W", c_int), ("g_lin1_b", c_int), ("g_lin2_W", c_int), ("g_lin2_b", c_int), ("n_flat", c_int),
                 ("r1_sq", c_float), ("r2_sq", c_float), ("max_neighbors", c_int), ("drop_p", c_float),
                 ("fuse_global_level", c_int), ("fuse_eval_head", c_int), ("source_side", c_int),
-                ("fps_waves_shared", c_int), ("fps_waves_many", c_int)]
+                ("fps_waves_shared", c_int), ("fps_waves_many", c_int), ("fold_bn_edges", c_int)]
 
 
 class NetDims(Structure):
@@ -164,6 +164,7 @@
     "sn2_sa_order": [c_void_p, c_int, c_int, c_void_p, c_void_p],
     "sn2_sa_order_group": [c_void_p, c_int, c_int, c_int, c_void_p, ctypes.c_size_t, c_void_p],
     "sn2_sa_forward": [POINTER(SA), c_int, c_void_p],
+    "sn2_sa_forward_pending": [POINTER(SA), POINTER(c_int), c_void_p],
     "sn2_sa_backward": [POINTER(SA), c_void_p],
     "sn2_grad_reduce": [c_void_p, c_int, c_int, c_int, c_void_p],
     "sn2_interp_index": [c_void_p, c_void_p, c_void_p, c_int, c_int, c_int, c_void_p, c_void_p],
@@ -176,6 +177,7 @@
     "sn2_global_pool_backward": [c_void_p, c_int, c_void_p, c_void_p, c_void_p, c_void_p, c_int, c_int, c_int, c_void_p, c_void_p,
                                  c_void_p, c_void_p, c_void_p],
     "sn2_global_level_forward": [POINTER(FP), POINTER(FP), c_void_p, c_void_p, c_void_p, c_void_p, c_void_p],
+    "sn2_global_level_forward_sa2": [POINTER(FP), POINTER(FP), c_void_p, c_void_p, c_void_p, c_void_p, POINTER(SA), c_int, c_void_p],
     "sn2_global_level_backward": [POINTER(FP), POINTER(FP), c_void_p, c_void_p, c_void_p, c_void_p],
     "sn2_debug_global_spin_limit": [ctypes.c_uint],
     "sn2_head_forward": [POINTER(Head), c_void_p],
@@ -231,6 +233,7 @@
     "sn2_fp_source_side": [c_long, c_int, c_int],
     "sn2_global_level_forward_route": [c_int, c_int],
     "sn2_global_level_backward_route": [c_int, c_int, c_int, c_int],
+    "sn2_fold_sa2_finalize_route": [c_int, c_int],
     "sn2_head_loss_route": [c_int, c_int, c_int],
 }
 
diff --git a/stratanet2_vegetation_coverage_maps_amd/csrc/global_level.hip b/stratanet2_vegetation_coverage_maps_amd/csrc/global_level.hip
--- a/stratanet2_vegetation_coverage_maps_amd/csrc/global_level.hip
+++ b/stratanet2_vegetation_coverage_maps_amd/csrc/global_level.hip
@@ -53,9 +53,21 @@
     long long* nbt;
     float* h;
 };
+struct GlPendingSa2 {
+    const float* slots;
+    int nb;
+    const unsigned long long* total;
+    const float *gamma, *beta;
+    float *running_mean, *running_var, *a, *c, *mean, *invstd;
+    long long* nbt;
+    const float* ext;
+    const int* arg;
+};
 struct GlArgs {
     int B, M2;
     const float* x2;
+    float* sa2_out;
+    GlPendingSa2 sa2;
     const float* pos2;
     const int* knn_idx;
     const float* knn_w;
@@ -66,6 +78,93 @@
     unsigned* ctl;
     unsigned spin_limit;
 };
+
+__device__ __forceinline__ void gl_finish_sa2(const GlPendingSa2& P, float* __restrict__ out, int M2, int b_lo, int b_hi, bool lead,
+                                              double* s_part, float* s_ac2, float* s_tiles) {
+    constexpr int C = 32, W2 = 2 * C, G = 1024 / W2, PRE = 2;
+    const int tid = threadIdx.x, col = tid % W2, g = tid / W2, nslots = P.nb;
+    const float* __restrict__ slots = P.slots;
+    const long lo4 = (long)b_lo * M2 * (C / 4), hi4 = (long)b_hi * M2 * (C / 4);
+    float4 e_pre[PRE];
+    int4 g_pre[PRE];
+#pragma unroll
+    for (int u = 0; u < PRE; ++u) {
+        const long i4 = min(lo4 + tid + 1024 * u, hi4 - 1);
+        e_pre[u] = reinterpret_cast<const float4*>(P.ext)[i4];
+        g_pre[u] = reinterpret_cast<const int4*>(P.arg)[i4];
+    }
+    double acc = 0.0;
+    int k = g;
+    for (; k + 31 * G < nslots; k += 32 * G) {
+        float v[32];
+#pragma unroll
+        for (int u = 0; u < 32; ++u) v[u] = slots[(size_t)(k + u * G) * W2 + col];
+#pragma unroll
+        for (int u = 0; u < 32; ++u) acc += (double)v[u];
+    }
+    for (; k + 7 * G < nslots; k += 8 * G) {
+        float v[8];
+#pragma unroll
+        for (int u = 0; u < 8; ++u) v[u] = slots[(size_t)(k + u * G) * W2 + col];
+#pragma unroll
+        for (int u = 0; u < 8; ++u) acc += (double)v[u];
+    }
+    for (; k < nslots; k += G) acc += (double)slots[(size_t)k * W2 + col];
+    s_part[tid] = acc;
+    __syncthreads();
+    if (tid < C) {
+        double s1 = 0.0, s2 = 0.0;
+        for (int gg = 0; gg < G; ++gg) {
+            s1 += s_part[gg * W2 + tid];
+            s2 += s_part[gg * W2 + C + tid];
+        }
+        float aa, cc, mean, invstd;
+        sn2_bn_from_sums(s1, s2, (double)(*P.total), P.gamma[tid], P.beta[tid], lead ? &P.running_mean[tid] : nullptr,
+                         lead ? &P.running_var[tid] : nullptr, aa, cc, mean, invstd);
+        if (lead) {
+            P.a[tid] = aa, P.c[tid] = cc, P.mean[tid] = mean, P.invstd[tid] = invstd;
+            if (tid == 0 && P.nbt) *P.nbt += 1;
+        }
+        s_ac2[tid] = aa, s_ac2[C + tid] = cc;
+    }
+    __syncthreads();
+    auto apply = [&](long i4, const float4& e, const int4& g4) {
+        const int o0 = (int)((i4 << 2) % C);
+        float4 r;
+        r.x = g4.x >= 0 ? fmaf(s_ac2[o0], e.x, s_ac2[C + o0]) : 0.f;
+        r.y = g4.y >= 0 ? fmaf(s_ac2[o0 + 1], e.y, s_ac2[C + o0 + 1]) : 0.f;
+        r.z = g4.z >= 0 ? fmaf(s_ac2[o0 + 2], e.z, s_ac2[C + o0 + 2]) : 0.f;
+        r.w = g4.w >= 0 ? fmaf(s_ac2[o0 + 3], e.w, s_ac2[C + o0 + 3]) : 0.f;
+        reinterpret_cast<float4*>(out)[i4] = r;
+        if (s_tiles) {
+            const int rp = (int)((i4 - lo4) >> 3), q = (int)(i4 & 7);
+            *reinterpret_cast<float4*>(&s_tiles[rp * GL_QS + 4 * q]) = r;
+        }
+    };
+    if (s_tiles) {
+        for (int i = M2 * (C / 4) + tid; i < ((M2 + 63) & ~63) * (C / 4); i += 1024)
+            *reinterpret_cast<float4*>(&s_tiles[(i >> 3) * GL_QS + 4 * (i & 7)]) = make_float4(0.f, 0.f, 0.f, 0.f);
+    }
+#pragma unroll
+    for (int u = 0; u < PRE; ++u) {
+        const long i4 = lo4 + tid + 1024 * u;
+        if (i4 < hi4) apply(i4, e_pre[u], g_pre[u]);
+    }
+    for (long i4 = lo4 + tid + 1024 * PRE; i4 < hi4; i4 += 1024)
+        apply(i4, reinterpret_cast<const float4*>(P.ext)[i4], reinterpret_cast<const int4*>(P.arg)[i4]);
+    __syncthreads();
+}
+
+__device__ __forceinline__ void gl_stage_pos(float* __restrict__ s_q, int g, int lane, long r0, long R_lim, const float* __restrict__ pos2) {
+    if (lane < 16) {
+        const int row = 16 * g + lane;
+        const long r = r0 + row;
+        const size_t rr = r < R_lim ? (size_t)r : (size_t)(R_lim - 1);
+        const float4 p = reinterpret_cast<const float4*>(pos2)[rr];
+        s_q[row * GL_QS + 32] = p.x, s_q[row * GL_QS + 33] = p.y, s_q[row * GL_QS + 34] = p.z;
+        s_q[row * GL_QS + 35] = 1.0f;
+    }
+}
 
 template <bool REPAIR>
 __device__ __forceinline__ void gl_level_body(const GlArgs& A, float* gl_smem) {
@@ -96,6 +195,8 @@
     b3r = A.sa3.bias[tid & 63], bfr = A.fp3.bias[tid & 63];
     unsigned epoch_now = 0;
     if (tid == 0) epoch_now = __hip_atomic_load(&A.ctl[0], __ATOMIC_RELAXED, __HIP_MEMORY_SCOPE_AGENT);
+    const bool x2_staged = !REPAIR && A.sa2.slots && M2 <= 64 * GL_GROUPS;
+    if (A.sa2.slots) gl_finish_sa2(A.sa2, A.sa2_out, M2, b_lo, b_hi, !REPAIR && blockIdx.x == 0, s_d, s_mv, x2_staged ? gl_smem : nullptr);
 #pragma unroll
     for (int j = 0; j < 3; ++j)
         if (tid + 1024 * j < 64 * 35) s_w3[tid + 1024 * j] = w3r[j];
@@ -128,8 +229,11 @@
             const int blk = it * GL_GROUPS + grp;
             const long r0 = row_lo + (long)blk * 64;
             if (blk < nblk) {
-                stage_inputs<CA, CB, false>(s_q, QS, g, lane, r0, (int)R_lim, M2, M2, A.x2, 32, nullptr, nullptr, nullptr, nullptr,
-                                            A.pos2, 4);
+                if (x2_staged)
+                    gl_stage_pos(s_q, g, lane, r0, R_lim, A.pos2);
+                else
+                    stage_inputs<CA, CB, false>(s_q, QS, g, lane, r0, (int)R_lim, M2, M2, A.x2, 32, nullptr, nullptr, nullptr, nullptr,
+                                                A.pos2, 4);
                 if (g == 2) {
 #pragma unroll
                     for (int k = CK; k < 4 * KB; ++k) s_q[lane * QS + k] = 0.f;
@@ -408,8 +512,10 @@
 extern "C" int sn2_global_level_forward_route(int B, int bf16) { return B <= GL_MAX_PLOTS && !bf16; }
 extern "C" size_t sn2_global_xchg_words(int B) { return SN2_GLOBAL_XCHG_WORDS(B); }
 
-extern "C" int sn2_global_level_forward(const sn2_fp* sa3, const sn2_fp* fp3, float* x3, int* arg3, unsigned long long* xchg,
-                                        unsigned* ctl, void* stream) {
+extern "C" int sn2_fold_sa2_finalize_route(int B, int bf16) { return sn2_global_level_forward_route(B, bf16); }
+
+static int global_level_forward_impl(const sn2_fp* sa3, const sn2_fp* fp3, float* x3, int* arg3, unsigned long long* xchg,
+                                     unsigned* ctl, const sn2_sa* sa2, int sa2_slots, void* stream) {
     if (!sa3 || !fp3 || !x3 || !arg3 || !xchg || !ctl) return SN2_EINVAL;
     const int B = sa3->B, M2 = sa3->R_per_plot;
     if (!(B > 0 && M2 > 0 && fp3->B == B && fp3->R_per_plot == M2 && sa3->S_per_plot == M2 && fp3->S_per_plot == 1)) return SN2_EINVAL;
@@ -427,6 +533,21 @@
             return SN2_EINVAL;
     GlArgs A;
     A.B = B, A.M2 = M2;
+    A.sa2_out = nullptr;
+    A.sa2 = GlPendingSa2{};
+    if (sa2) {
+        const sn2_block* k = &sa2->blk[0];
+        if (sa2->B != B || sa2->M != M2 || sa2->nl != 1 || sa2->cf != 16 || k->cout != 32) return SN2_ELIMIT;
+        if (!sa2->ext || !sa2->arg || !sa2->out || sa2->out != sa3->src || !sa2->total || !k->stat_slots || sa2_slots < 1 ||
+            sa2_slots > SN2_STAT_SLOTS || !k->gamma || !k->beta || !k->running_mean || !k->running_var || !k->a || !k->c || !k->mean ||
+            !k->invstd)
+            return SN2_EINVAL;
+        A.sa2_out = sa2->out;
+        A.sa2.slots = k->stat_slots, A.sa2.nb = sa2_slots, A.sa2.total = sa2->total;
+        A.sa2.gamma = k->gamma, A.sa2.beta = k->beta, A.sa2.running_mean = k->running_mean, A.sa2.running_var = k->running_var;
+        A.sa2.a = k->a, A.sa2.c = k->c, A.sa2.mean = k->mean, A.sa2.invstd = k->invstd, A.sa2.nbt = k->num_batches_tracked;
+        A.sa2.ext = sa2->ext, A.sa2.arg = sa2->arg;
+    }
     A.x2 = sa3->src, A.pos2 = sa3->skip, A.knn_idx = fp3->knn_idx, A.knn_w = fp3->knn_w, A.x3 = x3, A.arg3 = arg3;
     auto layer = [](const sn2_fp* p) {
         GlLayer l;
@@ -444,3 +565,14 @@
     hipLaunchKernelGGL(global_level_fwd_kernel, dim3(B), dim3(1024), lds, (hipStream_t)stream, A);
     SN2_RETURN_LAUNCH();
 }
+
+extern "C" int sn2_global_level_forward(const sn2_fp* sa3, const sn2_fp* fp3, float* x3, int* arg3, unsigned long long* xchg,
+                                        unsigned* ctl, void* stream) {
+    return global_level_forward_impl(sa3, fp3, x3, arg3, xchg, ctl, nullptr, 0, stream);
+}
+
+extern "C" int sn2_global_level_forward_sa2(const sn2_fp* sa3, const sn2_fp* fp3, float* x3, int* arg3, unsigned long long* xchg,
+                                            unsigned* ctl, const sn2_sa* sa2, int sa2_slots, void* stream) {
+    if (!sa2) return SN2_EINVAL;
+    return global_level_forward_impl(sa3, fp3, x3, arg3, xchg, ctl, sa2, sa2_slots, stream);
+}
diff --git a/stratanet2_vegetation_coverage_maps_amd/csrc/net.hip b/stratanet2_vegetation_coverage_maps_amd/csrc/net.hip
--- a/stratanet2_vegetation_coverage_maps_amd/csrc/net.hip
+++ b/stratanet2_vegetation_coverage_maps_amd/csrc/net.hip
@@ -474,12 +474,18 @@
     SN2_TRY(sn2_sa_forward(&sa, mode, cur));
     if (join_b) NET_HIP(hipStreamWaitEvent(cur, ctx->b_tables, 0));
     sa2_desc(&sa, m, d, g, a, nograd, nullptr, nullptr);
-    SN2_TRY(sn2_sa_forward(&sa, mode, cur));
+    const bool gl_fused = batch_stats && m->fuse_global_level && io->gl_xchg && io->gl_ctl && sn2_global_level_forward_route(B, gl_bf16(m));
+    const bool fold_sa2 = gl_fused && (m->fold_bn_edges & SN2_FOLD_SA2_FINALIZE) && sn2_fold_sa2_finalize_route(B, gl_bf16(m) || m->sa2.mma_bf16);
+    int sa2_slots = 0;
+    if (fold_sa2) SN2_TRY(sn2_sa_forward_pending(&sa, &sa2_slots, cur));
+    else SN2_TRY(sn2_sa_forward(&sa, mode, cur));
     if (join_b) NET_HIP(hipStreamWaitEvent(cur, ctx->b_nn, 0));
     sn2_fp p3, pf3;
     fp_desc(&p3, d, a, sa3_in(m, d, g, a), nograd);
     fp_desc(&pf3, d, a, fp3_in(m, d, g, a), nograd);
-    if (batch_stats && m->fuse_global_level && io->gl_xchg && io->gl_ctl && sn2_global_level_forward_route(B, gl_bf16(m))) {
+    if (fold_sa2) {
+        SN2_TRY(sn2_global_level_forward_sa2(&p3, &pf3, a->x3, a->arg3, io->gl_xchg, io->gl_ctl, &sa, sa2_slots, cur));
+    } else if (gl_fused) {
         SN2_TRY(sn2_global_level_forward(&p3, &pf3, a->x3, a->arg3, io->gl_xchg, io->gl_ctl, cur));
     } else {
         SN2_TRY(sn2_fp_forward(&p3, mode, cur));
diff --git a/stratanet2_vegetation_coverage_maps_amd/csrc/sa.hip b/stratanet2_vegetation_coverage_maps_amd/csrc/sa.hip
--- a/stratanet2_vegetation_coverage_maps_amd/csrc/sa.hip
+++ b/stratanet2_vegetation_coverage_maps_amd/csrc/sa.hip
@@ -85,7 +85,7 @@
 }
 
 template <int CF, int NL, int C1, int C2>
-int forward_t(const sn2_sa* p, int training, hipStream_t st) {
+int forward_t(const sn2_sa* p, int training, hipStream_t st, int* pending_slots = nullptr) {
     const sn2_block* last = &p->blk[NL - 1];
     int nb = 0;
     const int batch_stats = training == 1;
@@ -98,6 +98,10 @@
         return sa_mfma_launch_fwd<CF, NL, C1, C2, 1>(p, 0, st, &nb);
     }
     SN2_TRY((sa_mfma_launch_fwd<CF, NL, C1, C2, 1>(p, training, st, &nb)));
+    if (pending_slots) {
+        *pending_slots = nb;
+        return 0;
+    }
     return sn2_bn_finalize_apply(last, batch_stats ? nb : 0, p->total, 0, batch_stats, p->ext, p->arg, p->out, (long)p->B * p->M, st);
 }
 
@@ -228,6 +232,12 @@
     return forward_t<16, 1, 32, 32>(p, training, (hipStream_t)stream);
 }
 
+extern "C" int sn2_sa_forward_pending(const sn2_sa* p, int* nslots, void* stream) {
+    SN2_TRY(check(p));
+    if (!nslots || p->nl != 1 || p->cf != 16) return SN2_ELIMIT;
+    return forward_t<16, 1, 32, 32>(p, 1, (hipStream_t)stream, nslots);
+}
+
 extern "C" int sn2_sa_backward(const sn2_sa* p, void* stream) {
     SN2_TRY(check(p));
     if (!p->dout) return SN2_EINVAL;
diff --git a/stratanet2_vegetation_coverage_maps_amd/executor.py b/stratanet2_vegetation_coverage_maps_amd/executor.py
--- a/stratanet2_vegetation_coverage_maps_amd/executor.py
+++ b/stratanet2_vegetation_coverage_maps_amd/executor.py
@@ -246,6 +246,7 @@
         m.drop_p = float(model.drop)
         m.fuse_global_level, m.fuse_eval_head, m.source_side = int(bool(model.fuse_global_level)), int(bool(model.fuse_eval_head)), int(bool(ops.SOURCE_SIDE))
         m.fps_waves_shared, m.fps_waves_many = int(model.fps_waves_shared), int(model.fps_waves_many)
+        m.fold_bn_edges = int(model.fold_mask())
         self.c = m
         self.settings = settings_of(model, max_neighbors)
         self.key = tuple(t.data_ptr() for t in self.tensors)
@@ -271,7 +272,7 @@
     return (model.mma_dtype, float(model.drop), bool(model.fuse_global_level), bool(model.fuse_eval_head), bool(ops.SOURCE_SIDE),
             int(model.fps_waves_shared), int(model.fps_waves_many), float(model.sa1_module.r), float(model.sa2_module.r),
             float(model.sa1_module.ratio), float(model.sa2_module.ratio), int(max_neighbors), model.p2_diam_pix,
-            bool(model.fp1_morton_rows))
+            bool(model.fp1_morton_rows), int(model.fold_mask()))
 
 
 class NetCtx:
diff --git a/stratanet2_vegetation_coverage_maps_amd/hip_ops.py b/stratanet2_vegetation_coverage_maps_amd/hip_ops.py
--- a/stratanet2_vegetation_coverage_maps_amd/hip_ops.py
+++ b/stratanet2_vegetation_coverage_maps_amd/hip_ops.py
@@ -751,6 +751,12 @@
     _call("sn2_sa_forward", d, int(training), _stream(), tag=f"cf={d.cf}")
 
 
+def sa_forward_pending(d: SA) -> int:
+    n = ctypes.c_int(0)
+    _call("sn2_sa_forward_pending", d, ctypes.byref(n), _stream(), tag=f"cf={d.cf}")
+    return int(n.value)
+
+
 def sa_backward(d: SA):
     _call("sn2_sa_backward", d, _stream(), tag=f"cf={d.cf}")
 
@@ -948,11 +954,23 @@
     return bool(_host("sn2_global_level_forward_route", int(B), int(any(b.mma_bf16 for b in blocks))))
 
 
-def global_level_forward(d_sa3: FP, d_fp3: FP, x3: torch.Tensor, arg3: torch.Tensor, owner=None):
+FOLD_SA2_FINALIZE = _lib.SN2_FOLD_SA2_FINALIZE
+FOLD_BUILT = FOLD_SA2_FINALIZE
+
+
+def fold_sa2_finalize(B: int, *blocks) -> bool:
+    return bool(_host("sn2_fold_sa2_finalize_route", int(B), int(any(b.mma_bf16 for b in blocks))))
+
+
+def global_level_forward(d_sa3: FP, d_fp3: FP, x3: torch.Tensor, arg3: torch.Tensor, owner=None, sa2: Optional[SA] = None,
+                         sa2_slots: int = 0):
     B = d_sa3.B
     _chk(x3, F32, (B, 64), "x3")
     _chk(arg3, I32, (B, 64), "arg3")
     ws = global_level_ws(x3.device, B, owner=owner)
+    if sa2 is not None:
+        _call("sn2_global_level_forward_sa2", d_sa3, d_fp3, _ptr(x3), _ptr(arg3), _ptr(ws[0]), _ptr(ws[1]), sa2, int(sa2_slots), _stream())
+        return
     _call("sn2_global_level_forward", d_sa3, d_fp3, _ptr(x3), _ptr(arg3), _ptr(ws[0]), _ptr(ws[1]), _stream())
 
 
diff --git a/stratanet2_vegetation_coverage_maps_amd/point_net2.py b/stratanet2_vegetation_coverage_maps_amd/point_net2.py
--- a/stratanet2_vegetation_coverage_maps_amd/point_net2.py
+++ b/stratanet2_vegetation_coverage_maps_amd/point_net2.py
@@ -165,6 +165,11 @@
     fuse_eval_head = os.environ.get("SN2_FUSE_EVAL_HEAD", "1") == "1"
     fuse_global_level = os.environ.get("SN2_FUSE_GLOBAL_LEVEL", "1") == "1"
     fuse_loss_backward = os.environ.get("SN2_FUSE_LOSS_BACKWARD", "1") == "1"
+    fold_bn_edges = True
+
+    def fold_mask(self) -> int:
+        return (int(os.environ.get("SN2_FOLD_BN_EDGES", "7")) & ops.FOLD_BUILT) if self.fold_bn_edges else 0
+
     p2_diam_pix = None
 
     def set_mma_dtype(self, dtype: str):
@@ -667,21 +672,30 @@
             s.rows0 = rows0
         else:
             s.rows0 = ops.pack_rows(cloud, xyz)
+        gl_fused = bool(training) and self.fuse_global_level and ops.global_level_forward_fused(B, s.b_glob, s.b_fp[G])
+        fold_sa2 = (gl_fused and L == 2 and bool(self.fold_mask() & ops.FOLD_SA2_FINALIZE)
+                    and ops.fold_sa2_finalize(B, s.b_sa[L][-1], s.b_glob, s.b_fp[G]))
+        sa2_desc, sa2_slots = None, 0
         for l in range(1, L + 1):
             R, C = B * Ms[l], s.b_sa[l][-1].cout
             _put(s, "ext", l, e(R, C))
             _put(s, "arg", l, e(R, C, dt=I32))
             _put(s, "x", l, e(R, C))
-            ops.sa_forward(self._sa_desc(s, l), mode)
+            if l == L and fold_sa2:
+                sa2_desc = self._sa_desc(s, l)
+                sa2_slots = ops.sa_forward_pending(sa2_desc)
+            else:
+                ops.sa_forward(self._sa_desc(s, l), mode)
             if l == 1 and join is not None:
                 cur_stream.wait_stream(join[0])
         R, C = B * Ms[L], s.b_glob.cout
         _put(s, "h_sa", G, e(R, _pad4(C)))
         _put(s, "h", G, e(R, _pad4(s.b_fp[G].cout)))
-        if training and self.fuse_global_level and ops.global_level_forward_fused(B, s.b_glob, s.b_fp[G]):
+        if gl_fused:
             _put(s, "x", G, e(B, C))
             _put(s, "arg", G, e(B, C, dt=I32))
-            ops.global_level_forward(self._global_sa_desc(s), self._fp_desc(s, G), _at(s, "x", G), _at(s, "arg", G), owner=self)
+            ops.global_level_forward(self._global_sa_desc(s), self._fp_desc(s, G), _at(s, "x", G), _at(s, "arg", G), owner=self,
+                                     sa2=sa2_desc, sa2_slots=sa2_slots)
         else:
             ops.fp_forward(self._global_sa_desc(s), mode)
             x, arg = ops.plot_max_forward(_at(s, "h_sa", G), s.b_glob.a, s.b_glob.c, B, Ms[L], C)
```

Result: no change. 24250 plots/s (median of 6 runs) (+0.2%).
